# MrTornado24/IDE-3D

Hardware: NVIDIA H100
Metric: rendered frames/sec at 64^2 neural x 96 samples -> 512^2 (higher is better)
Workload: dtype f32

## Files before the change

ide-3d_b200/_lib.py:

```python

import ctypes as C
import os

import torch

_HERE = os.path.dirname(os.path.abspath(__file__))
LIB_PATH = os.environ.get('IDE3D_B200_LIB') or os.path.join(_HERE, 'lib', 'libide3d_b200.so')

OK, UNSUPPORTED, INVALID, CUDA_ERROR = 0, -1, -2, -3
F32, F16, F64 = 0, 1, 2
JITTER_NONE, JITTER_TENSOR, JITTER_HASH, JITTER_ZVALS = 0, 1, 2, 3
CLAMP_SOFTPLUS, CLAMP_RELU = 0, 1
PRECISION = {'auto': 0, 'fp32': 1, 'tc': 2}

_DTYPES = {torch.float32: F32, torch.float16: F16, torch.float64: F64}


class UpfirParams(C.Structure):
    _fields_ = [('x', C.c_void_p), ('f', C.c_void_p), ('y', C.c_void_p), ('dtype', C.c_int),
                ('up_x', C.c_int), ('up_y', C.c_int), ('down_x', C.c_int), ('down_y', C.c_int),
                ('pad_x0', C.c_int), ('pad_y0', C.c_int), ('flip', C.c_int), ('gain', C.c_float),
                ('in_w', C.c_int), ('in_h', C.c_int), ('in_c', C.c_int), ('in_n', C.c_int),
                ('in_stride_w', C.c_int64), ('in_stride_h', C.c_int64), ('in_stride_c', C.c_int64), ('in_stride_n', C.c_int64),
                ('f_w', C.c_int), ('f_h', C.c_int), ('f_stride_w', C.c_int64), ('f_stride_h', C.c_int64),
                ('out_w', C.c_int), ('out_h', C.c_int),
                ('out_stride_w', C.c_int64), ('out_stride_h', C.c_int64), ('out_stride_c', C.c_int64), ('out_stride_n', C.c_int64)]


class FirEpilogue(C.Structure):
    _fields_ = [('scale', C.c_void_p), ('noise', C.c_void_p), ('b', C.c_void_p), ('scale2', C.c_void_p), ('y2', C.c_void_p),
                ('act', C.c_int), ('alpha', C.c_float), ('gain', C.c_float), ('clamp', C.c_float), ('noise_batch', C.c_int64)]


class StyleLayer(C.Structure):
    _fields_ = [('affine_w', C.c_void_p), ('affine_b', C.c_void_p), ('wsq', C.c_void_p), ('w_gain', C.c_float), ('b_gain', C.c_float),
                ('out_scale', C.c_float), ('w_index', C.c_int), ('in_ch', C.c_int), ('out_ch', C.c_int),
                ('style_off', C.c_int64), ('dcoef_off', C.c_int64)]


class FlreluParams(C.Structure):
    _fields_ = [('x', C.c_void_p), ('b', C.c_void_p), ('fu', C.c_void_p), ('fd', C.c_void_p), ('y', C.c_void_p),
                ('s', C.c_void_p), ('dtype', C.c_int), ('up', C.c_int), ('down', C.c_int),
                ('fu_w', C.c_int), ('fu_h', C.c_int), ('fd_w', C.c_int), ('fd_h', C.c_int),
                ('pad_x0', C.c_int), ('pad_y0', C.c_int), ('flip', C.c_int),
                ('gain', C.c_float), ('slope', C.c_float), ('clamp', C.c_float),
                ('x_w', C.c_int), ('x_h', C.c_int), ('x_c', C.c_int), ('x_n', C.c_int),
                ('x_stride_w', C.c_int64), ('x_stride_h', C.c_int64), ('x_stride_c', C.c_int64), ('x_stride_n', C.c_int64),
                ('y_w', C.c_int), ('y_h', C.c_int),
                ('y_stride_w', C.c_int64), ('y_stride_h', C.c_int64), ('y_stride_c', C.c_int64), ('y_stride_n', C.c_int64),
                ('s_w', C.c_int), ('s_h', C.c_int), ('s_ofs_x', C.c_int), ('s_ofs_y', C.c_int),
                ('write_signs', C.c_int), ('read_signs', C.c_int)]


class FlreluActParams(C.Structure):
    _fields_ = [('x', C.c_void_p), ('s', C.c_void_p), ('dtype', C.c_int),
                ('x_w', C.c_int), ('x_h', C.c_int), ('x_c', C.c_int), ('x_n', C.c_int),
                ('x_stride_w', C.c_int64), ('x_stride_h', C.c_int64), ('x_stride_c', C.c_int64), ('x_stride_n', C.c_int64),
                ('s_w', C.c_int), ('s_h', C.c_int), ('s_ofs_x', C.c_int), ('s_ofs_y', C.c_int),
                ('gain', C.c_float), ('slope', C.c_float), ('clamp', C.c_float),
                ('write_signs', C.c_int), ('read_signs', C.c_int)]


class TriPlane(C.Structure):
    _fields_ = [('data', C.c_void_p), ('n', C.c_int), ('h', C.c_int), ('w', C.c_int),
                ('stride_n', C.c_int64), ('stride_c', C.c_int64), ('stride_h', C.c_int64), ('stride_w', C.c_int64)]


class MlpHead(C.Structure):
    _fields_ = [('in_sel', C.c_int), ('hidden', C.c_int), ('out_offset', C.c_int), ('out_count', C.c_int),
                ('w1', C.c_void_p), ('b1', C.c_void_p), ('w2', C.c_void_p), ('b2', C.c_void_p)]


class Decoder(C.Structure):
    _fields_ = [('num_heads', C.c_int), ('heads', MlpHead * 4)]


class RaymarchParams(C.Structure):
    _fields_ = [('tex', TriPlane), ('seg', TriPlane), ('dec', Decoder), ('cam2world', C.c_void_p),
                ('n', C.c_int), ('res_w', C.c_int), ('res_h', C.c_int), ('num_steps', C.c_int),
                ('fov_deg', C.c_float), ('ray_start', C.c_float), ('ray_end', C.c_float), ('box_scale', C.c_float),
                ('jitter_mode', C.c_int), ('jitter_u', C.c_void_p), ('jitter_seed', C.c_uint64),
                ('clamp_mode', C.c_int), ('last_back', C.c_int), ('white_back', C.c_int), ('max_depth', C.c_float),
                ('fill_weight', C.c_int), ('noise_std', C.c_float), ('noise', C.c_void_p),
                ('out_feat', C.c_void_p), ('out_depth', C.c_void_p), ('out_weights', C.c_void_p), ('precision', C.c_int),
                ('views', C.c_int), ('jitter_seeds', C.c_void_p)]


class RasterParams(C.Structure):
    _fields_ = [('vertices', C.c_void_p), ('triangles', C.c_void_p), ('normals', C.c_void_p), ('cam2world', C.c_void_p),
                ('num_vertices', C.c_int64), ('num_triangles', C.c_int64), ('num_frames', C.c_int), ('width', C.c_int), ('height', C.c_int),
                ('yfov_deg', C.c_float), ('znear', C.c_float), ('base', C.c_float), ('ambient', C.c_float), ('diffuse', C.c_float),
                ('background', C.c_int), ('rgb', C.c_void_p), ('ids', C.c_void_p), ('scratch', C.c_void_p), ('scratch_bytes', C.c_int64)]


FRAMES_IMAGE_SEG, FRAMES_IMAGE_DEPTH = 1, 2
FRAMES_PARTIALS = 64


class FramesParams(C.Structure):
    _fields_ = [('image', C.c_void_p), ('n', C.c_int), ('height', C.c_int), ('width', C.c_int),
                ('image_stride_n', C.c_int64), ('image_stride_c', C.c_int64), ('image_stride_h', C.c_int64), ('image_stride_w', C.c_int64),
                ('seg', C.c_void_p), ('seg_c', C.c_int), ('seg_h', C.c_int), ('seg_w', C.c_int),
                ('seg_stride_n', C.c_int64), ('seg_stride_c', C.c_int64), ('seg_stride_h', C.c_int64), ('seg_stride_w', C.c_int64),
                ('lut', C.c_void_p), ('mode', C.c_int), ('out', C.c_void_p), ('scratch', C.c_void_p)]


class StripsParams(C.Structure):
    _fields_ = [('image', C.c_void_p), ('seeds', C.c_int), ('views', C.c_int), ('height', C.c_int), ('width', C.c_int),
                ('image_stride_n', C.c_int64), ('image_stride_c', C.c_int64), ('image_stride_h', C.c_int64), ('image_stride_w', C.c_int64),
                ('seg', C.c_void_p), ('seg_c', C.c_int), ('seg_h', C.c_int), ('seg_w', C.c_int),
                ('seg_stride_n', C.c_int64), ('seg_stride_c', C.c_int64), ('seg_stride_h', C.c_int64), ('seg_stride_w', C.c_int64),
                ('lut', C.c_void_p), ('out_image', C.c_void_p), ('out_seg', C.c_void_p)]


NOISE_MAX_BUFFERS = 64


class NoiseTable(C.Structure):
    _fields_ = [('count', C.c_int), ('sides', C.c_int * NOISE_MAX_BUFFERS), ('bufs', C.c_void_p * NOISE_MAX_BUFFERS),
                ('grads', C.c_void_p * NOISE_MAX_BUFFERS), ('scratch', C.c_void_p), ('scratch_floats', C.c_int64)]


class SegXentParams(C.Structure):
    _fields_ = [('seg', C.c_void_p), ('n', C.c_int), ('classes', C.c_int), ('in_h', C.c_int), ('in_w', C.c_int),
                ('seg_stride_n', C.c_int64), ('seg_stride_c', C.c_int64), ('seg_stride_h', C.c_int64), ('seg_stride_w', C.c_int64),
                ('mask', C.c_void_p), ('out_h', C.c_int), ('out_w', C.c_int), ('lse', C.c_void_p), ('partials', C.c_void_p),
                ('loss', C.c_void_p), ('grad_loss', C.c_void_p), ('grad_seg', C.c_void_p)]


LPIPS_MAX_LAYERS = 8


class LpipsLayer(C.Structure):
    _fields_ = [('c', C.c_int), ('h', C.c_int), ('w', C.c_int), ('x', C.c_void_p), ('x_stride', C.c_int64 * 4),
                ('y', C.c_void_p), ('y_stride', C.c_int64 * 4), ('lin', C.c_void_p),
                ('grad_x', C.c_void_p), ('gx_stride', C.c_int64 * 4), ('grad_y', C.c_void_p), ('gy_stride', C.c_int64 * 4)]


class LpipsParams(C.Structure):
    _fields_ = [('n', C.c_int), ('num_layers', C.c_int), ('layers', LpipsLayer * LPIPS_MAX_LAYERS), ('value', C.c_void_p),
                ('scratch', C.c_void_p), ('scratch_bytes', C.c_int64), ('grad_value', C.c_void_p)]


_lib = None


class _StreamHandle(int):
    device = None


class _GuardedLib:

    def __init__(self, lib):
        self._lib = lib

    def __getattr__(self, name):
        fn = getattr(self._lib, name)
        if not name.startswith('ide3d_'):
            return fn

        def call(*args):
            dev = getattr(args[-1], 'device', None) if args else None
            if dev is None:
                return fn(*args)
            with torch.cuda.device(dev):
                return fn(*args)

        call.__name__ = name
        self.__dict__[name] = call
        return call


def get_lib():
    global _lib
    if _lib is not None:
        return _lib
    if not os.path.exists(LIB_PATH):
        raise RuntimeError(f'ide3d_b200: CUDA library not built ({LIB_PATH} missing); run '
                           f'`python {os.path.join(_HERE, "build.py")}` -- there is no CPU fallback')
    lib = C.CDLL(LIB_PATH, mode=os.RTLD_NOW)
    lib.ide3d_last_error.restype = C.c_char_p
    lib.ide3d_launch_count.restype = C.c_uint64
    vp, i32, i64, f32 = C.c_void_p, C.c_int, C.c_int64, C.c_float
    lib.ide3d_bias_act.argtypes = [vp, vp, vp, vp, vp, vp, i32, i32, i32, f32, f32, f32, i64, i64, i64, vp]
    lib.ide3d_modconv_epilogue.argtypes = [vp, vp, vp, vp, vp, vp, vp, i32, i32, f32, f32, f32, i64, i64, i64, i64, i32, vp]
    lib.ide3d_modconv_epilogue_rgb.argtypes = [vp, vp, vp, vp, vp, vp, vp, vp, vp, vp, vp, vp, i64, i32, i32, f32, f32, f32, i64, i64, i64,
                                               i64, vp]
    lib.ide3d_upfirdn2d.argtypes = [C.POINTER(UpfirParams), vp]
    lib.ide3d_upfirdn2d_add.argtypes = [C.POINTER(UpfirParams), vp, i64, i64, i64, vp, vp]
    lib.ide3d_upfirdn2d_epilogue.argtypes = [C.POINTER(UpfirParams), C.POINTER(FirEpilogue), vp]
    lib.ide3d_filtered_lrelu.argtypes = [C.POINTER(FlreluParams), vp]
    lib.ide3d_filtered_lrelu_act.argtypes = [C.POINTER(FlreluActParams), vp]
    lib.ide3d_raymarch_fwd.argtypes = [C.POINTER(RaymarchParams), vp]
    lib.ide3d_raymarch_bwd.argtypes = [C.POINTER(RaymarchParams), vp, vp, vp, vp, C.POINTER(C.c_void_p), vp]
    lib.ide3d_raymarch_bwd_cam.argtypes = [C.POINTER(RaymarchParams), vp, vp, vp, vp, C.POINTER(C.c_void_p), vp, vp]
    lib.ide3d_sample_voxel.argtypes = [C.POINTER(TriPlane), C.POINTER(TriPlane), C.POINTER(Decoder), vp, i64, f32, i32, vp, vp]
    lib.ide3d_sigma_grid.argtypes = [C.POINTER(TriPlane), C.POINTER(TriPlane), C.POINTER(Decoder), i32,
                                     C.POINTER(C.c_float * 3), f32, f32, f32, i64, i64, vp, vp]
    lib.ide3d_planes_to_nhwc.argtypes = [vp, i32, i32, i32, i32, i64, i64, i64, i64, vp, vp]
    lib.ide3d_initial_rays.argtypes = [i32, i32, f32, i32, i32, f32, f32, vp, vp, vp, vp]
    lib.ide3d_transform_points.argtypes = [vp, vp, vp, vp, vp, i32, i32, i32, vp, vp, vp, vp, vp]
    lib.ide3d_sample_triplane.argtypes = [C.POINTER(TriPlane), vp, i64, vp, vp]
    lib.ide3d_mask2color.argtypes = [vp, i32, i32, i32, i32, i64, i64, i64, i64, vp, vp, i32, vp]
    lib.ide3d_integrate.argtypes = [vp, vp, vp, vp, f32, i32, i32, i32, i32, i32, i32, i32, f32, i32, vp, vp, vp, vp]
    lib.ide3d_sample_pdf.argtypes = [vp, vp, vp, i32, i32, i32, f32, vp, vp]
    lib.ide3d_mc_classify.argtypes = [vp, i32, i32, i32, f32, vp, vp, vp]
    lib.ide3d_mc_emit.argtypes = [vp, i32, i32, i32, f32, vp, vp, vp, vp, vp, vp, vp]
    lib.ide3d_style_plan.argtypes = [vp, i32, i32, i32, C.POINTER(StyleLayer), i32, vp, vp, vp]
    lib.ide3d_mesh_normals.argtypes = [vp, vp, i64, vp, vp, vp, vp]
    lib.ide3d_raster_scratch_bytes.argtypes = [i32, i32, i32, i64, i64]
    lib.ide3d_raster_scratch_bytes.restype = C.c_int64
    lib.ide3d_raster.argtypes = [C.POINTER(RasterParams), vp]
    lib.ide3d_video_frames.argtypes = [C.POINTER(FramesParams), vp]
    lib.ide3d_image_strips.argtypes = [C.POINTER(StripsParams), vp]
    lib.ide3d_noise_reg.argtypes = [C.POINTER(NoiseTable), vp, vp, vp]
    lib.ide3d_noise_normalize.argtypes = [C.POINTER(NoiseTable), vp]
    lib.ide3d_seg_xent_fwd.argtypes = [C.POINTER(SegXentParams), vp]
    lib.ide3d_seg_xent_bwd.argtypes = [C.POINTER(SegXentParams), vp]
    lib.ide3d_lpips_scratch_bytes.argtypes = [C.POINTER(LpipsParams)]
    lib.ide3d_lpips_scratch_bytes.restype = C.c_int64
    lib.ide3d_lpips_fwd.argtypes = [C.POINTER(LpipsParams), vp]
    lib.ide3d_lpips_bwd.argtypes = [C.POINTER(LpipsParams), vp]
    for name in ('bias_act', 'upfirdn2d', 'filtered_lrelu', 'filtered_lrelu_act', 'raymarch_fwd', 'raymarch_bwd', 'raymarch_bwd_cam', 'sample_voxel',
                 'sigma_grid', 'planes_to_nhwc', 'initial_rays', 'transform_points', 'sample_triplane', 'integrate',
                 'sample_pdf', 'style_plan', 'mc_classify', 'mc_emit', 'mesh_normals', 'raster', 'video_frames', 'image_strips',
                 'noise_reg', 'noise_normalize', 'seg_xent_fwd', 'seg_xent_bwd', 'lpips_fwd', 'lpips_bwd', 'abi_version'):
        getattr(lib, 'ide3d_' + name).restype = C.c_int
    if lib.ide3d_abi_version() != 1:
        raise RuntimeError('ide3d_b200: ABI version mismatch between _lib.py and libide3d_b200.so')
    _lib = _GuardedLib(lib)
    return _lib


def exported_symbols():
    return ['ide3d_abi_version', 'ide3d_last_error', 'ide3d_launch_count', 'ide3d_bias_act', 'ide3d_modconv_epilogue', 'ide3d_modconv_epilogue_rgb',
            'ide3d_upfirdn2d', 'ide3d_upfirdn2d_add', 'ide3d_upfirdn2d_epilogue',
            'ide3d_filtered_lrelu', 'ide3d_filtered_lrelu_act', 'ide3d_raymarch_fwd', 'ide3d_raymarch_bwd', 'ide3d_raymarch_bwd_cam', 'ide3d_sample_voxel',
            'ide3d_sigma_grid', 'ide3d_planes_to_nhwc', 'ide3d_initial_rays', 'ide3d_transform_points',
            'ide3d_sample_triplane', 'ide3d_integrate', 'ide3d_sample_pdf', 'ide3d_mask2color', 'ide3d_style_plan', 'ide3d_mc_classify', 'ide3d_mc_emit',
            'ide3d_mesh_normals', 'ide3d_raster_scratch_bytes', 'ide3d_raster', 'ide3d_video_frames', 'ide3d_image_strips',
            'ide3d_noise_reg', 'ide3d_noise_normalize', 'ide3d_seg_xent_fwd', 'ide3d_seg_xent_bwd',
            'ide3d_lpips_scratch_bytes', 'ide3d_lpips_fwd', 'ide3d_lpips_bwd']


def check(rc, allow_unsupported=False):
    if rc == OK or (allow_unsupported and rc == UNSUPPORTED):
        return rc
    msg = get_lib().ide3d_last_error().decode(errors='replace')
    raise RuntimeError(f'ide3d_b200: {msg} (status {rc})')


def require_cuda(*tensors):
    for t in tensors:
        if t is not None and (not isinstance(t, torch.Tensor) or t.device.type != 'cuda'):
            raise RuntimeError('ide3d_b200: tensors must reside on a CUDA device -- this package has no CPU path '
                               '(the CPU restatement lives in oracle/ and is test infrastructure only)')


def forbid_grad(name, *tensors):
    if torch.is_grad_enabled() and any(isinstance(t, torch.Tensor) and t.requires_grad for t in tensors):
        raise RuntimeError(f'ide3d_b200.{name}: inputs require grad, but this stage kernel is forward-only -- use '
                           f'ide3d_b200.render.raymarch (fused forward, render_grad backward) or wrap the call in torch.no_grad()')


def dtype_code(t):
    try:
        return _DTYPES[t.dtype]
    except KeyError:
        raise RuntimeError(f'ide3d_b200: unsupported dtype {t.dtype}') from None


def ptr(t):
    return None if t is None else t.data_ptr()


def stream_ptr(device=None):
    h = _StreamHandle(torch.cuda.current_stream(device).cuda_stream)
    h.device = torch.device('cuda', torch.cuda.current_device()) if device is None else torch.device(device)
    return h


def launch_count():
    return int(get_lib().ide3d_launch_count())


def triplane_view(t):
    if t.ndim != 4 or t.shape[1] != 96 or t.dtype != torch.float32:
        raise RuntimeError(f'ide3d_b200: tri-plane tensor must be float32 [N, 96, H, W], got {tuple(t.shape)} {t.dtype}')
    s = t.stride()
    return TriPlane(t.data_ptr(), t.shape[0], t.shape[2], t.shape[3], s[0], s[1], s[2], s[3])
```

ide-3d_b200/_plugins.py:

```python

import ctypes as C

import torch

from . import _lib as L


def _req(cond, msg):
    if not cond:
        raise RuntimeError(msg)


def _has(t):
    return t is not None and t.numel() > 0


def _suggest_memory_format(x):
    if x.ndim == 4 and x.is_contiguous(memory_format=torch.channels_last) and not x.is_contiguous():
        return torch.channels_last
    return torch.contiguous_format


def bias_act(x, b, xref, yref, dy, grad, dim, act, alpha, gain, clamp):
    L.require_cuda(x)
    _req(not _has(b) or (b.dtype == x.dtype and b.device == x.device), 'b must have the same dtype and device as x')
    for name, t in (('xref', xref), ('yref', yref), ('dy', dy)):
        _req(not _has(t) or (t.shape == x.shape and t.dtype == x.dtype and t.device == x.device),
             f'{name} must have the same shape, dtype, and device as x')
    _req(not _has(b) or b.ndim == 1, 'b must have rank 1')
    _req(not _has(b) or (0 <= dim < x.ndim), 'dim is out of bounds')
    _req(not _has(b) or b.shape[0] == x.shape[dim], 'b has wrong number of elements')
    _req(grad >= 0, 'grad must be non-negative')
    dense = x.is_contiguous() or (x.ndim == 4 and x.is_contiguous(memory_format=torch.channels_last))
    _req(dense, 'x must be non-overlapping and dense')
    for t in (xref, yref, dy):
        _req(not _has(t) or t.stride() == x.stride(), 'xref, yref and dy must have the same layout as x')
    if _has(b):
        b = b.contiguous()
    y = torch.empty_like(x)
    if x.numel() == 0:
        return y
    step_b = x.stride(dim) if _has(b) else 1
    rc = L.get_lib().ide3d_bias_act(L.ptr(x), L.ptr(b) if _has(b) else None, L.ptr(xref) if _has(xref) else None,
                                    L.ptr(yref) if _has(yref) else None, L.ptr(dy) if _has(dy) else None, L.ptr(y),
                                    L.dtype_code(x), int(grad), int(act), float(alpha), float(gain), float(clamp),
                                    x.numel(), b.numel() if _has(b) else 0, step_b, L.stream_ptr(x.device))
    L.check(rc)
    return y


def modconv_epilogue(x, scale, noise, b, act, alpha, gain, clamp, next_scale=None, only_next=False):
    L.require_cuda(x)
    _req(x.ndim == 4, 'x must be rank 4')
    n, c, h, w = x.shape
    cl = (not x.is_contiguous()) and x.is_contiguous(memory_format=torch.channels_last)
    _req(x.is_contiguous() or cl, 'x must be non-overlapping and dense')
    vec = 16 // x.element_size()
    if x.numel() == 0 or (cl and c % vec != 0) or (not cl and (h * w) % vec != 0):
        return None
    if _has(scale):
        _req(scale.numel() == n * c, 'scale must have N*C elements')
        scale = scale.to(dtype=x.dtype).reshape(n, c).contiguous()
    noise_batch = 1
    if _has(noise):
        _req(noise.numel() in (h * w, n * h * w), 'noise must be [H,W] or [N,1,H,W]')
        noise_batch = noise.numel() // (h * w)
        noise = noise.to(dtype=x.dtype).contiguous()
    if _has(b):
        _req(b.ndim == 1 and b.shape[0] == c, 'b has wrong number of elements')
        b = b.to(dtype=x.dtype).contiguous()
    y = y2 = None
    if _has(next_scale):
        _req(next_scale.numel() == n * c, 'next_scale must have N*C elements')
        next_scale = next_scale.to(dtype=x.dtype).reshape(n, c).contiguous()
        y2 = torch.empty_like(x)
    if not (only_next and y2 is not None):
        y = torch.empty_like(x)
    rc = L.get_lib().ide3d_modconv_epilogue(L.ptr(x), L.ptr(scale) if _has(scale) else None, L.ptr(noise) if _has(noise) else None,
                                            L.ptr(b) if _has(b) else None, L.ptr(y) if y is not None else None,
                                            L.ptr(next_scale) if y2 is not None else None, L.ptr(y2) if y2 is not None else None,
                                            L.dtype_code(x), int(act), float(alpha), float(gain), float(clamp), n, c, h * w,
                                            noise_batch, int(cl), L.stream_ptr(x.device))
    if L.check(rc, allow_unsupported=True) == L.UNSUPPORTED:
        return None
    if y2 is None:
        return y
    return y2 if y is None else (y, y2)


def modconv_epilogue_rgb(x, scale, noise, b, act, alpha, gain, clamp, emit_y=True, y_scale=None, next_scale=None, rgb=None):
    L.require_cuda(x)
    _req(x.ndim == 4, 'x must be rank 4')
    n, c, h, w = x.shape
    cl = (not x.is_contiguous()) and x.is_contiguous(memory_format=torch.channels_last)
    if not cl or x.dtype != torch.float32 or c % 4 != 0 or c > 512 or x.numel() == 0:
        return None

    def per_sample(t, name):
        if not _has(t):
            return None
        _req(t.numel() == n * c, f'{name} must have N*C elements')
        return t.to(dtype=x.dtype).reshape(n, c).contiguous()

    scale, y_scale, next_scale = per_sample(scale, 'scale'), per_sample(y_scale, 'y_scale'), per_sample(next_scale, 'next_scale')
    noise_batch = 1
    if _has(noise):
        _req(noise.numel() in (h * w, n * h * w), 'noise must be [H,W] or [N,1,H,W]')
        noise_batch = noise.numel() // (h * w)
        noise = noise.to(dtype=x.dtype).contiguous()
    if _has(b):
        _req(b.ndim == 1 and b.shape[0] == c, 'b has wrong number of elements')
        b = b.to(dtype=x.dtype).contiguous()
    _req(y_scale is None or emit_y, 'y_scale needs emit_y')
    wrgb = srgb = brgb = out_rgb = None
    o = 0
    if rgb is not None:
        wrgb, srgb, brgb = rgb
        o = wrgb.shape[0]
        if o > 4:
            return None
        _req(wrgb.numel() == o * c, 'rgb weight must be [O, C, 1, 1]')
        wrgb = wrgb.to(dtype=x.dtype).reshape(o, c).contiguous()
        srgb = per_sample(srgb, 'rgb styles')
        if brgb is not None:
            _req(brgb.numel() == o, 'rgb bias must have O elements')
            brgb = brgb.to(dtype=x.dtype).contiguous()
        out_rgb = torch.empty([n, o, h, w], dtype=x.dtype, device=x.device)
    y = torch.empty_like(x) if emit_y else None
    y2 = torch.empty_like(x) if next_scale is not None else None
    _req(y is not None or y2 is not None or out_rgb is not None, 'no output requested')
    opt = lambda t: L.ptr(t) if t is not None else None
    rc = L.get_lib().ide3d_modconv_epilogue_rgb(L.ptr(x), opt(scale), opt(noise), opt(b), opt(y_scale), opt(y), opt(next_scale), opt(y2),
                                                opt(wrgb), opt(srgb), opt(brgb), opt(out_rgb), o, L.dtype_code(x), int(act), float(alpha),
                                                float(gain), float(clamp), n, c, h * w, noise_batch, L.stream_ptr(x.device))
    if L.check(rc, allow_unsupported=True) == L.UNSUPPORTED:
        return None
    return [t for t in (y, y2, out_rgb) if t is not None]


def upfirdn2d(x, f, upx, upy, downx, downy, padx0, padx1, pady0, pady1, flip, gain, add=None, bias=None, epilogue=None):
    L.require_cuda(x, f)
    _req(f.device == x.device, 'f must reside on the same device as x')
    _req(f.dtype == torch.float32, 'f must be float32')
    _req(x.numel() > 0, 'x has zero size')
    _req(f.numel() > 0, 'f has zero size')
    _req(x.ndim == 4, 'x must be rank 4')
    _req(f.ndim == 2, 'f must be rank 2')
    _req(f.shape[0] >= 1 and f.shape[1] >= 1, 'f must be at least 1x1')
    _req(upx >= 1 and upy >= 1, 'upsampling factor must be at least 1')
    _req(downx >= 1 and downy >= 1, 'downsampling factor must be at least 1')
    n, c, h, w = x.shape
    fh, fw = f.shape
    out_w = (w * upx + padx0 + padx1 - fw + downx) // downx
    out_h = (h * upy + pady0 + pady1 - fh + downy) // downy
    _req(out_w >= 1 and out_h >= 1, 'output must be at least 1x1')
    y = torch.empty([n, c, out_h, out_w], dtype=x.dtype, device=x.device, memory_format=_suggest_memory_format(x))
    xs, ys, fs = x.stride(), y.stride(), f.stride()
    p = L.UpfirParams(L.ptr(x), L.ptr(f), L.ptr(y), L.dtype_code(x), upx, upy, downx, downy, padx0, pady0,
                      1 if flip else 0, float(gain), w, h, c, n, xs[3], xs[2], xs[1], xs[0],
                      fw, fh, fs[1], fs[0], out_w, out_h, ys[3], ys[2], ys[1], ys[0])
    if epilogue is not None:
        e = epilogue
        if not (y.is_contiguous(memory_format=torch.channels_last) and not y.is_contiguous()) or e['act'] not in (1, 3) or x.dtype == torch.float64:
            return None
        def prep(t, numel):
            if t is None:
                return None
            _req(t.numel() == numel, 'epilogue operand has the wrong number of elements')
            return t.to(dtype=x.dtype).contiguous()
        scale, b, scale2 = prep(e.get('scale'), n * c), prep(e.get('b'), c), prep(e.get('next_scale'), n * c)
        noise = e.get('noise')
        noise_batch = 1
        if noise is not None:
            _req(noise.numel() in (out_h * out_w, n * out_h * out_w), 'noise must be [H,W] or [N,1,H,W]')
            noise_batch = noise.numel() // (out_h * out_w)
            noise = noise.to(dtype=x.dtype).contiguous()
        y2 = torch.empty_like(y) if scale2 is not None else None
        want_y = not (e.get('only_next') and y2 is not None)
        if not want_y:
            p.y = None
        ep = L.FirEpilogue(L.ptr(scale) if scale is not None else None, L.ptr(noise) if noise is not None else None,
                           L.ptr(b) if b is not None else None, L.ptr(scale2) if scale2 is not None else None,
                           L.ptr(y2) if y2 is not None else None, int(e['act']), float(e['alpha']), float(e['gain']),
                           float(e['clamp']), noise_batch)
        rc = L.get_lib().ide3d_upfirdn2d_epilogue(C.byref(p), C.byref(ep), L.stream_ptr(x.device))
        if L.check(rc, allow_unsupported=True) == L.UNSUPPORTED:
            return None
        if y2 is None:
            return y
        return (y, y2) if want_y else y2
    if add is not None:
        if tuple(add.shape) != (n, c, out_h, out_w) or add.dtype != x.dtype or add.stride(1) != 1 or not y.is_contiguous(memory_format=torch.channels_last) or y.is_contiguous():
            return None
        if bias is not None:
            bias = bias.to(dtype=x.dtype).contiguous()
        a = add.stride()
        rc = L.get_lib().ide3d_upfirdn2d_add(C.byref(p), L.ptr(add), a[0], a[2], a[3], L.ptr(bias) if bias is not None else None,
                                             L.stream_ptr(x.device))
        return None if L.check(rc, allow_unsupported=True) == L.UNSUPPORTED else y
    L.check(L.get_lib().ide3d_upfirdn2d(C.byref(p), L.stream_ptr(x.device)))
    return y


def filtered_lrelu(x, fu, fd, b, si, up, down, px0, px1, py0, py1, sx, sy, gain, slope, clamp, flip_filters, writeSigns):
    L.require_cuda(x, fu, fd, b)
    _req(fu.device == x.device and fd.device == x.device and b.device == x.device, 'all input tensors must reside on the same device')
    _req(fu.dtype == torch.float32 and fd.dtype == torch.float32, 'fu and fd must be float32')
    _req(b.dtype == x.dtype, 'x and b must have the same dtype')
    _req(x.dtype in (torch.float16, torch.float32), 'x and b must be float16 or float32')
    _req(x.ndim == 4, 'x must be rank 4')
    _req(x.numel() > 0, 'x is empty')
    _req(fu.ndim in (1, 2) and fd.ndim in (1, 2), 'fu and fd must be rank 1 or 2')
    _req(fu.numel() > 0, 'fu is empty')
    _req(fd.numel() > 0, 'fd is empty')
    _req(b.ndim == 1 and b.shape[0] == x.shape[1], 'b must be a vector with the same number of channels as x')
    _req(up >= 1 and down >= 1, 'up and down must be at least 1')
    n, c, xh, xw = x.shape
    fut_w, fut_h = fu.shape[-1] - 1, fu.shape[0] - 1
    fdt_w, fdt_h = fd.shape[-1] - 1, fd.shape[0] - 1
    cw = xw * up + (px0 + px1) - fut_w
    ch = xh * up + (py0 + py1) - fut_h
    _req(cw > fdt_w and ch > fdt_h, 'upsampled buffer must be at least the size of downsampling filter')
    yw = (cw - fdt_w + (down - 1)) // down
    yh = (ch - fdt_h + (down - 1)) // down
    _req(yw > 0 and yh > 0, 'output must be at least 1x1')
    read_signs = _has(si)
    s = si if read_signs else None
    so = None
    sw = sh = 0
    y = torch.empty([n, c, yh, yw], dtype=x.dtype, device=x.device, memory_format=_suggest_memory_format(x))
    if writeSigns:
        sw_active = yw * down - (down - 1) + fdt_w
        sh = yh * down - (down - 1) + fdt_h
        sw = (sw_active + 15) & ~15
        s = so = torch.empty([n, c, sh, sw >> 2], dtype=torch.uint8, device=x.device)
    elif read_signs:
        _req(s.is_contiguous(), 'signs must be contiguous')
        _req(s.dtype == torch.uint8, 'signs must be uint8')
        _req(s.ndim == 4 and s.shape[0] == n and s.shape[1] == c, 'signs must have same batch & channels as x')
        sw, sh = s.shape[3] << 2, s.shape[2]
    fu_c, fd_c = fu.contiguous(), fd.contiguous()
    xs, ys = x.stride(), y.stride()
    p = L.FlreluParams(L.ptr(x), L.ptr(b.contiguous()), L.ptr(fu_c), L.ptr(fd_c), L.ptr(y), L.ptr(s) if s is not None else None,
                       L.dtype_code(x), up, down, fu.shape[-1], fu.shape[0] if fu.ndim == 2 else 0,
                       fd.shape[-1], fd.shape[0] if fd.ndim == 2 else 0, px0, py0, 1 if flip_filters else 0,
                       float(gain), float(slope), float(min(clamp, 3.0e38)), xw, xh, c, n, xs[3], xs[2], xs[1], xs[0],
                       yw, yh, ys[3], ys[2], ys[1], ys[0], sw, sh, sx, sy, 1 if writeSigns else 0,
                       1 if (read_signs and not writeSigns) else 0)
    rc = L.check(L.get_lib().ide3d_filtered_lrelu(C.byref(p), L.stream_ptr(x.device)), allow_unsupported=True)
    if rc == L.UNSUPPORTED:
        return None, None, -1
    return y, so, 0


def filtered_lrelu_act_(x, si, sx, sy, gain, slope, clamp, writeSigns):
    L.require_cuda(x)
    _req(x.ndim == 4, 'x must be rank 4')
    _req(x.numel() > 0, 'x is empty')
    _req(x.dtype in (torch.float16, torch.float32, torch.float64), 'x must be float16, float32 or float64')
    read_signs = _has(si)
    s, so = (si if read_signs else None), None
    n, c, h, w = x.shape
    if writeSigns:
        sw = (w + 15) & ~15
        s = so = torch.empty([n, c, h, sw >> 2], dtype=torch.uint8, device=x.device)
    if s is not None:
        _req(s.is_contiguous(), 'signs must be contiguous')
        _req(s.dtype == torch.uint8, 'signs must be uint8')
        _req(s.device == x.device, 'signs must reside on the same device as x')
        _req(s.ndim == 4 and s.shape[0] == n and s.shape[1] == c, 'signs must have same batch & channels as x')
    xs = x.stride()
    p = L.FlreluActParams(L.ptr(x), L.ptr(s) if s is not None else None, L.dtype_code(x), w, h, c, n,
                          xs[3], xs[2], xs[1], xs[0], (s.shape[3] << 2) if s is not None else 0,
                          s.shape[2] if s is not None else 0, sx, sy, float(gain), float(slope),
                          float(min(clamp, 3.0e38)), 1 if writeSigns else 0, 1 if (read_signs and not writeSigns) else 0)
    L.check(L.get_lib().ide3d_filtered_lrelu_act(C.byref(p), L.stream_ptr(x.device)))
    return so


class _Plugin:

    def __init__(self, name, **funcs):
        self.__name__ = name
        self.__dict__.update(funcs)


PLUGINS = {
    'bias_act_plugin': _Plugin('bias_act_plugin', bias_act=bias_act, modconv_epilogue=modconv_epilogue,
                                 modconv_epilogue_rgb=modconv_epilogue_rgb),
    'upfirdn2d_plugin': _Plugin('upfirdn2d_plugin', upfirdn2d=upfirdn2d),
    'filtered_lrelu_plugin': _Plugin('filtered_lrelu_plugin', filtered_lrelu=filtered_lrelu,
                                     filtered_lrelu_act_=filtered_lrelu_act_),
}
```

ide-3d_b200/build.py:

```python

import hashlib
import os
import shutil
import subprocess
import sys
from concurrent.futures import ThreadPoolExecutor

HERE = os.path.dirname(os.path.abspath(__file__))
CSRC = os.path.join(HERE, 'csrc')
OBJ = os.path.join(HERE, '_build_tuning' if os.environ.get('IDE3D_BUILD_TUNING', '0') == '1' else '_build')
LIBDIR = os.path.join(HERE, 'lib')
LIB = os.path.join(LIBDIR, 'libide3d_b200_tuning.so' if os.environ.get('IDE3D_BUILD_TUNING', '0') == '1' else 'libide3d_b200.so')
TUNING = os.environ.get('IDE3D_BUILD_TUNING', '0') == '1'
UNITS = ['capi', 'raymarch', 'raymarch_bwd', 'raymarch_tc', 'voxel', 'voxel_tc', 'stages', 'style_plan', 'mcubes', 'raster', 'frames', 'strips', 'projector', 'lpips', 'bias_act', 'upfirdn2d', 'filtered_lrelu', 'filtered_lrelu_fused']
NVCC_FLAGS = ['-O3', '-std=c++17', '--expt-relaxed-constexpr', '-gencode', 'arch=compute_90a,code=sm_90a',
              '-lineinfo', '-Xcompiler', '-fPIC', '-Xptxas', '-v'] + (['-DIDE3D_TUNING'] if TUNING else [])


def _nvcc():
    for cand in (os.environ.get('NVCC'), shutil.which('nvcc'), '/usr/local/cuda/bin/nvcc'):
        if cand and os.path.exists(cand):
            return cand
    raise RuntimeError('nvcc not found (set NVCC=/path/to/nvcc)')


def _sources():
    return [u for u in UNITS if os.path.exists(os.path.join(CSRC, u + '.cu'))]


def _digest():
    h = hashlib.sha256(' '.join(NVCC_FLAGS).encode())
    names = sorted(os.listdir(CSRC)) + ['../../include/ide3d_b200.h']
    for n in names:
        p = os.path.join(CSRC, n)
        if os.path.isfile(p):
            h.update(n.encode())
            h.update(open(p, 'rb').read())
    return h.hexdigest()


def _compile(nvcc, unit, verbose):
    src = os.path.join(CSRC, unit + '.cu')
    obj = os.path.join(OBJ, unit + '.o')
    cmd = [nvcc, '-c'] + NVCC_FLAGS + [src, '-o', obj]
    r = subprocess.run(cmd, stdout=subprocess.PIPE, stderr=subprocess.STDOUT, text=True)
    with open(os.path.join(OBJ, unit + '.log'), 'w') as f:
        f.write(' '.join(cmd) + '\n' + r.stdout)
    if r.returncode != 0:
        raise RuntimeError(f'nvcc failed on {unit}.cu:\n{r.stdout[-6000:]}')
    if verbose:
        print(r.stdout)
    return obj


def build(force=False, verbose=False):
    os.makedirs(OBJ, exist_ok=True)
    os.makedirs(LIBDIR, exist_ok=True)
    stamp = os.path.join(LIBDIR, 'build_tuning.sha256' if TUNING else 'build.sha256')
    digest = _digest()
    if not force and os.path.exists(LIB) and os.path.exists(stamp) and open(stamp).read().strip() == digest:
        return LIB
    nvcc = _nvcc()
    units = _sources()
    with ThreadPoolExecutor(max_workers=min(8, len(units))) as ex:
        objs = list(ex.map(lambda u: _compile(nvcc, u, verbose), units))
    cmd = [nvcc, '-shared', '-gencode', 'arch=compute_90a,code=sm_90a', '-o', LIB] + objs + ['-lcudart']
    r = subprocess.run(cmd, stdout=subprocess.PIPE, stderr=subprocess.STDOUT, text=True)
    if r.returncode != 0:
        raise RuntimeError('link failed:\n' + r.stdout)
    with open(stamp, 'w') as f:
        f.write(digest)
    return LIB


if __name__ == '__main__':
    path = build(force='--force' in sys.argv, verbose='--verbose' in sys.argv)
    print(path)
```

ide-3d_b200/csrc/bias_act.cu:

```cuda
#include "common.cuh"

namespace ide3d {

struct BiasActArgs {
    const void *x, *b, *xref, *yref, *dy;
    void* y;
    int grad;
    float alpha, gain, clamp;
    long long size_x, size_b, step_b;
};

template <typename T> struct Acc { using type = float; };
template <> struct Acc<double> { using type = double; };

template <typename S> __device__ __forceinline__ S exp_(S v);
template <> __device__ __forceinline__ float exp_<float>(float v) { return __expf(v); }
template <> __device__ __forceinline__ double exp_<double>(double v) { return exp(v); }
template <typename S> __device__ __forceinline__ S log_(S v);
template <> __device__ __forceinline__ float log_<float>(float v) { return __logf(v); }
template <> __device__ __forceinline__ double log_<double>(double v) { return log(v); }

template <typename S, int A>
__device__ __forceinline__ S eval(S x, S b, S xref, S yref, S dy, int G, S alpha, S gain, S clamp) {
    const S one = (S)1, two = (S)2, expRange = (S)80, halfExpRange = (S)40;
    const S seluScale = (S)1.0507009873554804934193349852946, seluAlpha = (S)1.6732632423543772848170429916717;
    const S yy = (gain != (S)0) ? yref / gain : (S)0;
    S y = 0;
    if (G == 0) x += b; else xref += b;
    if (A == 1) { y = x; if (G == 2) y = 0; }
    if (A == 2) { if (G == 0) y = (x > 0) ? x : 0; if (G == 1) y = (yy > 0) ? x : 0; }
    if (A == 3) { if (G == 0) y = (x > 0) ? x : x * alpha; if (G == 1) y = (yy > 0) ? x : x * alpha; }
    if (A == 4) {
        if (G == 0) { const S c = exp_(x), d = one / c; y = (x < -expRange) ? -one : (x > expRange) ? one : (c - d) / (c + d); }
        if (G == 1) y = x * (one - yy * yy);
        if (G == 2) y = x * (one - yy * yy) * (-two * yy);
    }
    if (A == 5) {
        if (G == 0) y = (x < -expRange) ? 0 : one / (exp_(-x) + one);
        if (G == 1) y = x * yy * (one - yy);
        if (G == 2) y = x * yy * (one - yy) * (one - two * yy);
    }
    if (A == 6) {
        if (G == 0) y = (x >= 0) ? x : exp_(x) - one;
        if (G == 1) y = (yy >= 0) ? x : x * (yy + one);
        if (G == 2) y = (yy >= 0) ? 0 : x * (yy + one);
    }
    if (A == 7) {
        if (G == 0) y = (x >= 0) ? seluScale * x : (seluScale * seluAlpha) * (exp_(x) - one);
        if (G == 1) y = (yy >= 0) ? x * seluScale : x * (yy + seluScale * seluAlpha);
        if (G == 2) y = (yy >= 0) ? 0 : x * (yy + seluScale * seluAlpha);
    }
    if (A == 8) {
        if (G == 0) y = (x > expRange) ? x : log_(exp_(x) + one);
        if (G == 1) y = x * (one - exp_(-yy));
        if (G == 2) { const S c = exp_(-yy); y = x * c * (one - c); }
    }
    if (A == 9) {
        if (G == 0) {
            y = (x < -expRange) ? 0 : x / (exp_(-x) + one);
        } else {
            const S c = exp_(xref), d = c + one;
            if (G == 1) y = (xref > halfExpRange) ? x : x * c * (xref + d) / (d * d);
            else y = (xref > halfExpRange) ? 0 : x * c * (xref * (two - d) + two * d) / (d * d * d);
            yref = (xref < -expRange) ? 0 : xref / (exp_(-xref) + one) * gain;
        }
    }
    y *= gain * dy;
    if (clamp >= 0) {
        if (G == 0) y = (y > -clamp & y < clamp) ? y : (y >= 0) ? clamp : -clamp;
        else y = (yref > -clamp & yref < clamp) ? y : 0;
    }
    return y;
}

__device__ __forceinline__ long long bias_index(long long e, const BiasActArgs& p, bool small) {
    if (small) return (long long)(((unsigned)e / (unsigned)p.step_b) % (unsigned)p.size_b);
    return (e / p.step_b) % p.size_b;
}

template <typename T> struct Vec;
template <> struct Vec<float> { static constexpr int N = 4; using type = float4; };
template <> struct Vec<__half> { static constexpr int N = 8; using type = uint4; };
template <> struct Vec<double> { static constexpr int N = 2; using type = double2; };

template <typename T> __device__ __forceinline__ typename Acc<T>::type to_acc(T v) { return (typename Acc<T>::type)v; }
template <> __device__ __forceinline__ float to_acc<__half>(__half v) { return __half2float(v); }
template <typename T> __device__ __forceinline__ T from_acc(typename Acc<T>::type v) { return (T)v; }
template <> __device__ __forceinline__ __half from_acc<__half>(float v) { return __float2half(v); }

__device__ __forceinline__ void load_vec(const float* p, long long v, float (&o)[4]) {
    const float4 t = __ldcs(reinterpret_cast<const float4*>(p) + v);
    o[0] = t.x; o[1] = t.y; o[2] = t.z; o[3] = t.w;
}
__device__ __forceinline__ void load_vec(const double* p, long long v, double (&o)[2]) {
    const double2 t = __ldcs(reinterpret_cast<const double2*>(p) + v);
    o[0] = t.x; o[1] = t.y;
}
__device__ __forceinline__ void load_vec(const __half* p, long long v, float (&o)[8]) {
    const uint4 t = __ldcs(reinterpret_cast<const uint4*>(p) + v);
    const unsigned w[4] = {t.x, t.y, t.z, t.w};
#pragma unroll
    for (int i = 0; i < 4; ++i) {
        const float2 f = __half22float2(*reinterpret_cast<const __half2*>(&w[i]));
        o[2 * i] = f.x; o[2 * i + 1] = f.y;
    }
}
__device__ __forceinline__ void store_vec(float* p, long long v, const float (&o)[4]) {
    __stcs(reinterpret_cast<float4*>(p) + v, make_float4(o[0], o[1], o[2], o[3]));
}
__device__ __forceinline__ void store_vec(double* p, long long v, const double (&o)[2]) {
    __stcs(reinterpret_cast<double2*>(p) + v, make_double2(o[0], o[1]));
}
__device__ __forceinline__ void store_vec(__half* p, long long v, const float (&o)[8]) {
    unsigned w[4];
#pragma unroll
    for (int i = 0; i < 4; ++i) {
        const __half2 h = __floats2half2_rn(o[2 * i], o[2 * i + 1]);
        w[i] = *reinterpret_cast<const unsigned*>(&h);
    }
    __stcs(reinterpret_cast<uint4*>(p) + v, make_uint4(w[0], w[1], w[2], w[3]));
}

template <typename T, int A, int UNROLL, bool kFwd>
__global__ void __launch_bounds__(256) bias_act_kernel(const BiasActArgs p, const int bmode) {
    using S = typename Acc<T>::type;
    constexpr int N = Vec<T>::N;
    const S alpha = (S)p.alpha, gain = (S)p.gain, clamp = (S)p.clamp;
    const int G = kFwd ? 0 : p.grad;
    const T* x = (const T*)p.x;
    const T* b = (const T*)p.b;
    const T* xref = (const T*)p.xref;
    const T* yref = (const T*)p.yref;
    const T* dy = (const T*)p.dy;
    T* y = (T*)p.y;
    const long long nvec = p.size_x / N;
    const long long stride = (long long)gridDim.x * blockDim.x;
    const bool small = p.size_x <= 0x7fffffffll;

    for (long long v0 = (long long)blockIdx.x * blockDim.x + threadIdx.x; v0 < nvec; v0 += stride * UNROLL) {
        S vx[UNROLL][N];
#pragma unroll
        for (int u = 0; u < UNROLL; ++u) {
            const long long v = v0 + u * stride;
            if (v < nvec) load_vec(x, v, vx[u]);
        }
#pragma unroll
        for (int u = 0; u < UNROLL; ++u) {
            const long long v = v0 + u * stride;
            if (v >= nvec) continue;
            const long long e0 = v * N;
            S exr[N], eyr[N], edy[N], out[N], bb[N];
            if (xref) load_vec(xref, v, exr);
            if (yref) load_vec(yref, v, eyr);
            if (dy) load_vec(dy, v, edy);
            if (bmode == 1) {
                const S t = to_acc<T>(b[bias_index(e0, p, small)]);
#pragma unroll
                for (int j = 0; j < N; ++j) bb[j] = t;
            } else if (bmode == 2) {
                const long long i0 = small ? (long long)((unsigned)e0 % (unsigned)p.size_b) : e0 % p.size_b;
#pragma unroll
                for (int j = 0; j < N; ++j) bb[j] = to_acc<T>(b[i0 + j]);
            } else {
#pragma unroll
                for (int j = 0; j < N; ++j) bb[j] = (bmode == 3) ? to_acc<T>(b[bias_index(e0 + j, p, small)]) : (S)0;
            }
#pragma unroll
            for (int j = 0; j < N; ++j)
                out[j] = eval<S, A>(vx[u][j], bb[j], xref ? exr[j] : (S)0, yref ? eyr[j] : (S)0, dy ? edy[j] : (S)1, G, alpha, gain, clamp);
            store_vec(y, v, out);
        }
    }
    const long long tail0 = nvec * N;
    for (long long e = tail0 + (long long)blockIdx.x * blockDim.x + threadIdx.x; e < p.size_x; e += stride) {
        const S bb = b ? to_acc<T>(b[bias_index(e, p, small)]) : (S)0;
        y[e] = from_acc<T>(eval<S, A>(to_acc<T>(x[e]), bb, xref ? to_acc<T>(xref[e]) : (S)0,
                                      yref ? to_acc<T>(yref[e]) : (S)0, dy ? to_acc<T>(dy[e]) : (S)1, G, alpha,
                                      gain, clamp));
    }
}

template <typename T, int A, int UNROLL, bool kFwd>
__global__ void __launch_bounds__(256) bias_act_planar_kernel(const BiasActArgs p, long long plane_elems, long long chunks_per_plane,
                                                             long long items) {
    using S = typename Acc<T>::type;
    constexpr int N = Vec<T>::N;
    const S alpha = (S)p.alpha, gain = (S)p.gain, clamp = (S)p.clamp;
    const int G = kFwd ? 0 : p.grad;
    const T* b = (const T*)p.b;
    const long long plane_vecs = plane_elems / N;
    for (long long item = blockIdx.x; item < items; item += gridDim.x) {
        const long long plane = item / chunks_per_plane;
        const long long chunk = item - plane * chunks_per_plane;
        const S bias = b ? to_acc<T>(b[plane % p.size_b]) : (S)0;
        const long long vbase = plane * plane_vecs;
        const long long v0 = chunk * (256 * UNROLL) + threadIdx.x;
        S vx[UNROLL][N];
#pragma unroll
        for (int u = 0; u < UNROLL; ++u)
            if (v0 + u * 256 < plane_vecs) load_vec((const T*)p.x, vbase + v0 + u * 256, vx[u]);
#pragma unroll
        for (int u = 0; u < UNROLL; ++u) {
            const long long vi = v0 + u * 256;
            if (vi >= plane_vecs) continue;
            const long long v = vbase + vi;
            S exr[N], eyr[N], edy[N], out[N];
            if (p.xref) load_vec((const T*)p.xref, v, exr);
            if (p.yref) load_vec((const T*)p.yref, v, eyr);
            if (p.dy) load_vec((const T*)p.dy, v, edy);
#pragma unroll
            for (int j = 0; j < N; ++j)
                out[j] = eval<S, A>(vx[u][j], bias, p.xref ? exr[j] : (S)0, p.yref ? eyr[j] : (S)0, p.dy ? edy[j] : (S)1, G, alpha, gain, clamp);
            store_vec((T*)p.y, v, out);
        }
    }
}

template <typename T, int A>
static int launch_bias_act(const BiasActArgs& p, cudaStream_t st) {
    constexpr int UNROLL = 4;
    constexpr int N = Vec<T>::N;
    const long long nvec = p.size_x / N;
    long long blocks = ceil_div<long long>(nvec > 0 ? nvec : 1, 256ll * UNROLL);
    const long long cap = (long long)sm_count() * 8;
    if (blocks > cap) blocks = cap;
    if (blocks < 1) blocks = 1;
    int bmode = 0;
    if (p.b != nullptr) bmode = (p.step_b % N == 0) ? 1 : ((p.step_b == 1 && p.size_b % N == 0) ? 2 : 3);
    const long long plane_elems = (p.b == nullptr) ? p.size_x : p.step_b;
    if ((p.b == nullptr || bmode == 1) && plane_elems >= 1024 && plane_elems % N == 0 && p.size_x % plane_elems == 0) {
        const long long cpp = ceil_div<long long>(plane_elems / N, 256ll * UNROLL);
        const long long items = (p.size_x / plane_elems) * cpp;
        long long g = items < cap ? items : cap;
        if (p.grad == 0) bias_act_planar_kernel<T, A, UNROLL, true><<<(unsigned)g, 256, 0, st>>>(p, plane_elems, cpp, items);
        else bias_act_planar_kernel<T, A, UNROLL, false><<<(unsigned)g, 256, 0, st>>>(p, plane_elems, cpp, items);
        IDE3D_CHECK_LAUNCH("bias_act_planar_kernel");
        return IDE3D_OK;
    }
    if (p.grad == 0) bias_act_kernel<T, A, UNROLL, true><<<(unsigned)blocks, 256, 0, st>>>(p, bmode);
    else bias_act_kernel<T, A, UNROLL, false><<<(unsigned)blocks, 256, 0, st>>>(p, bmode);
    IDE3D_CHECK_LAUNCH("bias_act_kernel");
    return IDE3D_OK;
}

template <typename T>
static int dispatch_act(const BiasActArgs& p, int act, cudaStream_t st) {
    switch (act) {
        case 1: return launch_bias_act<T, 1>(p, st);
        case 2: return launch_bias_act<T, 2>(p, st);
        case 3: return launch_bias_act<T, 3>(p, st);
        case 4: return launch_bias_act<T, 4>(p, st);
        case 5: return launch_bias_act<T, 5>(p, st);
        case 6: return launch_bias_act<T, 6>(p, st);
        case 7: return launch_bias_act<T, 7>(p, st);
        case 8: return launch_bias_act<T, 8>(p, st);
        case 9: return launch_bias_act<T, 9>(p, st);
    }
    IDE3D_FAIL(IDE3D_INVALID, "bias_act: unknown activation index %d", act);
}

}

using namespace ide3d;

extern "C" int ide3d_bias_act(const void* x, const void* b, const void* xref, const void* yref, const void* dy,
                              void* y, int dtype, int grad, int act, float alpha, float gain, float clamp,
                              int64_t size_x, int64_t size_b, int64_t step_b, ide3d_stream_t stream) {
    IDE3D_REQUIRE(size_x >= 0, "bias_act: negative size");
    if (size_x == 0) return IDE3D_OK;
    IDE3D_REQUIRE(x && y, "bias_act: null x/y");
    IDE3D_REQUIRE(grad >= 0 && grad <= 2, "bias_act: grad must be 0, 1 or 2");
    IDE3D_REQUIRE(b == nullptr || (size_b > 0 && step_b > 0), "bias_act: bad bias geometry");
    const uintptr_t all = (uintptr_t)x | (uintptr_t)y | (uintptr_t)xref | (uintptr_t)yref | (uintptr_t)dy;
    IDE3D_REQUIRE((all & 15) == 0, "bias_act: tensors must be 16-byte aligned");
    BiasActArgs p{x, b, xref, yref, dy, y, grad, alpha, gain, clamp, size_x, size_b > 0 ? size_b : 1,
                  step_b > 0 ? step_b : 1};
    cudaStream_t st = (cudaStream_t)stream;
    switch (dtype) {
        case IDE3D_F32: return dispatch_act<float>(p, act, st);
        case IDE3D_F16: return dispatch_act<__half>(p, act, st);
        case IDE3D_F64: return dispatch_act<double>(p, act, st);
    }
    IDE3D_FAIL(IDE3D_INVALID, "bias_act: unsupported dtype %d", dtype);
}

namespace ide3d {

struct EpiArgs {
    const void *x, *scale, *noise, *b;
    void* y;
    const void* scale2;
    void* y2;
    float alpha, gain, clamp;
    long long n, c, hw;
    int noise_batch;
};

template <typename T> __device__ __forceinline__ void load_vec_keep(const T* p, long long v, typename Acc<T>::type (&o)[Vec<T>::N]);
template <> __device__ __forceinline__ void load_vec_keep<float>(const float* p, long long v, float (&o)[4]) {
    const float4 t = __ldg(reinterpret_cast<const float4*>(p) + v);
    o[0] = t.x; o[1] = t.y; o[2] = t.z; o[3] = t.w;
}
template <> __device__ __forceinline__ void load_vec_keep<double>(const double* p, long long v, double (&o)[2]) {
    const double2 t = __ldg(reinterpret_cast<const double2*>(p) + v);
    o[0] = t.x; o[1] = t.y;
}
template <> __device__ __forceinline__ void load_vec_keep<__half>(const __half* p, long long v, float (&o)[8]) {
    const uint4 t = __ldg(reinterpret_cast<const uint4*>(p) + v);
    const unsigned w[4] = {t.x, t.y, t.z, t.w};
#pragma unroll
    for (int i = 0; i < 4; ++i) {
        const float2 f = __half22float2(*reinterpret_cast<const __half2*>(&w[i]));
        o[2 * i] = f.x; o[2 * i + 1] = f.y;
    }
}

template <typename T, int A, int UNROLL>
__global__ void __launch_bounds__(256) modconv_epilogue_planar_kernel(const EpiArgs p, long long chunks_per_plane, long long items) {
    using S = typename Acc<T>::type;
    constexpr int N = Vec<T>::N;
    const S alpha = (S)p.alpha, gain = (S)p.gain, clamp = (S)p.clamp;
    const long long plane_vecs = p.hw / N;
    for (long long item = blockIdx.x; item < items; item += gridDim.x) {
        const long long plane = item / chunks_per_plane;
        const long long chunk = item - plane * chunks_per_plane;
        const long long smp = plane / p.c;
        const S d = p.scale ? to_acc<T>(((const T*)p.scale)[plane]) : (S)1;
        const S bias = p.b ? to_acc<T>(((const T*)p.b)[plane - smp * p.c]) : (S)0;
        const S d2 = p.y2 ? to_acc<T>(((const T*)p.scale2)[plane]) : (S)1;
        const long long vbase = plane * plane_vecs;
        const long long nbase = (p.noise_batch == 1 ? 0 : smp) * plane_vecs;
        const long long v0 = chunk * (256 * UNROLL) + threadIdx.x;
        S vx[UNROLL][N], vn[UNROLL][N];
#pragma unroll
        for (int u = 0; u < UNROLL; ++u)
            if (v0 + u * 256 < plane_vecs) {
                load_vec((const T*)p.x, vbase + v0 + u * 256, vx[u]);
                if (p.noise) load_vec_keep<T>((const T*)p.noise, nbase + v0 + u * 256, vn[u]);
            }
#pragma unroll
        for (int u = 0; u < UNROLL; ++u) {
            const long long vi = v0 + u * 256;
            if (vi >= plane_vecs) continue;
            S out[N];
#pragma unroll
            for (int j = 0; j < N; ++j) {
                const S t = p.noise ? vx[u][j] * d + vn[u][j] : vx[u][j] * d;
                out[j] = eval<S, A>(t, bias, (S)0, (S)0, (S)1, 0, alpha, gain, clamp);
            }
            if (p.y) store_vec((T*)p.y, vbase + vi, out);
            if (p.y2) {
#pragma unroll
                for (int j = 0; j < N; ++j) out[j] *= d2;
                store_vec((T*)p.y2, vbase + vi, out);
            }
        }
    }
}

template <typename T, int A, int UNROLL>
__global__ void __launch_bounds__(256) modconv_epilogue_cl_kernel(const EpiArgs p, unsigned chunks_per_sample, long long items, int cv_shift) {
    using S = typename Acc<T>::type;
    constexpr int N = Vec<T>::N;
    const S alpha = (S)p.alpha, gain = (S)p.gain, clamp = (S)p.clamp;
    const unsigned cv = (unsigned)(p.c / N);
    const unsigned svec = (unsigned)p.hw * cv;
    for (long long item = blockIdx.x; item < items; item += gridDim.x) {
        const unsigned smp = (unsigned)(item / chunks_per_sample);
        const unsigned chunk = (unsigned)(item - (long long)smp * chunks_per_sample);
        const long long vbase = (long long)smp * svec;
        const unsigned v0 = chunk * (256u * UNROLL) + threadIdx.x;
        S vx[UNROLL][N];
#pragma unroll
        for (int u = 0; u < UNROLL; ++u)
            if (v0 + u * 256u < svec) load_vec((const T*)p.x, vbase + v0 + u * 256u, vx[u]);
#pragma unroll
// ... 272 lines not shown
```

ide-3d_b200/csrc/tc_ptx.cuh:

```cuda
#pragma once

#include <cuda_bf16.h>
#include <stdint.h>

namespace ide3d {
namespace tc {

__device__ __forceinline__ uint32_t smem_u32(const void* p) { return (uint32_t)__cvta_generic_to_shared(p); }

__device__ __forceinline__ void fence_async_smem() { asm volatile("fence.proxy.async.shared::cta;" ::: "memory"); }

__device__ __forceinline__ void bar_sync(int id, int threads) { asm volatile("bar.sync %0, %1;" ::"r"(id), "r"(threads) : "memory"); }

__device__ __forceinline__ void wgmma_fence() { asm volatile("wgmma.fence.sync.aligned;" ::: "memory"); }
__device__ __forceinline__ void wgmma_commit() { asm volatile("wgmma.commit_group.sync.aligned;" ::: "memory"); }
template <int N> __device__ __forceinline__ void wgmma_wait() { asm volatile("wgmma.wait_group.sync.aligned %0;" ::"n"(N) : "memory"); }
template <int R> __device__ __forceinline__ void fence_regs(float (&d)[R]) {
#pragma unroll
    for (int i = 0; i < R; ++i) asm volatile("" : "+f"(d[i])::"memory");
}

__device__ __forceinline__ uint64_t make_sdesc_sw128(uint32_t smem_addr) {
    return (uint64_t)((smem_addr & 0x3FFFFu) >> 4) | (1ull << 16) | ((uint64_t)(1024u >> 4) << 32) | (1ull << 62);
}

__device__ __forceinline__ uint32_t sw128_offset(int r, int c) {
    return (uint32_t)((r >> 3) * 1024 + (r & 7) * 128 + (((c ^ r) & 7) << 4));
}

template <int N> struct Wgmma;

template <> struct Wgmma<16> {
    __device__ __forceinline__ static void ss(float* d, uint64_t a_desc, uint64_t b_desc, int scale_d) {
        asm volatile(
            "{\n\t.reg .pred p;\n\tsetp.ne.b32 p, %10, 0;\n\t"
            "wgmma.mma_async.sync.aligned.m64n16k16.f32.bf16.bf16 {%0, %1, %2, %3, %4, %5, %6, %7}, %8, %9, p, 1, 1, 0, 0;\n\t}\n"
            : "+f"(d[0]), "+f"(d[1]), "+f"(d[2]), "+f"(d[3]), "+f"(d[4]), "+f"(d[5]), "+f"(d[6]), "+f"(d[7])
            : "l"(a_desc), "l"(b_desc), "r"(scale_d));
    }
    __device__ __forceinline__ static void rs(float* d, const uint32_t (&a)[4], uint64_t b_desc) {
        asm volatile(
            "{\n\t.reg .pred p;\n\tsetp.ne.b32 p, %13, 0;\n\t"
            "wgmma.mma_async.sync.aligned.m64n16k16.f32.bf16.bf16 {%0, %1, %2, %3, %4, %5, %6, %7}, {%8, %9, %10, %11}, %12, p, 1, 1, 0;\n\t}\n"
            : "+f"(d[0]), "+f"(d[1]), "+f"(d[2]), "+f"(d[3]), "+f"(d[4]), "+f"(d[5]), "+f"(d[6]), "+f"(d[7])
            : "r"(a[0]), "r"(a[1]), "r"(a[2]), "r"(a[3]), "l"(b_desc), "r"(1));
    }
};

template <> struct Wgmma<32> {
    __device__ __forceinline__ static void ss(float* d, uint64_t a_desc, uint64_t b_desc, int scale_d) {
        asm volatile(
            "{\n\t.reg .pred p;\n\tsetp.ne.b32 p, %18, 0;\n\t"
            "wgmma.mma_async.sync.aligned.m64n32k16.f32.bf16.bf16 {%0, %1, %2, %3, %4, %5, %6, %7, %8, %9, %10, %11, %12, %13, %14, %15}, %16, %17, p, 1, 1, 0, 0;\n\t}\n"
            : "+f"(d[0]), "+f"(d[1]), "+f"(d[2]), "+f"(d[3]), "+f"(d[4]), "+f"(d[5]), "+f"(d[6]), "+f"(d[7]), "+f"(d[8]), "+f"(d[9]), "+f"(d[10]), "+f"(d[11]), "+f"(d[12]), "+f"(d[13]), "+f"(d[14]), "+f"(d[15])
            : "l"(a_desc), "l"(b_desc), "r"(scale_d));
    }
    __device__ __forceinline__ static void rs(float* d, const uint32_t (&a)[4], uint64_t b_desc) {
        asm volatile(
            "{\n\t.reg .pred p;\n\tsetp.ne.b32 p, %21, 0;\n\t"
            "wgmma.mma_async.sync.aligned.m64n32k16.f32.bf16.bf16 {%0, %1, %2, %3, %4, %5, %6, %7, %8, %9, %10, %11, %12, %13, %14, %15}, {%16, %17, %18, %19}, %20, p, 1, 1, 0;\n\t}\n"
            : "+f"(d[0]), "+f"(d[1]), "+f"(d[2]), "+f"(d[3]), "+f"(d[4]), "+f"(d[5]), "+f"(d[6]), "+f"(d[7]), "+f"(d[8]), "+f"(d[9]), "+f"(d[10]), "+f"(d[11]), "+f"(d[12]), "+f"(d[13]), "+f"(d[14]), "+f"(d[15])
            : "r"(a[0]), "r"(a[1]), "r"(a[2]), "r"(a[3]), "l"(b_desc), "r"(1));
    }
};

template <> struct Wgmma<48> {
    __device__ __forceinline__ static void ss(float* d, uint64_t a_desc, uint64_t b_desc, int scale_d) {
        asm volatile(
            "{\n\t.reg .pred p;\n\tsetp.ne.b32 p, %26, 0;\n\t"
            "wgmma.mma_async.sync.aligned.m64n48k16.f32.bf16.bf16 {%0, %1, %2, %3, %4, %5, %6, %7, %8, %9, %10, %11, %12, %13, %14, %15, %16, %17, %18, %19, %20, %21, %22, %23}, %24, %25, p, 1, 1, 0, 0;\n\t}\n"
            : "+f"(d[0]), "+f"(d[1]), "+f"(d[2]), "+f"(d[3]), "+f"(d[4]), "+f"(d[5]), "+f"(d[6]), "+f"(d[7]), "+f"(d[8]), "+f"(d[9]), "+f"(d[10]), "+f"(d[11]), "+f"(d[12]), "+f"(d[13]), "+f"(d[14]), "+f"(d[15]), "+f"(d[16]), "+f"(d[17]), "+f"(d[18]), "+f"(d[19]), "+f"(d[20]), "+f"(d[21]), "+f"(d[22]), "+f"(d[23])
            : "l"(a_desc), "l"(b_desc), "r"(scale_d));
    }
    __device__ __forceinline__ static void rs(float* d, const uint32_t (&a)[4], uint64_t b_desc) {
        asm volatile(
            "{\n\t.reg .pred p;\n\tsetp.ne.b32 p, %29, 0;\n\t"
            "wgmma.mma_async.sync.aligned.m64n48k16.f32.bf16.bf16 {%0, %1, %2, %3, %4, %5, %6, %7, %8, %9, %10, %11, %12, %13, %14, %15, %16, %17, %18, %19, %20, %21, %22, %23}, {%24, %25, %26, %27}, %28, p, 1, 1, 0;\n\t}\n"
            : "+f"(d[0]), "+f"(d[1]), "+f"(d[2]), "+f"(d[3]), "+f"(d[4]), "+f"(d[5]), "+f"(d[6]), "+f"(d[7]), "+f"(d[8]), "+f"(d[9]), "+f"(d[10]), "+f"(d[11]), "+f"(d[12]), "+f"(d[13]), "+f"(d[14]), "+f"(d[15]), "+f"(d[16]), "+f"(d[17]), "+f"(d[18]), "+f"(d[19]), "+f"(d[20]), "+f"(d[21]), "+f"(d[22]), "+f"(d[23])
            : "r"(a[0]), "r"(a[1]), "r"(a[2]), "r"(a[3]), "l"(b_desc), "r"(1));
    }
};

template <> struct Wgmma<64> {
    __device__ __forceinline__ static void ss(float* d, uint64_t a_desc, uint64_t b_desc, int scale_d) {
        asm volatile(
            "{\n\t.reg .pred p;\n\tsetp.ne.b32 p, %34, 0;\n\t"
            "wgmma.mma_async.sync.aligned.m64n64k16.f32.bf16.bf16 {%0, %1, %2, %3, %4, %5, %6, %7, %8, %9, %10, %11, %12, %13, %14, %15, %16, %17, %18, %19, %20, %21, %22, %23, %24, %25, %26, %27, %28, %29, %30, %31}, %32, %33, p, 1, 1, 0, 0;\n\t}\n"
            : "+f"(d[0]), "+f"(d[1]), "+f"(d[2]), "+f"(d[3]), "+f"(d[4]), "+f"(d[5]), "+f"(d[6]), "+f"(d[7]), "+f"(d[8]), "+f"(d[9]), "+f"(d[10]), "+f"(d[11]), "+f"(d[12]), "+f"(d[13]), "+f"(d[14]), "+f"(d[15]), "+f"(d[16]), "+f"(d[17]), "+f"(d[18]), "+f"(d[19]), "+f"(d[20]), "+f"(d[21]), "+f"(d[22]), "+f"(d[23]), "+f"(d[24]), "+f"(d[25]), "+f"(d[26]), "+f"(d[27]), "+f"(d[28]), "+f"(d[29]), "+f"(d[30]), "+f"(d[31])
            : "l"(a_desc), "l"(b_desc), "r"(scale_d));
    }
    __device__ __forceinline__ static void rs(float* d, const uint32_t (&a)[4], uint64_t b_desc) {
        asm volatile(
            "{\n\t.reg .pred p;\n\tsetp.ne.b32 p, %37, 0;\n\t"
            "wgmma.mma_async.sync.aligned.m64n64k16.f32.bf16.bf16 {%0, %1, %2, %3, %4, %5, %6, %7, %8, %9, %10, %11, %12, %13, %14, %15, %16, %17, %18, %19, %20, %21, %22, %23, %24, %25, %26, %27, %28, %29, %30, %31}, {%32, %33, %34, %35}, %36, p, 1, 1, 0;\n\t}\n"
            : "+f"(d[0]), "+f"(d[1]), "+f"(d[2]), "+f"(d[3]), "+f"(d[4]), "+f"(d[5]), "+f"(d[6]), "+f"(d[7]), "+f"(d[8]), "+f"(d[9]), "+f"(d[10]), "+f"(d[11]), "+f"(d[12]), "+f"(d[13]), "+f"(d[14]), "+f"(d[15]), "+f"(d[16]), "+f"(d[17]), "+f"(d[18]), "+f"(d[19]), "+f"(d[20]), "+f"(d[21]), "+f"(d[22]), "+f"(d[23]), "+f"(d[24]), "+f"(d[25]), "+f"(d[26]), "+f"(d[27]), "+f"(d[28]), "+f"(d[29]), "+f"(d[30]), "+f"(d[31])
            : "r"(a[0]), "r"(a[1]), "r"(a[2]), "r"(a[3]), "l"(b_desc), "r"(1));
    }
};

__device__ __forceinline__ void split_bf16(float x, __nv_bfloat16& hi, __nv_bfloat16& lo) {
    hi = __float2bfloat16_rn(x);
    lo = __float2bfloat16_rn(x - __bfloat162float(hi));
}
__device__ __forceinline__ void split4_bf16(const float (&f)[4], uint2& hi, uint2& lo) {
    const __nv_bfloat162 h01 = __floats2bfloat162_rn(f[0], f[1]), h23 = __floats2bfloat162_rn(f[2], f[3]);
    const float2 b01 = __bfloat1622float2(h01), b23 = __bfloat1622float2(h23);
    const __nv_bfloat162 l01 = __floats2bfloat162_rn(f[0] - b01.x, f[1] - b01.y), l23 = __floats2bfloat162_rn(f[2] - b23.x, f[3] - b23.y);
    hi = make_uint2(*reinterpret_cast<const uint32_t*>(&h01), *reinterpret_cast<const uint32_t*>(&h23));
    lo = make_uint2(*reinterpret_cast<const uint32_t*>(&l01), *reinterpret_cast<const uint32_t*>(&l23));
}
__device__ __forceinline__ void split2_bf16(float x0, float x1, uint32_t& hi, uint32_t& lo) {
    const __nv_bfloat162 h = __floats2bfloat162_rn(x0, x1);
    const float2 b = __bfloat1622float2(h);
    const __nv_bfloat162 l = __floats2bfloat162_rn(x0 - b.x, x1 - b.y);
    hi = *reinterpret_cast<const uint32_t*>(&h);
    lo = *reinterpret_cast<const uint32_t*>(&l);
}

}
}
```

ide-3d_b200/csrc/upfirdn2d.cu:

```cuda
#include <cuda.h>
#include <stdlib.h>

#include "common.cuh"

namespace ide3d {

struct UpfirArgs {
    const void* x;
    const float* f;
    void* y;
    int ux, uy, dx, dy, px0, py0, flip;
    float gain;
    int in_w, in_h, in_c, in_n;
    long long isw, ish, isc, isn;
    int fw, fh;
    long long fsw, fsh;
    int out_w, out_h;
    long long osw, osh, osc, osn;
    const void* add = nullptr;
    long long asw = 0, ash = 0, asn = 0;
    const void* bias = nullptr;
    int epi = 0, act = 1, noise_batch = 1;
    float alpha = 0.f, act_gain = 1.f, clamp = -1.f;
    const void *scale = nullptr, *noise = nullptr, *scale2 = nullptr;
    void* y2 = nullptr;
};

template <typename T> struct AccT { using type = float; };
template <> struct AccT<double> { using type = double; };
template <typename T> __device__ __forceinline__ typename AccT<T>::type ld(const T* p) { return (typename AccT<T>::type)(*p); }
template <> __device__ __forceinline__ float ld<__half>(const __half* p) { return __half2float(*p); }
template <typename T> __device__ __forceinline__ void st(T* p, typename AccT<T>::type v) { *p = (T)v; }
template <> __device__ __forceinline__ void st<__half>(__half* p, float v) { *p = __float2half(v); }

constexpr int cmod(int a, int m) { return ((a % m) + m) % m; }
constexpr int cfloor(int a, int m) { return (a - cmod(a, m)) / m; }
constexpr int kPatch = 4;
constexpr int kTile = 64;

template <int U, int D, int F, int PH>
struct Axis {
    static constexpr int k0(int j) { return cmod(PH - j * D, U); }
    static constexpr int taps(int j) { return k0(j) < F ? (F - k0(j) + U - 1) / U : 0; }
    static constexpr int off(int j) { return cfloor(j * D - PH + k0(j), U); }
    static constexpr int lo() {
        int m = 1 << 20;
        for (int j = 0; j < kPatch; ++j) if (taps(j) > 0 && off(j) < m) m = off(j);
        return m == (1 << 20) ? 0 : m;
    }
    static constexpr int hi() {
        int m = -(1 << 20);
        for (int j = 0; j < kPatch; ++j) if (taps(j) > 0 && off(j) + taps(j) - 1 > m) m = off(j) + taps(j) - 1;
        return m == -(1 << 20) ? 0 : m;
    }
    static constexpr int kWin = hi() - lo() + 1;
    static constexpr int kStep = kPatch * D / U;
    static constexpr int kTileIn = (kTile / kPatch - 1) * kStep + kWin;
    static_assert((kPatch * D) % U == 0, "patch origin must stay phase aligned");
};

template <typename T, typename TT, int UX, int UY, int DX, int DY, int FW, int FH, int PHX, int PHY, int PITCH>
__device__ __forceinline__ void patch_compute_store_impl(const UpfirArgs& p, const TT* __restrict__ tile,
                                                         const typename AccT<T>::type (&fk)[FH][FW], int n, int c, int ox_t, int oy_t) {
    using S = typename AccT<T>::type;
    using AX = Axis<UX, DX, FW, PHX>;
    using AY = Axis<UY, DY, FH, PHY>;
    constexpr int TIWP = PITCH;
    const int tx = threadIdx.x & 15, ty = threadIdx.x >> 4;
    const TT* wbase = tile + (ty * AY::kStep) * TIWP + tx * AX::kStep;
    S acc[kPatch][kPatch];
#pragma unroll
    for (int i = 0; i < kPatch; ++i)
#pragma unroll
        for (int j = 0; j < kPatch; ++j) acc[i][j] = 0;

#pragma unroll
    for (int r = 0; r < AY::kWin; ++r) {
        S win[AX::kWin];
#pragma unroll
        for (int q = 0; q < AX::kWin; ++q) win[q] = ld<TT>(wbase + r * TIWP + q);
#pragma unroll
        for (int i = 0; i < kPatch; ++i) {
#pragma unroll
            for (int ty_ = 0; ty_ < AY::taps(i); ++ty_) {
                if (AY::off(i) - AY::lo() + ty_ != r) continue;
                const int ky = AY::k0(i) + ty_ * UY;
#pragma unroll
                for (int j = 0; j < kPatch; ++j)
#pragma unroll
                    for (int tx_ = 0; tx_ < AX::taps(j); ++tx_)
                        acc[i][j] += fk[ky][AX::k0(j) + tx_ * UX] * win[AX::off(j) - AX::lo() + tx_];
            }
        }
    }

    const int ox0 = ox_t + tx * kPatch, oy0 = oy_t + ty * kPatch;
    T* yout = (T*)p.y + n * p.osn + c * p.osc;
#pragma unroll
    for (int i = 0; i < kPatch; ++i) {
        const int oy = oy0 + i;
        if (oy >= p.out_h) break;
        T* rowp = yout + oy * p.osh + ox0;
        if (sizeof(T) == 4 && ox0 + kPatch <= p.out_w && ((reinterpret_cast<uintptr_t>(rowp) & 15) == 0)) {
            __stcs(reinterpret_cast<float4*>(rowp), make_float4((float)acc[i][0], (float)acc[i][1], (float)acc[i][2], (float)acc[i][3]));
        } else {
#pragma unroll
            for (int j = 0; j < kPatch; ++j)
                if (ox0 + j < p.out_w) st<T>(rowp + j, acc[i][j]);
        }
    }
}

template <typename T, int UX, int UY, int DX, int DY, int FW, int FH, int PHX, int PHY, int PITCH>
__device__ __forceinline__ void patch_compute_store(const UpfirArgs& p, const typename AccT<T>::type* __restrict__ tile,
                                                    const typename AccT<T>::type (&fk)[FH][FW], int n, int c, int ox_t, int oy_t) {
    patch_compute_store_impl<T, typename AccT<T>::type, UX, UY, DX, DY, FW, FH, PHX, PHY, PITCH>(p, tile, fk, n, c, ox_t, oy_t);
}
template <int UX, int UY, int DX, int DY, int FW, int FH, int PHX, int PHY, int PITCH>
__device__ __forceinline__ void patch_compute_store_h(const UpfirArgs& p, const __half* __restrict__ tile, const float (&fk)[FH][FW],
                                                      int n, int c, int ox_t, int oy_t) {
    patch_compute_store_impl<__half, __half, UX, UY, DX, DY, FW, FH, PHX, PHY, PITCH>(p, tile, fk, n, c, ox_t, oy_t);
}

template <typename T, int UX, int UY, int DX, int DY, int FW, int FH, int PHX, int PHY, bool kVec>
__global__ void __launch_bounds__(256) upfirdn2d_patch_kernel(const UpfirArgs p, int tiles_x, int tiles_y) {
    using S = typename AccT<T>::type;
    using AX = Axis<UX, DX, FW, PHX>;
    using AY = Axis<UY, DY, FH, PHY>;
    constexpr int TIW = AX::kTileIn, TIH = AY::kTileIn;
    constexpr int TIWP = (kVec ? ((TIW + 3 + 3) / 4 * 4) : TIW) | 1;
    constexpr int TIV = (TIW + 3 + 3) / 4;
    extern __shared__ __align__(16) unsigned char smem_raw[];
    S* tile = reinterpret_cast<S*>(smem_raw);

    S fk[FH][FW];
#pragma unroll
    for (int ky = 0; ky < FH; ++ky)
#pragma unroll
        for (int kx = 0; kx < FW; ++kx) {
            const int sy = p.flip ? ky : FH - 1 - ky, sx = p.flip ? kx : FW - 1 - kx;
            fk[ky][kx] = (S)p.f[sy * p.fsh + sx * p.fsw] * (S)p.gain;
        }

    const int ax = floor_div(p.px0, UX), ay = floor_div(p.py0, UY);
    const long long tiles_plane = (long long)tiles_x * tiles_y;
    const long long total = tiles_plane * p.in_c * p.in_n;

    for (long long blk = blockIdx.x; blk < total; blk += gridDim.x) {
        const long long plane = blk / tiles_plane;
        const int t = (int)(blk - plane * tiles_plane);
        const int n = (int)(plane / p.in_c), c = (int)(plane - (long long)n * p.in_c);
        const int ox_t = (t % tiles_x) * kTile, oy_t = (t / tiles_x) * kTile;
        const int ix_t = ox_t * DX / UX - ax + AX::lo();
        const int iy_t = oy_t * DY / UY - ay + AY::lo();
        const T* xin = (const T*)p.x + n * p.isn + c * p.isc;

        __syncthreads();
        int shift = 0;
        if constexpr (kVec) {
            const int ixa = ix_t & ~3;
            shift = ix_t - ixa;
            for (int i = threadIdx.x; i < TIV * TIH; i += 256) {
                const int ty = i / TIV, tv = i - ty * TIV;
                const int gx = ixa + tv * 4, gy = iy_t + ty;
                float4 v = make_float4(0.f, 0.f, 0.f, 0.f);
                if ((unsigned)gx < (unsigned)p.in_w && (unsigned)gy < (unsigned)p.in_h)
                    v = __ldg(reinterpret_cast<const float4*>(reinterpret_cast<const float*>(xin) + gy * p.ish + gx));
                S* d = tile + ty * TIWP + tv * 4;
                d[0] = v.x; d[1] = v.y; d[2] = v.z; d[3] = v.w;
            }
        } else {
            for (int i = threadIdx.x; i < TIW * TIH; i += 256) {
                const int ty = i / TIW, tx = i - ty * TIW;
                const int gx = ix_t + tx, gy = iy_t + ty;
                S v = 0;
                if ((unsigned)gx < (unsigned)p.in_w && (unsigned)gy < (unsigned)p.in_h) v = ld<T>(xin + gy * p.ish + gx);
                tile[ty * TIWP + tx] = v;
            }
        }
        __syncthreads();

        patch_compute_store<T, UX, UY, DX, DY, FW, FH, PHX, PHY, TIWP>(p, tile + shift, fk, n, c, ox_t, oy_t);
    }
}

__device__ __forceinline__ unsigned smem_addr(const void* p) { return (unsigned)__cvta_generic_to_shared(p); }
__device__ __forceinline__ void tma_bar_init(unsigned long long* bar) {
    asm volatile("mbarrier.init.shared::cta.b64 [%0], 1;" ::"r"(smem_addr(bar)) : "memory");
}
__device__ __forceinline__ void tma_load_tile(void* dst, const CUtensorMap* map, unsigned long long* bar, int x, int y, int z, unsigned bytes) {
    asm volatile("mbarrier.arrive.expect_tx.shared::cta.b64 _, [%0], %1;" ::"r"(smem_addr(bar)), "r"(bytes) : "memory");
    asm volatile("cp.async.bulk.tensor.3d.shared::cluster.global.tile.mbarrier::complete_tx::bytes [%0], [%1, {%3, %4, %5}], [%2];"
                 ::"r"(smem_addr(dst)), "l"(map), "r"(smem_addr(bar)), "r"(x), "r"(y), "r"(z) : "memory");
}
__device__ __forceinline__ void tma_bar_wait(unsigned long long* bar, unsigned parity) {
    unsigned ok = 0;
    while (!ok) {
        asm volatile("{\n\t.reg .pred p;\n\tmbarrier.try_wait.parity.shared::cta.b64 p, [%1], %2;\n\tselp.u32 %0, 1, 0, p;\n\t}\n"
                     : "=r"(ok) : "r"(smem_addr(bar)), "r"(parity) : "memory");
    }
}

template <typename T, int UX, int UY, int DX, int DY, int FW, int FH, int PHX, int PHY>
struct TmaGeom {
    using AX = Axis<UX, DX, FW, PHX>;
    using AY = Axis<UY, DY, FH, PHY>;
    static constexpr int kVec = 16 / (int)sizeof(T);
    static constexpr int BW = (AX::kTileIn + kVec - 1 + kVec - 1) / kVec * kVec, BH = AY::kTileIn;
    static constexpr int kTileBytes = ((BW * BH * (int)sizeof(T) + 127) / 128) * 128;
    static constexpr int kSmem = 2 * kTileBytes + 128 + 128;
};

template <typename T, int UX, int UY, int DX, int DY, int FW, int FH, int PHX, int PHY>
__global__ void __launch_bounds__(256) upfirdn2d_patch_tma_kernel(const UpfirArgs p, int tiles_x, int tiles_y,
                                                                  const __grid_constant__ CUtensorMap tmap) {
    using GM = TmaGeom<T, UX, UY, DX, DY, FW, FH, PHX, PHY>;
    using AX = typename GM::AX;
    using AY = typename GM::AY;
    static_assert(sizeof(T) == sizeof(typename AccT<T>::type) || sizeof(T) == 2, "fp32 / fp16 only");
    static_assert((kTile * DX / UX) % GM::kVec == 0, "tile origins must keep the 16-byte phase of the box origin");
    extern __shared__ unsigned char tma_raw[];
    unsigned char* base = reinterpret_cast<unsigned char*>((reinterpret_cast<uintptr_t>(tma_raw) + 127) & ~(uintptr_t)127);
    T* tiles[2] = {reinterpret_cast<T*>(base), reinterpret_cast<T*>(base + GM::kTileBytes)};
    unsigned long long* bars = reinterpret_cast<unsigned long long*>(base + 2 * GM::kTileBytes);

    float fk[FH][FW];
#pragma unroll
    for (int ky = 0; ky < FH; ++ky)
#pragma unroll
        for (int kx = 0; kx < FW; ++kx) {
            const int sy = p.flip ? ky : FH - 1 - ky, sx = p.flip ? kx : FW - 1 - kx;
            fk[ky][kx] = p.f[sy * p.fsh + sx * p.fsw] * p.gain;
        }
    const int ax = floor_div(p.px0, UX), ay = floor_div(p.py0, UY);
    const long long tiles_plane = (long long)tiles_x * tiles_y;
    const long long total = tiles_plane * p.in_c * p.in_n;
    constexpr unsigned kBytes = GM::BW * GM::BH * sizeof(T);

    auto coords = [&](long long blk, int& plane, int& ox_t, int& oy_t) {
        const long long pl = blk / tiles_plane;
        const int t = (int)(blk - pl * tiles_plane);
        plane = (int)pl;
        ox_t = (t % tiles_x) * kTile; oy_t = (t / tiles_x) * kTile;
    };
    const int shift = (-ax + AX::lo()) & (GM::kVec - 1);
    auto issue = [&](long long blk, int buf) {
        int pl, ox_t, oy_t;
        coords(blk, pl, ox_t, oy_t);
        tma_load_tile(tiles[buf], &tmap, &bars[buf], ox_t * DX / UX - ax + AX::lo() - shift, oy_t * DY / UY - ay + AY::lo(), pl, kBytes);
    };
    if (threadIdx.x == 0) {
        tma_bar_init(&bars[0]); tma_bar_init(&bars[1]);
        asm volatile("fence.mbarrier_init.release.cluster;" ::: "memory");
        if ((long long)blockIdx.x < total) issue(blockIdx.x, 0);
    }
    __syncthreads();

    int it = 0;
    for (long long blk = blockIdx.x; blk < total; blk += gridDim.x, ++it) {
        const int cur = it & 1;
        const long long nxt = blk + gridDim.x;
        if (threadIdx.x == 0 && nxt < total) issue(nxt, cur ^ 1);
        int plane, ox_t, oy_t;
        coords(blk, plane, ox_t, oy_t);
        const int n = plane / p.in_c, c = plane - n * p.in_c;
        tma_bar_wait(&bars[cur], (it >> 1) & 1);
        if constexpr (sizeof(T) == 4) {
            patch_compute_store<T, UX, UY, DX, DY, FW, FH, PHX, PHY, GM::BW>(p, reinterpret_cast<const float*>(tiles[cur]) + shift, fk, n, c, ox_t, oy_t);
        } else {
            patch_compute_store_h<UX, UY, DX, DY, FW, FH, PHX, PHY, GM::BW>(p, reinterpret_cast<const __half*>(tiles[cur]) + shift, fk, n, c, ox_t, oy_t);
        }
        __syncthreads();
    }
}

template <typename T>
__global__ void __launch_bounds__(256) upfirdn2d_generic_kernel(const UpfirArgs p, int c_fastest) {
    using S = typename AccT<T>::type;
    const long long total = (long long)p.out_w * p.out_h * p.in_c * p.in_n;
    for (long long i = (long long)blockIdx.x * blockDim.x + threadIdx.x; i < total; i += (long long)gridDim.x * blockDim.x) {
        int ox, oy, c, n;
        long long r = i;
        if (c_fastest) { c = (int)(r % p.in_c); r /= p.in_c; ox = (int)(r % p.out_w); r /= p.out_w; oy = (int)(r % p.out_h); n = (int)(r / p.out_h); }
        else { ox = (int)(r % p.out_w); r /= p.out_w; oy = (int)(r % p.out_h); r /= p.out_h; c = (int)(r % p.in_c); n = (int)(r / p.in_c); }
        const int bx = ox * p.dx - p.px0, by = oy * p.dy - p.py0;
        const int kx0 = ((-bx) % p.ux + p.ux) % p.ux, ky0 = ((-by) % p.uy + p.uy) % p.uy;
        const T* xin = (const T*)p.x + n * p.isn + c * p.isc;
        S acc = 0;
        for (int ky = ky0; ky < p.fh; ky += p.uy) {
            const int iy = (by + ky) / p.uy;
            if (iy < 0 || by + ky < 0) continue;
            if (iy >= p.in_h) break;
            const int sy = p.flip ? ky : p.fh - 1 - ky;
            for (int kx = kx0; kx < p.fw; kx += p.ux) {
                const int ix = (bx + kx) / p.ux;
                if (ix < 0 || bx + kx < 0) continue;
                if (ix >= p.in_w) break;
                const int sx = p.flip ? kx : p.fw - 1 - kx;
                acc += (S)p.f[sy * p.fsh + sx * p.fsw] * ld<T>(xin + iy * p.ish + ix * p.isw);
            }
        }
        st<T>((T*)p.y + n * p.osn + c * p.osc + oy * p.osh + ox * p.osw, acc * (S)p.gain);
    }
}

typedef CUresult (*EncodeTiledFn)(CUtensorMap*, CUtensorMapDataType, cuuint32_t, void*, const cuuint64_t*, const cuuint64_t*,
                                  const cuuint32_t*, const cuuint32_t*, CUtensorMapInterleave, CUtensorMapSwizzle,
                                  CUtensorMapL2promotion, CUtensorMapFloatOOBfill);
static EncodeTiledFn encode_tiled() {
    static EncodeTiledFn fn = []() -> EncodeTiledFn {
        void* ptr = nullptr;
        cudaDriverEntryPointQueryResult qr;
        if (cudaGetDriverEntryPoint("cuTensorMapEncodeTiled", &ptr, cudaEnableDefault, &qr) != cudaSuccess || qr != cudaDriverEntryPointSuccess) return nullptr;
        return (EncodeTiledFn)ptr;
    }();
    return fn;
}

template <typename T>
static bool tma_eligible(const UpfirArgs& p) {
    if (sizeof(T) > 4 || encode_tiled() == nullptr) return false;
    if (p.isw != 1 || p.osw != 1) return false;
    if (p.isn != p.isc * p.in_c) return false;
    if ((reinterpret_cast<uintptr_t>(p.x) & 15) || (p.ish * sizeof(T)) % 16 || (p.isc * sizeof(T)) % 16) return false;
    if ((long long)p.in_c * p.in_n > 0x7fffffffll) return false;
    return true;
}

template <typename T, int UX, int UY, int DX, int DY, int FW, int FH, int PHX, int PHY>
static int launch_patch_tma(const UpfirArgs& p, cudaStream_t st_) {
    using GM = TmaGeom<T, UX, UY, DX, DY, FW, FH, PHX, PHY>;
    CUtensorMap map;
    const cuuint64_t dims[3] = {(cuuint64_t)p.in_w, (cuuint64_t)p.in_h, (cuuint64_t)p.in_c * p.in_n};
    const cuuint64_t strides[2] = {(cuuint64_t)p.ish * sizeof(T), (cuuint64_t)p.isc * sizeof(T)};
    const cuuint32_t box[3] = {(cuuint32_t)GM::BW, (cuuint32_t)GM::BH, 1};
    const cuuint32_t estr[3] = {1, 1, 1};
    const CUresult r = encode_tiled()(&map, sizeof(T) == 4 ? CU_TENSOR_MAP_DATA_TYPE_FLOAT32 : CU_TENSOR_MAP_DATA_TYPE_FLOAT16, 3,
                                      const_cast<void*>(p.x), dims, strides, box, estr, CU_TENSOR_MAP_INTERLEAVE_NONE,
                                      CU_TENSOR_MAP_SWIZZLE_NONE, CU_TENSOR_MAP_L2_PROMOTION_L2_128B, CU_TENSOR_MAP_FLOAT_OOB_FILL_NONE);
    if (r != CUDA_SUCCESS) IDE3D_FAIL(IDE3D_UNSUPPORTED, "upfirdn2d: cuTensorMapEncodeTiled failed (%d)", (int)r);
    auto kern = upfirdn2d_patch_tma_kernel<T, UX, UY, DX, DY, FW, FH, PHX, PHY>;
    const size_t smem = GM::kSmem;
    if (smem > 48 * 1024) IDE3D_CUDA(cudaFuncSetAttribute(kern, cudaFuncAttributeMaxDynamicSharedMemorySize, (int)smem));
    const int tiles_x = ceil_div(p.out_w, kTile), tiles_y = ceil_div(p.out_h, kTile);
    const long long total = (long long)tiles_x * tiles_y * p.in_c * p.in_n;
    int per_sm = 1;
    IDE3D_CUDA(cudaOccupancyMaxActiveBlocksPerMultiprocessor(&per_sm, kern, 256, smem));
    if (per_sm < 1) per_sm = 1;
    long long grid = (long long)sm_count() * per_sm;
    if (grid > total) grid = total;
    kern<<<(unsigned)grid, 256, smem, st_>>>(p, tiles_x, tiles_y, map);
    IDE3D_CHECK_LAUNCH("upfirdn2d_patch_tma_kernel");
    return IDE3D_OK;
}

template <typename T, int UX, int UY, int DX, int DY, int FW, int FH, int PHX, int PHY>
static int launch_patch(const UpfirArgs& p, cudaStream_t st_) {
    if constexpr (sizeof(T) <= 4) {
        constexpr bool fits = TmaGeom<T, UX, UY, DX, DY, FW, FH, PHX, PHY>::kSmem <= 200 * 1024;
        const char* tma_env = tuning_env("IDE3D_TMA");
        if (fits && !(tma_env != nullptr && tma_env[0] == '0') && tma_eligible<T>(p)) {
            const int rc = launch_patch_tma<T, UX, UY, DX, DY, FW, FH, PHX, PHY>(p, st_);
// ... 512 lines not shown
```

ide-3d_b200/torch_utils/ops/bias_act.py:

```python

import math

import torch

from .. import custom_ops


class _Spec(dict):
    __getattr__ = dict.__getitem__


def _spec(def_alpha, def_gain, cuda_idx, ref, has_2nd_grad):
    return _Spec(def_alpha=def_alpha, def_gain=def_gain, cuda_idx=cuda_idx, ref=ref, has_2nd_grad=has_2nd_grad)


_SQRT2 = math.sqrt(2)
activation_funcs = {
    'linear':   _spec(0,   1,      1, '',  False),
    'relu':     _spec(0,   _SQRT2, 2, 'y', False),
    'lrelu':    _spec(0.2, _SQRT2, 3, 'y', False),
    'tanh':     _spec(0,   1,      4, 'y', True),
    'sigmoid':  _spec(0,   1,      5, 'y', True),
    'elu':      _spec(0,   1,      6, 'y', True),
    'selu':     _spec(0,   1,      7, 'y', True),
    'softplus': _spec(0,   1,      8, 'y', True),
    'swish':    _spec(0,   _SQRT2, 9, 'x', True),
}

_plugin = None


def _init():
    global _plugin
    if _plugin is None:
        _plugin = custom_ops.get_plugin(module_name='bias_act_plugin', sources=['bias_act.cu'])
    return True


def _layout(x):
    if x.ndim == 4 and x.is_contiguous(memory_format=torch.channels_last):
        return x
    return x.contiguous()


class _BiasAct(torch.autograd.Function):
    @staticmethod
    def forward(ctx, x, b, dim, spec, alpha, gain, clamp):
        x = _layout(x)
        y = _plugin.bias_act(x, b, None, None, None, 0, dim, spec.cuda_idx, alpha, gain, clamp)
        ctx.cfg = (dim, spec, alpha, gain, clamp)
        ctx.has_bias = b is not None
        ctx.cl = (x.ndim == 4 and not x.is_contiguous())
        ctx.save_for_backward(x if 'x' in spec.ref or spec.has_2nd_grad else None, b if b is not None else None,
                              y if 'y' in spec.ref else None)
        return y

    @staticmethod
    def backward(ctx, dy):
        dim, spec, alpha, gain, clamp = ctx.cfg
        x, b, y = ctx.saved_tensors
        dx = db = None
        if ctx.needs_input_grad[0] or ctx.needs_input_grad[1]:
            dy = dy.contiguous(memory_format=torch.channels_last) if ctx.cl else dy.contiguous()
            dx = dy
            if spec.cuda_idx != 1 or gain != 1 or clamp >= 0:
                dx = _BiasActGrad.apply(dy, x, b, y, dim, spec, alpha, gain, clamp)
        if ctx.needs_input_grad[1] and ctx.has_bias:
            db = dx.sum([i for i in range(dx.ndim) if i != dim])
        return dx, db, None, None, None, None, None


class _BiasActGrad(torch.autograd.Function):

    @staticmethod
    def forward(ctx, dy, x, b, y, dim, spec, alpha, gain, clamp):
        ctx.cfg = (dim, spec, alpha, gain, clamp)
        ctx.cl = (dy.ndim == 4 and not dy.is_contiguous())
        dx = _plugin.bias_act(dy, b, x, y, None, 1, dim, spec.cuda_idx, alpha, gain, clamp)
        ctx.save_for_backward(dy if spec.has_2nd_grad else None, x, b, y)
        return dx

    @staticmethod
    def backward(ctx, d_dx):
        dim, spec, alpha, gain, clamp = ctx.cfg
        d_dx = d_dx.contiguous(memory_format=torch.channels_last) if ctx.cl else d_dx.contiguous()
        dy, x, b, y = ctx.saved_tensors
        d_dy = d_x = d_b = None
        if ctx.needs_input_grad[0]:
            d_dy = _BiasActGrad.apply(d_dx, x, b, y, dim, spec, alpha, gain, clamp)
        if spec.has_2nd_grad and (ctx.needs_input_grad[1] or ctx.needs_input_grad[2]):
            d_x = _plugin.bias_act(d_dx, b, x, y, dy, 2, dim, spec.cuda_idx, alpha, gain, clamp)
        if spec.has_2nd_grad and ctx.needs_input_grad[2]:
            d_b = d_x.sum([i for i in range(d_x.ndim) if i != dim])
        return d_dy, d_x, d_b, None, None, None, None, None, None


def bias_act(x, b=None, dim=1, act='linear', alpha=None, gain=None, clamp=None, impl='cuda'):
    assert isinstance(x, torch.Tensor)
    assert impl in ['ref', 'cuda']
    if impl == 'ref':
        raise NotImplementedError("ide3d_b200 has no PyTorch reference path; impl='ref' lives in oracle/ops.py (tests only)")
    if x.device.type != 'cuda':
        raise RuntimeError('ide3d_b200.bias_act: x must be a CUDA tensor (no CPU path in this package)')
    _init()
    assert clamp is None or clamp >= 0
    spec = activation_funcs[act]
    alpha = float(alpha if alpha is not None else spec.def_alpha)
    gain = float(gain if gain is not None else spec.def_gain)
    clamp = float(clamp if clamp is not None else -1)
    if b is not None:
        assert isinstance(b, torch.Tensor) and b.ndim == 1
        assert 0 <= dim < x.ndim
        assert b.shape[0] == x.shape[dim]
    if act == 'linear' and gain == 1 and clamp < 0 and b is None:
        return x
    if torch.is_grad_enabled() and (x.requires_grad or (b is not None and b.requires_grad)):
        return _BiasAct.apply(x, b, dim, spec, alpha, gain, clamp)
    return _plugin.bias_act(_layout(x), b, None, None, None, 0, dim, spec.cuda_idx, alpha, gain, clamp)


def scaled_bias_act(x, scale=None, noise=None, b=None, act='linear', alpha=None, gain=None, clamp=None, next_scale=None,
                    only_next=False, emit_y=True, y_scale=None, rgb=None):
    from . import fma
    if x.device.type != 'cuda':
        raise RuntimeError('ide3d_b200.scaled_bias_act: x must be a CUDA tensor (no CPU path in this package)')
    _init()
    if rgb is not None or y_scale is not None or not emit_y:
        return _scaled_bias_act_fold(x, scale, noise, b, act, alpha, gain, clamp, next_scale, emit_y and not only_next, y_scale, rgb)
    spec = activation_funcs[act]
    needs_grad = torch.is_grad_enabled() and any(t is not None and t.requires_grad for t in (x, scale, noise, b, next_scale))
    if not needs_grad and x.ndim == 4:
        out = _plugin.modconv_epilogue(_layout(x), scale, noise, b, spec.cuda_idx, float(alpha if alpha is not None else spec.def_alpha),
                                       float(gain if gain is not None else spec.def_gain), float(clamp if clamp is not None else -1),
                                       next_scale=next_scale, only_next=only_next)
        if out is not None:
            return out
    if scale is not None and noise is not None:
        x = fma.fma(x, scale.to(x.dtype).reshape(x.shape[0], -1, 1, 1), noise.to(x.dtype))
    elif scale is not None:
        x = x * scale.to(x.dtype).reshape(x.shape[0], -1, 1, 1)
    elif noise is not None:
        x = x + noise.to(x.dtype)
    y = bias_act(x, None if b is None else b.to(x.dtype), act=act, alpha=alpha, gain=gain, clamp=clamp)
    if next_scale is None:
        return y
    y2 = y * next_scale.to(y.dtype).reshape(y.shape[0], -1, 1, 1)
    return y2 if only_next else (y, y2)


def _scaled_bias_act_fold(x, scale, noise, b, act, alpha, gain, clamp, next_scale, emit_y, y_scale, rgb):
    from . import conv2d_resample
    spec = activation_funcs[act]
    alpha = float(alpha if alpha is not None else spec.def_alpha)
    gain = float(gain if gain is not None else spec.def_gain)
    clamp_f = float(clamp if clamp is not None else -1)
    needs_grad = torch.is_grad_enabled() and any(t is not None and t.requires_grad for t in (x, scale, noise, b, next_scale, y_scale, *(rgb or ())))
    if not needs_grad and x.ndim == 4:
        out = _plugin.modconv_epilogue_rgb(x, scale, noise, b, spec.cuda_idx, alpha, gain, clamp_f, emit_y=emit_y, y_scale=y_scale,
                                           next_scale=next_scale, rgb=rgb)
        if out is not None:
            return out
    y = scaled_bias_act(x, scale, noise, b, act=act, alpha=alpha, gain=gain, clamp=clamp)
    mod = lambda s: y * s.to(y.dtype).reshape(y.shape[0], -1, 1, 1)
    out = []
    if emit_y:
        out.append(y if y_scale is None else mod(y_scale))
    if next_scale is not None:
        out.append(mod(next_scale))
    if rgb is not None:
        weight, styles, bias = rgb
        r = conv2d_resample.conv2d_resample(x=mod(styles), w=weight.to(y.dtype))
        r = bias_act(r, None if bias is None else bias.to(r.dtype))
        out.append(r.contiguous())
    return out
```

ide-3d_b200/training/networks.py:

```python

import os

import numpy as np
import torch

from ..torch_utils import misc, persistence
from ..torch_utils.ops import bias_act, conv2d_resample, fma, upfirdn2d


FUSED_MODCONV_MIN_RES = 1 << 30

CHANNELS_LAST = os.environ.get('IDE3D_CHANNELS_LAST', '1') != '0'
STYLE_PLAN = os.environ.get('IDE3D_STYLE_PLAN', '1') != '0'
CHAIN_MODULATION = True
FUSED_TORGB = os.environ.get('IDE3D_FUSED_TORGB', '1') != '0'
CONV1X1_AS_MATMUL = os.environ.get('IDE3D_CONV1X1_MM', '0') != '0'


def _conv1x1_nhwc(x, weight):
    n, c, h, w = x.shape
    o = weight.shape[0]
    prev = torch.backends.cuda.matmul.allow_tf32
    torch.backends.cuda.matmul.allow_tf32 = bool(torch.backends.cudnn.allow_tf32)
    try:
        y = x.permute(0, 2, 3, 1).reshape(n * h * w, c) @ weight.reshape(o, c).t()
    finally:
        torch.backends.cuda.matmul.allow_tf32 = prev
    return y.reshape(n, h, w, o).permute(0, 3, 1, 2)


def normalize_2nd_moment(x, dim=1, eps=1e-8):
    return x * (x.square().mean(dim=dim, keepdim=True) + eps).rsqrt()


def modulated_conv2d(x, weight, styles, noise=None, up=1, down=1, padding=0, resample_filter=None, demodulate=True,
                     flip_weight=True, fused_modconv=True, epilogue=None, premodulated=False, dcoefs=None, w_transposed=None):
    batch_size = x.shape[0]
    out_channels, in_channels, kh, kw = weight.shape
    if x.dtype == torch.float16 and demodulate:
        weight = weight * (1 / np.sqrt(in_channels * kh * kw) / weight.norm(float('inf'), dim=[1, 2, 3], keepdim=True))
        styles = styles / styles.norm(float('inf'), dim=1, keepdim=True)
    w = None
    if fused_modconv:
        dcoefs = None
        w = weight.unsqueeze(0) * styles.reshape(batch_size, 1, -1, 1, 1)
    if demodulate and fused_modconv:
        dcoefs = (w.square().sum(dim=[2, 3, 4]) + 1e-8).rsqrt()
        w = w * dcoefs.reshape(batch_size, -1, 1, 1, 1)
    elif demodulate and dcoefs is not None:
        pass
    elif demodulate:
        dcoefs = (styles.square() @ weight.square().sum(dim=[2, 3]).t() + 1e-8).rsqrt()

    assert not (premodulated and (fused_modconv or (x.dtype == torch.float16 and demodulate)))
    if not fused_modconv:
        if not premodulated:
            x = bias_act.scaled_bias_act(x, scale=styles)
        if epilogue is not None and up > 1 and down == 1 and kh > 1:
            e = dict(epilogue)
            e['act_gain'] = e.pop('gain', None)
            e.update(scale=dcoefs if demodulate else None, noise=noise)
            return conv2d_resample.conv2d_resample(x=x, w=weight.to(x.dtype), f=resample_filter, up=up, down=down,
                                                   padding=padding, flip_weight=flip_weight, fir_epilogue=e, w_transposed=w_transposed)
        if (CONV1X1_AS_MATMUL and kh == 1 and kw == 1 and up == 1 and down == 1 and padding == 0 and x.dtype == torch.float32 and x.is_cuda
                and x.is_contiguous(memory_format=torch.channels_last) and not x.is_contiguous()
                and not (torch.is_grad_enabled() and (x.requires_grad or weight.requires_grad))):
            x = _conv1x1_nhwc(x, weight)
        else:
            x = conv2d_resample.conv2d_resample(x=x, w=weight.to(x.dtype), f=resample_filter, up=up, down=down,
                                                padding=padding, flip_weight=flip_weight)
        if epilogue is not None:
            return bias_act.scaled_bias_act(x, scale=dcoefs if demodulate else None, noise=noise, **epilogue)
        if demodulate and noise is not None:
            x = fma.fma(x, dcoefs.to(x.dtype).reshape(batch_size, -1, 1, 1), noise.to(x.dtype))
        elif demodulate:
            x = x * dcoefs.to(x.dtype).reshape(batch_size, -1, 1, 1)
        elif noise is not None:
            x = x.add_(noise.to(x.dtype))
        return x

    x = x.reshape(1, -1, *x.shape[2:])
    w = w.reshape(-1, in_channels, kh, kw)
    x = conv2d_resample.conv2d_resample(x=x, w=w.to(x.dtype), f=resample_filter, up=up, down=down, padding=padding,
                                        groups=batch_size, flip_weight=flip_weight)
    x = x.reshape(batch_size, -1, *x.shape[2:])
    if noise is not None:
        x = x.add_(noise)
    if epilogue is not None:
        b = epilogue['b']
        return bias_act.bias_act(x, None if b is None else b.to(x.dtype), act=epilogue.get('act', 'linear'), gain=epilogue.get('gain'),
                                 clamp=epilogue.get('clamp'))
    return x


@persistence.persistent_class
class FullyConnectedLayer(torch.nn.Module):

    def __init__(self, in_features, out_features, bias=True, activation='linear', lr_multiplier=1, bias_init=0):
        super().__init__()
        self.in_features, self.out_features, self.activation = in_features, out_features, activation
        self.weight = torch.nn.Parameter(torch.randn([out_features, in_features]) / lr_multiplier)
        self.bias = torch.nn.Parameter(torch.full([out_features], np.float32(bias_init))) if bias else None
        self.weight_gain = lr_multiplier / np.sqrt(in_features)
        self.bias_gain = lr_multiplier

    def effective(self):
        w = self.weight.to(torch.float32) * self.weight_gain
        b = None if self.bias is None else self.bias.to(torch.float32) * self.bias_gain
        return w, b

    def forward(self, x):
        w = self.weight.to(x.dtype) * self.weight_gain
        b = self.bias
        if b is not None:
            b = b.to(x.dtype)
            if self.bias_gain != 1:
                b = b * self.bias_gain
        if self.activation == 'linear' and b is not None:
            return torch.addmm(b.unsqueeze(0), x, w.t())
        x = x.matmul(w.t())
        return bias_act.bias_act(x, b, act=self.activation)


@persistence.persistent_class
class MappingNetwork(torch.nn.Module):

    def __init__(self, z_dim, c_dim, w_dim, num_ws, num_layers=8, embed_features=None, layer_features=None,
                 activation='lrelu', lr_multiplier=0.01, w_avg_beta=0.995):
        super().__init__()
        self.z_dim, self.c_dim, self.w_dim, self.num_ws = z_dim, c_dim, w_dim, num_ws
        self.num_layers, self.w_avg_beta = num_layers, w_avg_beta
        if embed_features is None:
            embed_features = w_dim
        if c_dim == 0:
            embed_features = 0
        if layer_features is None:
            layer_features = w_dim
        feats = [z_dim + embed_features] + [layer_features] * (num_layers - 1) + [w_dim]
        if c_dim > 0:
            self.embed = FullyConnectedLayer(c_dim, embed_features)
        for idx in range(num_layers):
            setattr(self, f'fc{idx}', FullyConnectedLayer(feats[idx], feats[idx + 1], activation=activation,
                                                          lr_multiplier=lr_multiplier))
        if num_ws is not None and w_avg_beta is not None:
            self.register_buffer('w_avg', torch.zeros([w_dim]))

    def forward(self, z=None, c=None, truncation_psi=1, truncation_cutoff=None, skip_w_avg_update=False, **_unused):
        x = None
        if self.z_dim > 0:
            misc.assert_shape(z, [None, self.z_dim])
            x = normalize_2nd_moment(z.to(torch.float32))
        if self.c_dim > 0:
            misc.assert_shape(c, [None, self.c_dim])
            y = normalize_2nd_moment(self.embed(c.to(torch.float32)))
            x = torch.cat([x, y], dim=1) if x is not None else y
        for idx in range(self.num_layers):
            x = getattr(self, f'fc{idx}')(x)
        if self.w_avg_beta is not None and self.training and not skip_w_avg_update:
            self.w_avg.copy_(x.detach().mean(dim=0).lerp(self.w_avg, self.w_avg_beta))
        if self.num_ws is not None:
            x = x.unsqueeze(1).repeat([1, self.num_ws, 1])
        if truncation_psi != 1:
            if self.num_ws is None or truncation_cutoff is None:
                x = self.w_avg.lerp(x, truncation_psi)
            else:
                x[:, :truncation_cutoff] = self.w_avg.lerp(x[:, :truncation_cutoff], truncation_psi)
        return x


@persistence.persistent_class
class SynthesisLayer(torch.nn.Module):

    def __init__(self, in_channels, out_channels, w_dim, resolution, kernel_size=3, up=1, use_noise=True,
                 activation='lrelu', resample_filter=[1, 3, 3, 1], conv_clamp=None, channels_last=False):
        super().__init__()
        self.resolution, self.up, self.use_noise = resolution, up, use_noise
        self.activation, self.conv_clamp = activation, conv_clamp
        self.register_buffer('resample_filter', upfirdn2d.setup_filter(resample_filter))
        self.padding = kernel_size // 2
        self.act_gain = bias_act.activation_funcs[activation].def_gain
        self.affine = FullyConnectedLayer(w_dim, in_channels, bias_init=1)
        memory_format = torch.channels_last if channels_last else torch.contiguous_format
        self.weight = torch.nn.Parameter(torch.randn([out_channels, in_channels, kernel_size, kernel_size]).to(memory_format=memory_format))
        if use_noise:
            self.register_buffer('noise_const', torch.randn([resolution, resolution]))
            self.noise_strength = torch.nn.Parameter(torch.zeros([]))
        self.bias = torch.nn.Parameter(torch.zeros([out_channels]))

    def forward(self, x, w, noise_mode='random', fused_modconv=True, gain=1, styles=None, premodulated=False, next_styles=None,
                only_next=False, dcoefs=None, y_styles=None, emit_y=True, rgb=None):
        assert noise_mode in ['random', 'const', 'none']
        if styles is None:
            styles = self.affine(w)
        noise = None
        if self.use_noise and noise_mode == 'random':
            noise = torch.randn([x.shape[0], 1, self.up * x.shape[2], self.up * x.shape[3]], device=x.device) * self.noise_strength
        inference = not (torch.is_grad_enabled() and (self.weight.requires_grad or (self.use_noise and (
            self.noise_strength.requires_grad or self.noise_const.requires_grad))))
        if self.use_noise and noise_mode == 'const':
            noise = self._cached('noise', (self.noise_const, self.noise_strength), lambda: self.noise_const * self.noise_strength) if inference \
                else self.noise_const * self.noise_strength
        act_gain = self.act_gain * gain
        act_clamp = self.conv_clamp * gain if self.conv_clamp is not None else None
        epilogue = dict(b=self.bias, act=self.activation, gain=act_gain, clamp=act_clamp)
        if next_styles is not None:
            epilogue.update(next_scale=next_styles, only_next=only_next)
        if y_styles is not None:
            epilogue['y_scale'] = y_styles
        if not emit_y:
            epilogue['emit_y'] = False
        if rgb is not None:
            epilogue['rgb'] = rgb
        w_t = None
        if inference and self.up > 1 and not fused_modconv and x.dtype == self.weight.dtype:
            fmt = torch.channels_last if CHANNELS_LAST else torch.contiguous_format
            w_t = self._cached('w_t', (self.weight,), lambda: self.weight.detach().transpose(0, 1).contiguous(memory_format=fmt))
        return modulated_conv2d(x=x, weight=self.weight, styles=styles, noise=noise, up=self.up, padding=self.padding,
                                resample_filter=self.resample_filter, flip_weight=(self.up == 1), fused_modconv=fused_modconv,
                                epilogue=epilogue, premodulated=premodulated, dcoefs=None if fused_modconv else dcoefs, w_transposed=w_t)

    def _cached(self, name, tensors, make):
        key = tuple((t.data_ptr(), t._version, str(t.device)) for t in tensors)
        store = self.__dict__.setdefault('_const_cache', {})
        hit = store.get(name)
        if hit is None or hit[0] != key:
            with torch.no_grad():
                hit = store[name] = (key, make())
        return hit[1]


@persistence.persistent_class
class ToRGBLayer(torch.nn.Module):

    def __init__(self, in_channels, out_channels, w_dim, kernel_size=1, conv_clamp=None, channels_last=False):
        super().__init__()
        self.conv_clamp = conv_clamp
        self.affine = FullyConnectedLayer(w_dim, in_channels, bias_init=1)
        memory_format = torch.channels_last if channels_last else torch.contiguous_format
        self.weight = torch.nn.Parameter(torch.randn([out_channels, in_channels, kernel_size, kernel_size]).to(memory_format=memory_format))
        self.bias = torch.nn.Parameter(torch.zeros([out_channels]))
        self.weight_gain = 1 / np.sqrt(in_channels * (kernel_size ** 2))

    def styles(self, w):
        return self.affine(w) * self.weight_gain

    def forward(self, x, w, fused_modconv=True, styles=None, premodulated=False, raw=False):
        if styles is None:
            styles = self.styles(w)
        return modulated_conv2d(x=x, weight=self.weight, styles=styles, demodulate=False, fused_modconv=fused_modconv,
                                epilogue=None if raw else dict(b=self.bias, clamp=self.conv_clamp), premodulated=premodulated)


@persistence.persistent_class
class SynthesisBlock(torch.nn.Module):

    def __init__(self, in_channels, out_channels, w_dim, resolution, img_channels, is_last, resample_filter=[1, 3, 3, 1],
                 conv_clamp=None, use_fp16=False, fp16_channels_last=False, **layer_kwargs):
        super().__init__()
        self.in_channels, self.out_channels, self.w_dim = in_channels, out_channels, w_dim
        self.resolution, self.img_channels, self.is_last = resolution, img_channels, is_last
        self.architecture = 'skip'
        self.use_fp16 = use_fp16
        self.channels_last = use_fp16 and fp16_channels_last
        self.register_buffer('resample_filter', upfirdn2d.setup_filter(resample_filter))
        self.num_conv = 0
        self.num_torgb = 0
        if in_channels == 0:
            self.const = torch.nn.Parameter(torch.randn([out_channels, resolution, resolution]))
        if in_channels != 0:
            self.conv0 = SynthesisLayer(in_channels, out_channels, w_dim=w_dim, resolution=resolution, up=2,
                                        resample_filter=resample_filter, conv_clamp=conv_clamp,
                                        channels_last=self.channels_last or CHANNELS_LAST, **layer_kwargs)
            self.num_conv += 1
        self.conv1 = SynthesisLayer(out_channels, out_channels, w_dim=w_dim, resolution=resolution, conv_clamp=conv_clamp,
                                    channels_last=self.channels_last or CHANNELS_LAST, **layer_kwargs)
        self.num_conv += 1
        self.torgb = ToRGBLayer(out_channels, img_channels, w_dim=w_dim, conv_clamp=conv_clamp,
                                channels_last=self.channels_last or CHANNELS_LAST)
        self.num_torgb += 1

    def can_fold(self):
        return FUSED_TORGB and CHAIN_MODULATION and CHANNELS_LAST and self.conv1.conv_clamp is None and self.torgb.conv_clamp is None

    def _features(self, x, ws, force_fp32, fused_modconv, layer_kwargs):
        layer_kwargs = dict(layer_kwargs)
        premod_in = layer_kwargs.pop('premodulated_x', False)
        x_next_styles = layer_kwargs.pop('x_next_styles', None)
        drop_x = layer_kwargs.pop('drop_x', False)
        misc.assert_shape(ws, [None, self.num_conv + self.num_torgb, self.w_dim])
        w_iter = iter(ws.unbind(dim=1))
        dtype = torch.float16 if self.use_fp16 and not force_fp32 else torch.float32
        memory_format = torch.channels_last if CHANNELS_LAST or (self.channels_last and not force_fp32) else torch.contiguous_format
        if fused_modconv is None:
            fused_modconv = (not self.training) and (dtype == torch.float32 or int(ws.shape[0]) == 1)
            thr = int(os.environ.get('IDE3D_FUSED_MODCONV_MIN_RES', FUSED_MODCONV_MIN_RES))
            fused_modconv = fused_modconv and self.resolution >= thr
        chain = CHAIN_MODULATION and (not fused_modconv) and dtype == torch.float32 and not (torch.is_grad_enabled() and (
            ws.requires_grad or any(p.requires_grad for p in self.parameters())))
        if not chain and (premod_in or x_next_styles is not None or drop_x):
            raise RuntimeError('SynthesisBlock: cross-block chaining needs the chained fp32 inference path')
        rgb_in = y_rgb = None
        if self.in_channels == 0:
            x = self.const.to(dtype=dtype).unsqueeze(0).repeat([ws.shape[0], 1, 1, 1]).contiguous(memory_format=memory_format)
            w1 = next(w_iter)
        else:
            misc.assert_shape(x, [None, self.in_channels, self.resolution // 2, self.resolution // 2])
            x = x.to(dtype=dtype, memory_format=memory_format)
            w0, w1 = next(w_iter), next(w_iter)
        w_rgb = next(w_iter)
        plan = layer_kwargs.pop('style_plan', None) if chain else None
        layer_kwargs.pop('style_plan', None)
        if chain:
            if plan is not None:
                (s1, d1), (s_rgb, _) = plan[self.conv1], plan[self.torgb]
                s0, d0 = plan[self.conv0] if self.in_channels != 0 else (None, None)
            else:
                s1, s_rgb, s0, d0, d1 = self.conv1.affine(w1), self.torgb.styles(w_rgb), None, None, None
            pre = False
            if self.in_channels != 0:
                x = self.conv0(x, w0, fused_modconv=False, styles=s0, dcoefs=d0, premodulated=premod_in, next_styles=s1, only_next=True,
                               **layer_kwargs)
                pre = True
            fold_rgb = x.is_cuda and self.torgb.weight.shape[0] <= 4 and self.can_fold()
            fold = {}
            if x_next_styles is not None:
                fold['y_styles'] = x_next_styles
            if drop_x:
                fold['emit_y'] = False
            if fold_rgb:
                fold['rgb'] = (self.torgb.weight, s_rgb, self.torgb.bias)
            outs = self.conv1(x, w1, fused_modconv=False, styles=s1, dcoefs=d1, premodulated=pre, next_styles=None if fold_rgb else s_rgb,
                              **fold, **layer_kwargs)
            x = None if drop_x else outs[0]
            if fold_rgb:
                y_rgb = outs[-1]
            else:
                rgb_in = (outs[-1], s_rgb)
        else:
            if self.in_channels != 0:
                x = self.conv0(x, w0, fused_modconv=fused_modconv, **layer_kwargs)
            x = self.conv1(x, w1, fused_modconv=fused_modconv, **layer_kwargs)
        return x, w_rgb, fused_modconv, rgb_in, y_rgb

    def _torgb(self, x, w_rgb, fused_modconv, rgb_in, raw=False):
        if rgb_in is not None:
            return self.torgb(rgb_in[0], w_rgb, fused_modconv=False, styles=rgb_in[1], premodulated=True, raw=raw)
        return self.torgb(x, w_rgb, fused_modconv=fused_modconv, raw=raw)

    def _fuse_skip(self, rgb_in, *imgs):
        return (rgb_in is not None and CHANNELS_LAST and self.torgb.conv_clamp is None and all(
            i is not None and i.dtype == torch.float32 and i.shape[-1] * 2 == self.resolution and i.shape[1] % 4 == 0 and
            i.stride(1) == 1 for i in imgs))

    def _accumulate(self, img, y):
        if img is not None and img.shape[-1] * 2 == y.shape[-1]:
            img = upfirdn2d.upsample2d(img, self.resample_filter)
        if CHANNELS_LAST and y.stride(1) == 1 and y.shape[1] % 4 == 0:
            y = y.to(dtype=torch.float32)
            return img.add_(y) if img is not None else y.contiguous(memory_format=torch.channels_last)
        y = y.to(dtype=torch.float32, memory_format=torch.contiguous_format)
        return img.add_(y) if img is not None else y

    def forward(self, x, img, ws, force_fp32=False, fused_modconv=None, **layer_kwargs):
        x, w_rgb, fused_modconv, rgb_in, y_rgb = self._features(x, ws, force_fp32, fused_modconv, layer_kwargs)
        if y_rgb is not None:
            return x, self._accumulate(img, y_rgb)
        if self._fuse_skip(rgb_in, img):
            y = self._torgb(x, w_rgb, fused_modconv, rgb_in, raw=True)
            return x, upfirdn2d.upsample2d_add(img, self.resample_filter, y, self.torgb.bias)
        img = self._accumulate(img, self._torgb(x, w_rgb, fused_modconv, rgb_in))
        return x, img


@persistence.persistent_class
class SegSynthesisBlock(SynthesisBlock):

    def __init__(self, in_channels, out_channels, w_dim, resolution, img_channels, seg_channels, is_last, **kwargs):
        super().__init__(in_channels, out_channels, w_dim, resolution, img_channels + seg_channels, is_last, **kwargs)
        self.img_channels, self.seg_channels = img_channels, seg_channels

    def _load_from_state_dict(self, state_dict, prefix, *args, **kwargs):
        ts = prefix + 'toseg.'
        if any(k.startswith(ts) for k in state_dict):
            for name in ('affine.weight', 'affine.bias'):
                a, b = state_dict.get(prefix + 'torgb.' + name), state_dict.get(ts + name)
                if a is None or b is None or a.shape != b.shape or not torch.equal(a, b):
                    raise RuntimeError(f'SegSynthesisBlock: {ts}{name} differs from torgb.{name}; a block with independent torgb / toseg '
                                       'affines has no equivalent in this single-ToRGB structure')
            for name in ('weight', 'bias'):
                state_dict[prefix + 'torgb.' + name] = torch.cat([state_dict[prefix + 'torgb.' + name], state_dict[ts + name]], 0)
            for k in [k for k in state_dict if k.startswith(ts)]:
                del state_dict[k]
        return super()._load_from_state_dict(state_dict, prefix, *args, **kwargs)

    def forward(self, x, img, ws, condition_img=None, force_fp32=False, fused_modconv=None, **layer_kwargs):
        x, w_shared, fused_modconv, rgb_in, y = self._features(x, ws, force_fp32, fused_modconv, layer_kwargs)
        if y is not None:
            return x, self._accumulate(img, y[:, :self.img_channels]), self._accumulate(condition_img, y[:, self.img_channels:])
        if self._fuse_skip(rgb_in, img, condition_img):
            y, b, ci = self._torgb(x, w_shared, fused_modconv, rgb_in, raw=True), self.torgb.bias, self.img_channels
            img = upfirdn2d.upsample2d_add(img, self.resample_filter, y[:, :ci], b[:ci])
            seg = upfirdn2d.upsample2d_add(condition_img, self.resample_filter, y[:, ci:], b[ci:])
            return x, img, seg
        y = self._torgb(x, w_shared, fused_modconv, rgb_in)
        img = self._accumulate(img, y[:, :self.img_channels])
        seg = self._accumulate(condition_img, y[:, self.img_channels:])
        return x, img, seg


class StylePlan:

    def __init__(self, blocks_with_base):
        self.entries = []
        for block, base in blocks_with_base:
            j = base
            if block.in_channels != 0:
                self.entries.append((block.conv0, j, True, 1.0)); j += 1
            self.entries.append((block.conv1, j, True, 1.0)); j += 1
            self.entries.append((block.torgb, j, False, float(block.torgb.weight_gain)))
        assert len(self.entries) <= 32
        self._key = None
        self._consts = None

    def _constants(self, device):
        params = [p for layer, *_ in self.entries for p in (layer.affine.weight, layer.affine.bias, layer.weight)]
        key = (str(device),) + tuple((p.data_ptr(), p._version) for p in params)
        if key == self._key:
            return self._consts
        from .. import _lib as L
        keep, structs = [], (L.StyleLayer * len(self.entries))()
        s_off = d_off = 0
        for k, (layer, w_index, demod, out_scale) in enumerate(self.entries):
            aw = layer.affine.weight.detach().to(device=device, dtype=torch.float32).contiguous()
            ab = layer.affine.bias.detach().to(device=device, dtype=torch.float32).contiguous()
            o, i = layer.weight.shape[0], layer.weight.shape[1]
            wsq = layer.weight.detach().to(device=device, dtype=torch.float32).square().sum(dim=[2, 3]).contiguous() if demod else None
            keep += [aw, ab, wsq]
            structs[k] = L.StyleLayer(aw.data_ptr(), ab.data_ptr(), wsq.data_ptr() if demod else None, float(layer.affine.weight_gain),
                                      float(layer.affine.bias_gain), float(out_scale), int(w_index), int(i), int(o), 0, 0)
            structs[k].style_off, structs[k].dcoef_off = s_off, d_off
            s_off += i
            d_off += o if demod else 0
        self._key, self._consts = key, (keep, structs, s_off, d_off)
        return self._consts

    @torch.no_grad()
    def run(self, ws):
        import ctypes as C
        from .. import _lib as L
        ws = ws.detach().to(torch.float32).contiguous()
        n, num_ws, w_dim = ws.shape
        _, base, s_tot, d_tot = self._constants(ws.device)
        structs = (L.StyleLayer * len(self.entries))()
        for k in range(len(self.entries)):
            C.memmove(C.byref(structs[k]), C.byref(base[k]), C.sizeof(L.StyleLayer))
            structs[k].style_off, structs[k].dcoef_off = base[k].style_off * n, base[k].dcoef_off * n
        styles = torch.empty(n * s_tot, dtype=torch.float32, device=ws.device)
        dcoefs = torch.empty(max(1, n * d_tot), dtype=torch.float32, device=ws.device)
        with torch.cuda.device(ws.device):
            L.check(L.get_lib().ide3d_style_plan(L.ptr(ws), n, num_ws, w_dim, structs, len(self.entries), L.ptr(styles), L.ptr(dcoefs),
                                                 L.stream_ptr(ws.device)))
        out = {}
        for k, (layer, _, demod, _) in enumerate(self.entries):
            i, o = structs[k].in_ch, structs[k].out_ch
            s = styles[structs[k].style_off:structs[k].style_off + n * i].view(n, i)
            d = dcoefs[structs[k].dcoef_off:structs[k].dcoef_off + n * o].view(n, o) if demod else None
            out[layer] = (s, d)
        return out
```

include/ide3d_b200.h:

```cpp
#ifndef IDE3D_B200_H_
#define IDE3D_B200_H_

#include <stdint.h>

#ifdef __cplusplus
extern "C" {
#endif

#define IDE3D_ABI_VERSION 1

enum ide3d_status {
    IDE3D_OK = 0,
    IDE3D_UNSUPPORTED = -1,
    IDE3D_INVALID = -2,
    IDE3D_CUDA_ERROR = -3
};

enum ide3d_dtype { IDE3D_F32 = 0, IDE3D_F16 = 1, IDE3D_F64 = 2 };

typedef void* ide3d_stream_t;

int ide3d_abi_version(void);
const char* ide3d_last_error(void);
uint64_t ide3d_launch_count(void);

int ide3d_bias_act(const void* x, const void* b, const void* xref, const void* yref, const void* dy,
                   void* y, int dtype, int grad, int act, float alpha, float gain, float clamp,
                   int64_t size_x, int64_t size_b, int64_t step_b, ide3d_stream_t stream);

int ide3d_modconv_epilogue(const void* x, const void* scale, const void* noise, const void* b, void* y,
                           const void* scale2, void* y2, int dtype, int act, float alpha, float gain, float clamp,
                           int64_t n, int64_t c, int64_t hw, int64_t noise_batch, int channels_last,
                           ide3d_stream_t stream);

int ide3d_modconv_epilogue_rgb(const void* x, const void* scale, const void* noise, const void* b, const void* yscale,
                               void* y, const void* scale2, void* y2, const void* wrgb, const void* srgb, const void* brgb,
                               void* rgb, int64_t rgb_channels, int dtype, int act, float alpha, float gain, float clamp,
                               int64_t n, int64_t c, int64_t hw, int64_t noise_batch, ide3d_stream_t stream);

typedef struct ide3d_upfirdn2d_params {
    const void* x;
    const float* f;
    void* y;
    int dtype;
    int up_x, up_y, down_x, down_y, pad_x0, pad_y0;
    int flip;
    float gain;
    int in_w, in_h, in_c, in_n;
    int64_t in_stride_w, in_stride_h, in_stride_c, in_stride_n;
    int f_w, f_h;
    int64_t f_stride_w, f_stride_h;
    int out_w, out_h;
    int64_t out_stride_w, out_stride_h, out_stride_c, out_stride_n;
} ide3d_upfirdn2d_params;
int ide3d_upfirdn2d(const ide3d_upfirdn2d_params* p, ide3d_stream_t stream);

int ide3d_upfirdn2d_add(const ide3d_upfirdn2d_params* p, const void* add, int64_t add_stride_n, int64_t add_stride_h,
                        int64_t add_stride_w, const void* bias, ide3d_stream_t stream);

typedef struct ide3d_fir_epilogue {
    const void *scale, *noise, *b, *scale2;
    void* y2;
    int act;
    float alpha, gain, clamp;
    int64_t noise_batch;
} ide3d_fir_epilogue;
int ide3d_upfirdn2d_epilogue(const ide3d_upfirdn2d_params* p, const ide3d_fir_epilogue* e, ide3d_stream_t stream);

typedef struct ide3d_filtered_lrelu_params {
    const void* x;
    const void* b;
    const float* fu;
    const float* fd;
    void* y;
    unsigned char* s;
    int dtype;
    int up, down;
    int fu_w, fu_h;
    int fd_w, fd_h;
    int pad_x0, pad_y0;
    int flip;
    float gain, slope, clamp;
    int x_w, x_h, x_c, x_n;
    int64_t x_stride_w, x_stride_h, x_stride_c, x_stride_n;
    int y_w, y_h;
    int64_t y_stride_w, y_stride_h, y_stride_c, y_stride_n;
    int s_w, s_h;
    int s_ofs_x, s_ofs_y;
    int write_signs, read_signs;
} ide3d_filtered_lrelu_params;
int ide3d_filtered_lrelu(const ide3d_filtered_lrelu_params* p, ide3d_stream_t stream);

typedef struct ide3d_filtered_lrelu_act_params {
    void* x;
    unsigned char* s;
    int dtype;
    int x_w, x_h, x_c, x_n;
    int64_t x_stride_w, x_stride_h, x_stride_c, x_stride_n;
    int s_w, s_h;
    int s_ofs_x, s_ofs_y;
    float gain, slope, clamp;
    int write_signs, read_signs;
} ide3d_filtered_lrelu_act_params;
int ide3d_filtered_lrelu_act(const ide3d_filtered_lrelu_act_params* p, ide3d_stream_t stream);

typedef struct ide3d_triplane {
    const float* data;
    int n, h, w;
    int64_t stride_n, stride_c, stride_h, stride_w;
} ide3d_triplane;

typedef struct ide3d_mlp_head {
    int in_sel, hidden, out_offset, out_count;
    const float *w1, *b1, *w2, *b2;
} ide3d_mlp_head;
typedef struct ide3d_decoder {
    int num_heads;
    ide3d_mlp_head heads[4];
} ide3d_decoder;

enum ide3d_jitter { IDE3D_JITTER_NONE = 0, IDE3D_JITTER_TENSOR = 1, IDE3D_JITTER_HASH = 2, IDE3D_JITTER_ZVALS = 3 };
enum ide3d_clamp { IDE3D_CLAMP_SOFTPLUS = 0, IDE3D_CLAMP_RELU = 1 };
enum ide3d_precision { IDE3D_PRECISION_AUTO = 0, IDE3D_PRECISION_FP32 = 1, IDE3D_PRECISION_TC = 2 };

typedef struct ide3d_raymarch_params {
    ide3d_triplane tex, seg;
    ide3d_decoder dec;
    const float* cam2world;
    int n;
    int res_w, res_h;
    int num_steps;
    float fov_deg, ray_start, ray_end;
    float box_scale;
    int jitter_mode;
    const float* jitter_u;
    uint64_t jitter_seed;
    int clamp_mode;
    int last_back, white_back;
    float max_depth;
    int fill_weight;
    float noise_std;
    const float* noise;
    float* out_feat;
    float* out_depth;
    float* out_weights;
    int precision;
    int views;
    const uint64_t* jitter_seeds;
} ide3d_raymarch_params;
int ide3d_raymarch_fwd(const ide3d_raymarch_params* p, ide3d_stream_t stream);

int ide3d_raymarch_bwd(const ide3d_raymarch_params* p, const float* grad_feat, const float* grad_depth, float* grad_tex,
                       float* grad_seg, float* const* grad_params, ide3d_stream_t stream);

int ide3d_raymarch_bwd_cam(const ide3d_raymarch_params* p, const float* grad_feat, const float* grad_depth, float* grad_tex,
                           float* grad_seg, float* const* grad_params, float* grad_cam2world, ide3d_stream_t stream);

int ide3d_sample_voxel(const ide3d_triplane* tex, const ide3d_triplane* seg, const ide3d_decoder* dec,
                       const float* points, int64_t num_points, float box_scale, int sigma_only,
                       float* out, ide3d_stream_t stream);

int ide3d_sigma_grid(const ide3d_triplane* tex, const ide3d_triplane* seg, const ide3d_decoder* dec,
                     int grid_n, const float voxel_origin[3], float cube_length, float pre_scale,
                     float box_scale, int64_t first, int64_t count, float* out, ide3d_stream_t stream);

int ide3d_planes_to_nhwc(const float* src, int n, int c, int h, int w, int64_t stride_n, int64_t stride_c,
                         int64_t stride_h, int64_t stride_w, float* dst, ide3d_stream_t stream);


int ide3d_initial_rays(int n, int num_steps, float fov_deg, int res_w, int res_h, float ray_start,
                       float ray_end, float* points, float* z_vals, float* rays_d_cam,
                       ide3d_stream_t stream);

int ide3d_transform_points(const float* points, const float* z_vals, const float* dirs, const float* u,
                           const float* cam2world, int n, int num_rays, int num_steps, float* points_world,
                           float* z_out, float* dirs_world, float* origins, ide3d_stream_t stream);

int ide3d_sample_triplane(const ide3d_triplane* planes, const float* coords, int64_t num_points,
                          float* out, ide3d_stream_t stream);

int ide3d_integrate(const float* rgb_sigma, const float* rays_d_cam, const float* z_vals, const float* noise,
                    float noise_std, int n, int num_rays, int num_steps, int channels, int clamp_mode,
                    int last_back, int white_back, float max_depth, int fill_weight, float* rgb,
                    float* depth, float* weights, ide3d_stream_t stream);

int ide3d_sample_pdf(const float* bins, const float* weights, const float* u, int num_rays, int num_bins,
                     int n_importance, float eps, float* samples, ide3d_stream_t stream);

int ide3d_mask2color(const float* masks, int n, int c, int h, int w, int64_t stride_n, int64_t stride_c, int64_t stride_h,
                     int64_t stride_w, const float* lut, void* out, int out_u8, ide3d_stream_t stream);

#define IDE3D_FRAMES_PARTIALS 64
enum ide3d_frames_mode { IDE3D_FRAMES_IMAGE_SEG = 1, IDE3D_FRAMES_IMAGE_DEPTH = 2 };
typedef struct ide3d_frames_params {
    const float* image;
    int n, height, width;
    int64_t image_stride_n, image_stride_c, image_stride_h, image_stride_w;
    const float* seg;
    int seg_c, seg_h, seg_w;
    int64_t seg_stride_n, seg_stride_c, seg_stride_h, seg_stride_w;
    const float* lut;
    int mode;
    uint8_t* out;
    float* scratch;
} ide3d_frames_params;
int ide3d_video_frames(const ide3d_frames_params* p, ide3d_stream_t stream);

typedef struct ide3d_strips_params {
    const float* image;
    int seeds, views, height, width;
    int64_t image_stride_n, image_stride_c, image_stride_h, image_stride_w;
    const float* seg;
    int seg_c, seg_h, seg_w;
    int64_t seg_stride_n, seg_stride_c, seg_stride_h, seg_stride_w;
    const float* lut;
    uint8_t* out_image;
    uint8_t* out_seg;
} ide3d_strips_params;
int ide3d_image_strips(const ide3d_strips_params* p, ide3d_stream_t stream);

int ide3d_mc_classify(const float* volume, int nx, int ny, int nz, float threshold, const int* ntri_table, unsigned char* counts,
                      ide3d_stream_t stream);
int ide3d_mc_emit(const float* volume, int nx, int ny, int nz, float threshold, const signed char* tri_table, const int* edge_corner,
                  const unsigned char* counts, const int64_t* offsets, int64_t* edge_ids, float* verts, ide3d_stream_t stream);

typedef struct ide3d_raster_params {
    const float* vertices;
    const int32_t* triangles;
    const float* normals;
    const float* cam2world;
    int64_t num_vertices, num_triangles;
    int num_frames, width, height;
    float yfov_deg, znear;
    float base, ambient, diffuse;
    int background;
    uint8_t* rgb;
    int32_t* ids;
    void* scratch;
    int64_t scratch_bytes;
} ide3d_raster_params;
int ide3d_mesh_normals(const float* vertices, const int32_t* triangles, int64_t num_vertices, const int32_t* adj_offsets,
                       const int32_t* adj_faces, float* normals, ide3d_stream_t stream);
int64_t ide3d_raster_scratch_bytes(int num_frames, int width, int height, int64_t num_vertices, int64_t num_triangles);
int ide3d_raster(const ide3d_raster_params* p, ide3d_stream_t stream);

typedef struct ide3d_style_layer {
    const float* affine_w;
    const float* affine_b;
    const float* wsq;
    float w_gain, b_gain;
    float out_scale;
    int w_index;
    int in_ch, out_ch;
    int64_t style_off, dcoef_off;
} ide3d_style_layer;
int ide3d_style_plan(const float* ws, int n, int num_ws, int w_dim, const ide3d_style_layer* layers, int num_layers,
                     float* styles, float* dcoefs, ide3d_stream_t stream);

#define IDE3D_NOISE_MAX_BUFFERS 64
typedef struct ide3d_noise_table {
    int count;
    int sides[IDE3D_NOISE_MAX_BUFFERS];
    float* bufs[IDE3D_NOISE_MAX_BUFFERS];
    float* grads[IDE3D_NOISE_MAX_BUFFERS];
    float* scratch;
    int64_t scratch_floats;
} ide3d_noise_table;
int ide3d_noise_reg(const ide3d_noise_table* t, float* loss, const float* grad_scale, ide3d_stream_t stream);
int ide3d_noise_normalize(const ide3d_noise_table* t, ide3d_stream_t stream);

typedef struct ide3d_seg_xent_params {
    const float* seg;
    int n, classes, in_h, in_w;
    int64_t seg_stride_n, seg_stride_c, seg_stride_h, seg_stride_w;
    const uint8_t* mask;
    int out_h, out_w;
    float* lse;
    double* partials;
    float* loss;
    const float* grad_loss;
    float* grad_seg;
} ide3d_seg_xent_params;
int ide3d_seg_xent_fwd(const ide3d_seg_xent_params* p, ide3d_stream_t stream);
int ide3d_seg_xent_bwd(const ide3d_seg_xent_params* p, ide3d_stream_t stream);

#define IDE3D_LPIPS_MAX_LAYERS 8
typedef struct ide3d_lpips_layer {
    int c, h, w;
    const float* x;
    int64_t x_stride[4];
    const float* y;
    int64_t y_stride[4];
    const float* lin;
    float* grad_x;
    int64_t gx_stride[4];
    float* grad_y;
    int64_t gy_stride[4];
} ide3d_lpips_layer;
typedef struct ide3d_lpips_params {
    int n, num_layers;
    ide3d_lpips_layer layers[IDE3D_LPIPS_MAX_LAYERS];
    float* value;
    void* scratch;
    int64_t scratch_bytes;
    const float* grad_value;
} ide3d_lpips_params;
int64_t ide3d_lpips_scratch_bytes(const ide3d_lpips_params* p);
int ide3d_lpips_fwd(const ide3d_lpips_params* p, ide3d_stream_t stream);
int ide3d_lpips_bwd(const ide3d_lpips_params* p, ide3d_stream_t stream);

#ifdef __cplusplus
}
#endif
#endif
```

Measured before the change: 777.1.

## Fuse conv1 epilogue with TF32 wgmma ToRGB and skip upsample-add for planes

```diff
diff --git a/ide-3d_b200/_lib.py b/ide-3d_b200/_lib.py
--- a/ide-3d_b200/_lib.py
+++ b/ide-3d_b200/_lib.py
@@ -186,6 +186,8 @@
     lib.ide3d_modconv_epilogue.argtypes = [vp, vp, vp, vp, vp, vp, vp, i32, i32, f32, f32, f32, i64, i64, i64, i64, i32, vp]
     lib.ide3d_modconv_epilogue_rgb.argtypes = [vp, vp, vp, vp, vp, vp, vp, vp, vp, vp, vp, vp, i64, i32, i32, f32, f32, f32, i64, i64, i64,
                                                i64, vp]
+    lib.ide3d_modconv_epilogue_planes.argtypes = [vp, vp, vp, vp, vp, vp, vp, vp, vp, i64, i64, C.POINTER(C.c_int64), C.POINTER(C.c_int64),
+                                                  C.POINTER(vp), C.POINTER(vp), vp, i32, i32, f32, f32, f32, i64, i64, i64, i64, i64, vp]
     lib.ide3d_upfirdn2d.argtypes = [C.POINTER(UpfirParams), vp]
     lib.ide3d_upfirdn2d_add.argtypes = [C.POINTER(UpfirParams), vp, i64, i64, i64, vp, vp]
     lib.ide3d_upfirdn2d_epilogue.argtypes = [C.POINTER(UpfirParams), C.POINTER(FirEpilogue), vp]
@@ -234,6 +236,7 @@
 
 def exported_symbols():
     return ['ide3d_abi_version', 'ide3d_last_error', 'ide3d_launch_count', 'ide3d_bias_act', 'ide3d_modconv_epilogue', 'ide3d_modconv_epilogue_rgb',
+            'ide3d_modconv_epilogue_planes',
             'ide3d_upfirdn2d', 'ide3d_upfirdn2d_add', 'ide3d_upfirdn2d_epilogue',
             'ide3d_filtered_lrelu', 'ide3d_filtered_lrelu_act', 'ide3d_raymarch_fwd', 'ide3d_raymarch_bwd', 'ide3d_raymarch_bwd_cam', 'ide3d_sample_voxel',
             'ide3d_sigma_grid', 'ide3d_planes_to_nhwc', 'ide3d_initial_rays', 'ide3d_transform_points',
diff --git a/ide-3d_b200/_plugins.py b/ide-3d_b200/_plugins.py
--- a/ide-3d_b200/_plugins.py
+++ b/ide-3d_b200/_plugins.py
@@ -136,6 +136,66 @@
     if L.check(rc, allow_unsupported=True) == L.UNSUPPORTED:
         return None
     return [t for t in (y, y2, out_rgb) if t is not None]
+
+
+def modconv_epilogue_planes(x, scale, noise, b, act, alpha, gain, clamp, emit_y, y_scale, planes):
+    L.require_cuda(x)
+    _req(x.ndim == 4, 'x must be rank 4')
+    n, c, h, w = x.shape
+    cl = (not x.is_contiguous()) and x.is_contiguous(memory_format=torch.channels_last)
+    weight, styles, bias, f, groups = planes
+    o = weight.shape[0]
+    if not cl or x.dtype != torch.float32 or c % 32 != 0 or c > 512 or o % 8 != 0 or o > 192 or len(groups) > 2 or (h * w) % 16 != 0:
+        return None
+    _req(sum(ch for ch, _ in groups) == o, 'the output groups must cover the ToRGB channels')
+    skips = []
+    for ch, skip in groups:
+        if skip is not None and (tuple(skip.shape) != (n, ch, h // 2, w // 2) or skip.dtype != x.dtype or
+                                 not skip.is_contiguous(memory_format=torch.channels_last)):
+            return None
+        skips.append(skip)
+
+    def per_sample(t, name):
+        if not _has(t):
+            return None
+        _req(t.numel() == n * c, f'{name} must have N*C elements')
+        return t.to(dtype=x.dtype).reshape(n, c).contiguous()
+
+    scale, y_scale, styles = per_sample(scale, 'scale'), per_sample(y_scale, 'y_scale'), per_sample(styles, 'rgb styles')
+    _req(styles is not None, 'rgb styles are required')
+    noise_batch = 1
+    if _has(noise):
+        _req(noise.numel() in (h * w, n * h * w), 'noise must be [H,W] or [N,1,H,W]')
+        noise_batch = noise.numel() // (h * w)
+        noise = noise.to(dtype=x.dtype).contiguous()
+    if _has(b):
+        _req(b.ndim == 1 and b.shape[0] == c, 'b has wrong number of elements')
+        b = b.to(dtype=x.dtype).contiguous()
+    _req(y_scale is None or emit_y, 'y_scale needs emit_y')
+    _req(weight.numel() == o * c, 'rgb weight must be [O, C, 1, 1]')
+    weight = weight.to(dtype=x.dtype).reshape(o, c).contiguous()
+    if bias is not None:
+        _req(bias.numel() == o, 'rgb bias must have O elements')
+        bias = bias.to(dtype=x.dtype).contiguous()
+    if any(s is not None for s in skips):
+        _req(f is not None and f.shape == (4, 4), 'the skip upsampling needs the 4x4 filter')
+        f = f.to(device=x.device, dtype=torch.float32).contiguous()
+    y = torch.empty_like(x) if emit_y else None
+    outs = [torch.empty([n, ch, h, w], dtype=x.dtype, device=x.device, memory_format=torch.channels_last) for ch, _ in groups]
+    begins, o0 = [], 0
+    for ch, _ in groups:
+        begins.append(o0)
+        o0 += ch
+    k = len(groups)
+    opt = lambda t: L.ptr(t) if t is not None else None
+    rc = L.get_lib().ide3d_modconv_epilogue_planes(
+        L.ptr(x), opt(scale), opt(noise), opt(b), opt(y_scale), opt(y), L.ptr(weight), L.ptr(styles), opt(bias), o, k,
+        (C.c_int64 * k)(*begins), (C.c_int64 * k)(*[ch for ch, _ in groups]), (C.c_void_p * k)(*[L.ptr(t) for t in outs]),
+        (C.c_void_p * k)(*[opt(s) for s in skips]), opt(f) if any(s is not None for s in skips) else None, L.dtype_code(x), int(act),
+        float(alpha), float(gain), float(clamp), n, c, h, w, noise_batch, L.stream_ptr(x.device))
+    if L.check(rc, allow_unsupported=True) == L.UNSUPPORTED:
+        return None
+    return ([y] if emit_y else []) + outs
 
 
 def upfirdn2d(x, f, upx, upy, downx, downy, padx0, padx1, pady0, pady1, flip, gain, add=None, bias=None, epilogue=None):
@@ -287,7 +347,7 @@
 
 PLUGINS = {
     'bias_act_plugin': _Plugin('bias_act_plugin', bias_act=bias_act, modconv_epilogue=modconv_epilogue,
-                                 modconv_epilogue_rgb=modconv_epilogue_rgb),
+                                 modconv_epilogue_rgb=modconv_epilogue_rgb, modconv_epilogue_planes=modconv_epilogue_planes),
     'upfirdn2d_plugin': _Plugin('upfirdn2d_plugin', upfirdn2d=upfirdn2d),
     'filtered_lrelu_plugin': _Plugin('filtered_lrelu_plugin', filtered_lrelu=filtered_lrelu,
                                      filtered_lrelu_act_=filtered_lrelu_act_),
diff --git a/ide-3d_b200/build.py b/ide-3d_b200/build.py
--- a/ide-3d_b200/build.py
+++ b/ide-3d_b200/build.py
@@ -12,7 +12,7 @@
 LIBDIR = os.path.join(HERE, 'lib')
 LIB = os.path.join(LIBDIR, 'libide3d_b200_tuning.so' if os.environ.get('IDE3D_BUILD_TUNING', '0') == '1' else 'libide3d_b200.so')
 TUNING = os.environ.get('IDE3D_BUILD_TUNING', '0') == '1'
-UNITS = ['capi', 'raymarch', 'raymarch_bwd', 'raymarch_tc', 'voxel', 'voxel_tc', 'stages', 'style_plan', 'mcubes', 'raster', 'frames', 'strips', 'projector', 'lpips', 'bias_act', 'upfirdn2d', 'filtered_lrelu', 'filtered_lrelu_fused']
+UNITS = ['capi', 'raymarch', 'raymarch_bwd', 'raymarch_tc', 'voxel', 'voxel_tc', 'stages', 'style_plan', 'mcubes', 'raster', 'frames', 'strips', 'projector', 'lpips', 'bias_act', 'torgb_tc', 'upfirdn2d', 'filtered_lrelu', 'filtered_lrelu_fused']
 NVCC_FLAGS = ['-O3', '-std=c++17', '--expt-relaxed-constexpr', '-gencode', 'arch=compute_90a,code=sm_90a',
               '-lineinfo', '-Xcompiler', '-fPIC', '-Xptxas', '-v'] + (['-DIDE3D_TUNING'] if TUNING else [])
 
diff --git a/ide-3d_b200/csrc/bias_act.cu b/ide-3d_b200/csrc/bias_act.cu
--- a/ide-3d_b200/csrc/bias_act.cu
+++ b/ide-3d_b200/csrc/bias_act.cu
@@ -1,4 +1,4 @@
-#include "common.cuh"
+#include "bias_act_common.cuh"
 
 namespace ide3d {
 
@@ -9,69 +9,6 @@
     float alpha, gain, clamp;
     long long size_x, size_b, step_b;
 };
-
-template <typename T> struct Acc { using type = float; };
-template <> struct Acc<double> { using type = double; };
-
-template <typename S> __device__ __forceinline__ S exp_(S v);
-template <> __device__ __forceinline__ float exp_<float>(float v) { return __expf(v); }
-template <> __device__ __forceinline__ double exp_<double>(double v) { return exp(v); }
-template <typename S> __device__ __forceinline__ S log_(S v);
-template <> __device__ __forceinline__ float log_<float>(float v) { return __logf(v); }
-template <> __device__ __forceinline__ double log_<double>(double v) { return log(v); }
-
-template <typename S, int A>
-__device__ __forceinline__ S eval(S x, S b, S xref, S yref, S dy, int G, S alpha, S gain, S clamp) {
-    const S one = (S)1, two = (S)2, expRange = (S)80, halfExpRange = (S)40;
-    const S seluScale = (S)1.0507009873554804934193349852946, seluAlpha = (S)1.6732632423543772848170429916717;
-    const S yy = (gain != (S)0) ? yref / gain : (S)0;
-    S y = 0;
-    if (G == 0) x += b; else xref += b;
-    if (A == 1) { y = x; if (G == 2) y = 0; }
-    if (A == 2) { if (G == 0) y = (x > 0) ? x : 0; if (G == 1) y = (yy > 0) ? x : 0; }
-    if (A == 3) { if (G == 0) y = (x > 0) ? x : x * alpha; if (G == 1) y = (yy > 0) ? x : x * alpha; }
-    if (A == 4) {
-        if (G == 0) { const S c = exp_(x), d = one / c; y = (x < -expRange) ? -one : (x > expRange) ? one : (c - d) / (c + d); }
-        if (G == 1) y = x * (one - yy * yy);
-        if (G == 2) y = x * (one - yy * yy) * (-two * yy);
-    }
-    if (A == 5) {
-        if (G == 0) y = (x < -expRange) ? 0 : one / (exp_(-x) + one);
-        if (G == 1) y = x * yy * (one - yy);
-        if (G == 2) y = x * yy * (one - yy) * (one - two * yy);
-    }
-    if (A == 6) {
-        if (G == 0) y = (x >= 0) ? x : exp_(x) - one;
-        if (G == 1) y = (yy >= 0) ? x : x * (yy + one);
-        if (G == 2) y = (yy >= 0) ? 0 : x * (yy + one);
-    }
-    if (A == 7) {
-        if (G == 0) y = (x >= 0) ? seluScale * x : (seluScale * seluAlpha) * (exp_(x) - one);
-        if (G == 1) y = (yy >= 0) ? x * seluScale : x * (yy + seluScale * seluAlpha);
-        if (G == 2) y = (yy >= 0) ? 0 : x * (yy + seluScale * seluAlpha);
-    }
-    if (A == 8) {
-        if (G == 0) y = (x > expRange) ? x : log_(exp_(x) + one);
-        if (G == 1) y = x * (one - exp_(-yy));
-        if (G == 2) { const S c = exp_(-yy); y = x * c * (one - c); }
-    }
-    if (A == 9) {
-        if (G == 0) {
-            y = (x < -expRange) ? 0 : x / (exp_(-x) + one);
-        } else {
-            const S c = exp_(xref), d = c + one;
-            if (G == 1) y = (xref > halfExpRange) ? x : x * c * (xref + d) / (d * d);
-            else y = (xref > halfExpRange) ? 0 : x * c * (xref * (two - d) + two * d) / (d * d * d);
-            yref = (xref < -expRange) ? 0 : xref / (exp_(-xref) + one) * gain;
-        }
-    }
-    y *= gain * dy;
-    if (clamp >= 0) {
-        if (G == 0) y = (y > -clamp & y < clamp) ? y : (y >= 0) ? clamp : -clamp;
-        else y = (yref > -clamp & yref < clamp) ? y : 0;
-    }
-    return y;
-}
 
 __device__ __forceinline__ long long bias_index(long long e, const BiasActArgs& p, bool small) {
     if (small) return (long long)(((unsigned)e / (unsigned)p.step_b) % (unsigned)p.size_b);
diff --git a/ide-3d_b200/csrc/bias_act_common.cuh b/ide-3d_b200/csrc/bias_act_common.cuh
--- /dev/null
+++ b/ide-3d_b200/csrc/bias_act_common.cuh
@@ -0,0 +1,70 @@
+#pragma once
+
+#include "common.cuh"
+
+namespace ide3d {
+
+template <typename T> struct Acc { using type = float; };
+template <> struct Acc<double> { using type = double; };
+
+template <typename S> __device__ __forceinline__ S exp_(S v);
+template <> __device__ __forceinline__ float exp_<float>(float v) { return __expf(v); }
+template <> __device__ __forceinline__ double exp_<double>(double v) { return exp(v); }
+template <typename S> __device__ __forceinline__ S log_(S v);
+template <> __device__ __forceinline__ float log_<float>(float v) { return __logf(v); }
+template <> __device__ __forceinline__ double log_<double>(double v) { return log(v); }
+
+template <typename S, int A>
+__device__ __forceinline__ S eval(S x, S b, S xref, S yref, S dy, int G, S alpha, S gain, S clamp) {
+    const S one = (S)1, two = (S)2, expRange = (S)80, halfExpRange = (S)40;
+    const S seluScale = (S)1.0507009873554804934193349852946, seluAlpha = (S)1.6732632423543772848170429916717;
+    const S yy = (gain != (S)0) ? yref / gain : (S)0;
+    S y = 0;
+    if (G == 0) x += b; else xref += b;
+    if (A == 1) { y = x; if (G == 2) y = 0; }
+    if (A == 2) { if (G == 0) y = (x > 0) ? x : 0; if (G == 1) y = (yy > 0) ? x : 0; }
+    if (A == 3) { if (G == 0) y = (x > 0) ? x : x * alpha; if (G == 1) y = (yy > 0) ? x : x * alpha; }
+    if (A == 4) {
+        if (G == 0) { const S c = exp_(x), d = one / c; y = (x < -expRange) ? -one : (x > expRange) ? one : (c - d) / (c + d); }
+        if (G == 1) y = x * (one - yy * yy);
+        if (G == 2) y = x * (one - yy * yy) * (-two * yy);
+    }
+    if (A == 5) {
+        if (G == 0) y = (x < -expRange) ? 0 : one / (exp_(-x) + one);
+        if (G == 1) y = x * yy * (one - yy);
+        if (G == 2) y = x * yy * (one - yy) * (one - two * yy);
+    }
+    if (A == 6) {
+        if (G == 0) y = (x >= 0) ? x : exp_(x) - one;
+        if (G == 1) y = (yy >= 0) ? x : x * (yy + one);
+        if (G == 2) y = (yy >= 0) ? 0 : x * (yy + one);
+    }
+    if (A == 7) {
+        if (G == 0) y = (x >= 0) ? seluScale * x : (seluScale * seluAlpha) * (exp_(x) - one);
+        if (G == 1) y = (yy >= 0) ? x * seluScale : x * (yy + seluScale * seluAlpha);
+        if (G == 2) y = (yy >= 0) ? 0 : x * (yy + seluScale * seluAlpha);
+    }
+    if (A == 8) {
+        if (G == 0) y = (x > expRange) ? x : log_(exp_(x) + one);
+        if (G == 1) y = x * (one - exp_(-yy));
+        if (G == 2) { const S c = exp_(-yy); y = x * c * (one - c); }
+    }
+    if (A == 9) {
+        if (G == 0) {
+            y = (x < -expRange) ? 0 : x / (exp_(-x) + one);
+        } else {
+            const S c = exp_(xref), d = c + one;
+            if (G == 1) y = (xref > halfExpRange) ? x : x * c * (xref + d) / (d * d);
+            else y = (xref > halfExpRange) ? 0 : x * c * (xref * (two - d) + two * d) / (d * d * d);
+            yref = (xref < -expRange) ? 0 : xref / (exp_(-xref) + one) * gain;
+        }
+    }
+    y *= gain * dy;
+    if (clamp >= 0) {
+        if (G == 0) y = (y > -clamp & y < clamp) ? y : (y >= 0) ? clamp : -clamp;
+        else y = (yref > -clamp & yref < clamp) ? y : 0;
+    }
+    return y;
+}
+
+}
diff --git a/ide-3d_b200/csrc/tc_ptx.cuh b/ide-3d_b200/csrc/tc_ptx.cuh
--- a/ide-3d_b200/csrc/tc_ptx.cuh
+++ b/ide-3d_b200/csrc/tc_ptx.cuh
@@ -98,6 +98,24 @@
     }
 };
 
+template <int N> struct WgmmaTf32;
+
+template <> struct WgmmaTf32<192> {
+    __device__ __forceinline__ static void rs(float* d, const uint32_t (&a)[4], uint64_t b_desc) {
+        asm volatile(
+            "{\n\t.reg .pred p;\n\tsetp.ne.b32 p, %101, 0;\n\t"
+            "wgmma.mma_async.sync.aligned.m64n192k8.f32.tf32.tf32 {%0, %1, %2, %3, %4, %5, %6, %7, %8, %9, %10, %11, %12, %13, %14, %15, %16, %17, %18, %19, %20, %21, %22, %23, %24, %25, %26, %27, %28, %29, %30, %31, %32, %33, %34, %35, %36, %37, %38, %39, %40, %41, %42, %43, %44, %45, %46, %47, %48, %49, %50, %51, %52, %53, %54, %55, %56, %57, %58, %59, %60, %61, %62, %63, %64, %65, %66, %67, %68, %69, %70, %71, %72, %73, %74, %75, %76, %77, %78, %79, %80, %81, %82, %83, %84, %85, %86, %87, %88, %89, %90, %91, %92, %93, %94, %95}, {%96, %97, %98, %99}, %100, p, 1, 1;\n\t}\n"
+            : "+f"(d[0]), "+f"(d[1]), "+f"(d[2]), "+f"(d[3]), "+f"(d[4]), "+f"(d[5]), "+f"(d[6]), "+f"(d[7]), "+f"(d[8]), "+f"(d[9]), "+f"(d[10]), "+f"(d[11]), "+f"(d[12]), "+f"(d[13]), "+f"(d[14]), "+f"(d[15]), "+f"(d[16]), "+f"(d[17]), "+f"(d[18]), "+f"(d[19]), "+f"(d[20]), "+f"(d[21]), "+f"(d[22]), "+f"(d[23]), "+f"(d[24]), "+f"(d[25]), "+f"(d[26]), "+f"(d[27]), "+f"(d[28]), "+f"(d[29]), "+f"(d[30]), "+f"(d[31]), "+f"(d[32]), "+f"(d[33]), "+f"(d[34]), "+f"(d[35]), "+f"(d[36]), "+f"(d[37]), "+f"(d[38]), "+f"(d[39]), "+f"(d[40]), "+f"(d[41]), "+f"(d[42]), "+f"(d[43]), "+f"(d[44]), "+f"(d[45]), "+f"(d[46]), "+f"(d[47]), "+f"(d[48]), "+f"(d[49]), "+f"(d[50]), "+f"(d[51]), "+f"(d[52]), "+f"(d[53]), "+f"(d[54]), "+f"(d[55]), "+f"(d[56]), "+f"(d[57]), "+f"(d[58]), "+f"(d[59]), "+f"(d[60]), "+f"(d[61]), "+f"(d[62]), "+f"(d[63]), "+f"(d[64]), "+f"(d[65]), "+f"(d[66]), "+f"(d[67]), "+f"(d[68]), "+f"(d[69]), "+f"(d[70]), "+f"(d[71]), "+f"(d[72]), "+f"(d[73]), "+f"(d[74]), "+f"(d[75]), "+f"(d[76]), "+f"(d[77]), "+f"(d[78]), "+f"(d[79]), "+f"(d[80]), "+f"(d[81]), "+f"(d[82]), "+f"(d[83]), "+f"(d[84]), "+f"(d[85]), "+f"(d[86]), "+f"(d[87]), "+f"(d[88]), "+f"(d[89]), "+f"(d[90]), "+f"(d[91]), "+f"(d[92]), "+f"(d[93]), "+f"(d[94]), "+f"(d[95])
+            : "r"(a[0]), "r"(a[1]), "r"(a[2]), "r"(a[3]), "l"(b_desc), "r"(1));
+    }
+};
+
+__device__ __forceinline__ uint32_t to_tf32(float x) {
+    uint32_t r;
+    asm("cvt.rna.tf32.f32 %0, %1;" : "=r"(r) : "f"(x));
+    return r;
+}
+
 __device__ __forceinline__ void split_bf16(float x, __nv_bfloat16& hi, __nv_bfloat16& lo) {
     hi = __float2bfloat16_rn(x);
     lo = __float2bfloat16_rn(x - __bfloat162float(hi));
diff --git a/ide-3d_b200/csrc/torgb_tc.cu b/ide-3d_b200/csrc/torgb_tc.cu
--- /dev/null
+++ b/ide-3d_b200/csrc/torgb_tc.cu
@@ -0,0 +1,279 @@
+#include "bias_act_common.cuh"
+#include "tc_ptx.cuh"
+#include "upfirdn2d_common.cuh"
+
+namespace ide3d {
+namespace {
+
+constexpr int kNT = 192;
+constexpr int kKC = 32;
+constexpr int kChunkBytes = kNT * kKC * 4;
+constexpr int kResidentChunks = 8;
+constexpr int kThreads = 256;
+constexpr int kTileM = 128;
+constexpr int kMaxGroups = 2;
+
+struct PlanesArgs {
+    const float *x, *scale, *noise, *b, *yscale;
+    float* y;
+    const float *wrgb, *srgb, *brgb, *filter;
+    float* out[kMaxGroups];
+    const float* skip[kMaxGroups];
+    int gbeg[kMaxGroups], gch[kMaxGroups];
+    int groups;
+    float alpha, gain, clamp;
+    int n, c, h, w, hw, o, noise_batch;
+    long long m;
+};
+
+__device__ __forceinline__ void stage_w(const PlanesArgs& p, unsigned char* dst, int kc) {
+    for (int f = threadIdx.x; f < kNT * 8; f += kThreads) {
+        const int row = f >> 3, m = f & 7;
+        float4 v = make_float4(0.f, 0.f, 0.f, 0.f);
+        if (row < p.o) v = __ldg(reinterpret_cast<const float4*>(p.wrgb + (long long)row * p.c + kc * kKC + 4 * m));
+        const float e[4] = {v.x, v.y, v.z, v.w};
+        const int kk = (m >> 1) + 4 * (m & 1);
+#pragma unroll
+        for (int s = 0; s < 4; ++s)
+            *reinterpret_cast<uint32_t*>(dst + tc::sw128_offset(row, 2 * s + (kk >> 2)) + (kk & 3) * 4) = tc::to_tf32(e[s]);
+    }
+}
+
+__device__ __forceinline__ void ld8(const float* p, float (&o)[8]) {
+    const float4 a = __ldg(reinterpret_cast<const float4*>(p)), b = __ldg(reinterpret_cast<const float4*>(p) + 1);
+    o[0] = a.x; o[1] = a.y; o[2] = a.z; o[3] = a.w; o[4] = b.x; o[5] = b.y; o[6] = b.z; o[7] = b.w;
+}
+
+constexpr int kStageBytes = kThreads * 64;
+
+__device__ __forceinline__ void cp_async16(void* dst, const void* src) {
+    asm volatile("cp.async.cg.shared.global [%0], [%1], 16;" ::"r"(tc::smem_u32(dst)), "l"(src) : "memory");
+}
+__device__ __forceinline__ void cp_async_commit() { asm volatile("cp.async.commit_group;" ::: "memory"); }
+template <int N> __device__ __forceinline__ void cp_async_wait() { asm volatile("cp.async.wait_group %0;" ::"n"(N) : "memory"); }
+
+}
+
+template <int A, int S>
+__global__ void __launch_bounds__(kThreads, 1) modconv_epilogue_planes_tc_kernel(const PlanesArgs p, int resident) {
+    extern __shared__ unsigned char smem_raw[];
+    unsigned char* wsm = reinterpret_cast<unsigned char*>((reinterpret_cast<uintptr_t>(smem_raw) + 1023) & ~(uintptr_t)1023);
+    const int nk = p.c / kKC;
+    unsigned char* ring = wsm + (resident ? nk : 1) * kChunkBytes + threadIdx.x * 16;
+    if (resident) {
+        for (int kc = 0; kc < nk; ++kc) stage_w(p, wsm + kc * kChunkBytes, kc);
+        tc::fence_async_smem();
+        __syncthreads();
+    }
+    const int wg = threadIdx.x >> 7, wi = (threadIdx.x >> 5) & 3, lane = threadIdx.x & 31, g = lane >> 2, t = lane & 3;
+    float fk[4][4];
+#pragma unroll
+    for (int ky = 0; ky < 4; ++ky)
+#pragma unroll
+        for (int kx = 0; kx < 4; ++kx) fk[ky][kx] = p.filter ? __ldg(p.filter + (3 - ky) * 4 + (3 - kx)) * 4.f : 0.f;
+
+    const long long tiles = (p.m + kTileM - 1) / kTileM;
+    const long long steps = blockIdx.x < tiles ? ((tiles - 1 - blockIdx.x) / gridDim.x + 1) * nk : 0;
+    auto issue = [&](long long it) {
+        if (it < steps) {
+            const long long tl = it / nk;
+            const int kc = (int)(it - tl * nk);
+            const long long r0 = (blockIdx.x + tl * gridDim.x) * kTileM + wg * 64 + wi * 16;
+            if (r0 < p.m) {
+                const float* src = p.x + (r0 + g) * p.c + kc * kKC + 8 * t;
+                unsigned char* dst = ring + (int)(it % S) * kStageBytes;
+                cp_async16(dst, src);
+                cp_async16(dst + kThreads * 16, src + 4);
+                cp_async16(dst + 2 * kThreads * 16, src + 8ll * p.c);
+                cp_async16(dst + 3 * kThreads * 16, src + 8ll * p.c + 4);
+            }
+        }
+        cp_async_commit();
+    };
+    for (int s = 0; s < S - 1; ++s) issue(s);
+    long long it = 0;
+    for (long long tile = blockIdx.x; tile < tiles; tile += gridDim.x) {
+        const long long row0 = tile * kTileM + wg * 64 + wi * 16;
+        const bool live = row0 < p.m;
+        const int smp = live ? (int)(row0 / p.hw) : 0;
+        const int pa = live ? (int)(row0 - (long long)smp * p.hw) + g : 0, pb = pa + 8;
+        float acc[kNT / 2];
+#pragma unroll
+        for (int i = 0; i < kNT / 2; ++i) acc[i] = 0.f;
+        float nza = 0.f, nzb = 0.f;
+        if (p.noise && live) {
+            const long long nb = p.noise_batch == 1 ? 0ll : (long long)smp * p.hw;
+            nza = __ldg(p.noise + nb + pa);
+            nzb = __ldg(p.noise + nb + pb);
+        }
+        for (int kc = 0; kc < nk; ++kc, ++it) {
+            if (!resident) {
+                __syncthreads();
+                stage_w(p, wsm, kc);
+                tc::fence_async_smem();
+                __syncthreads();
+            }
+            cp_async_wait<S - 2>();
+            float4 nx[4] = {make_float4(0.f, 0.f, 0.f, 0.f), make_float4(0.f, 0.f, 0.f, 0.f), make_float4(0.f, 0.f, 0.f, 0.f),
+                            make_float4(0.f, 0.f, 0.f, 0.f)};
+            if (live) {
+                const unsigned char* src = ring + (int)(it % S) * kStageBytes;
+#pragma unroll
+                for (int i = 0; i < 4; ++i) nx[i] = *reinterpret_cast<const float4*>(src + i * kThreads * 16);
+            }
+            issue(it + S - 1);
+            float xr[2][8] = {{nx[0].x, nx[0].y, nx[0].z, nx[0].w, nx[1].x, nx[1].y, nx[1].z, nx[1].w},
+                              {nx[2].x, nx[2].y, nx[2].z, nx[2].w, nx[3].x, nx[3].y, nx[3].z, nx[3].w}};
+            const int ch = kc * kKC + 8 * t;
+            const long long sv = (long long)smp * p.c + ch;
+            float d[8], bb[8], sr[8];
+            if (p.scale) ld8(p.scale + sv, d);
+            if (p.b) ld8(p.b + ch, bb);
+            ld8(p.srgb + sv, sr);
+            float tv[2][8];
+#pragma unroll
+            for (int r = 0; r < 2; ++r) {
+                const float nz = r ? nzb : nza;
+#pragma unroll
+                for (int j = 0; j < 8; ++j) {
+                    float v = p.scale ? xr[r][j] * d[j] : xr[r][j];
+                    if (p.noise) v = p.scale ? xr[r][j] * d[j] + nz : xr[r][j] + nz;
+                    tv[r][j] = eval<float, A>(v, p.b ? bb[j] : 0.f, 0.f, 0.f, 1.f, 0, p.alpha, p.gain, p.clamp);
+                }
+            }
+            if (p.y && live) {
+                float ys[8];
+                if (p.yscale) ld8(p.yscale + sv, ys);
+#pragma unroll
+                for (int r = 0; r < 2; ++r) {
+                    float o8[8];
+#pragma unroll
+                    for (int j = 0; j < 8; ++j) o8[j] = p.yscale ? tv[r][j] * ys[j] : tv[r][j];
+                    float* yp = p.y + ((long long)smp * p.hw + (r ? pb : pa)) * p.c + ch;
+                    __stcs(reinterpret_cast<float4*>(yp), make_float4(o8[0], o8[1], o8[2], o8[3]));
+                    __stcs(reinterpret_cast<float4*>(yp) + 1, make_float4(o8[4], o8[5], o8[6], o8[7]));
+                }
+            }
+            uint32_t af[4][4];
+#pragma unroll
+            for (int s = 0; s < 4; ++s) {
+                af[s][0] = tc::to_tf32(tv[0][s] * sr[s]);
+                af[s][1] = tc::to_tf32(tv[1][s] * sr[s]);
+                af[s][2] = tc::to_tf32(tv[0][4 + s] * sr[4 + s]);
+                af[s][3] = tc::to_tf32(tv[1][4 + s] * sr[4 + s]);
+            }
+            const uint32_t wbase = tc::smem_u32(wsm + (resident ? kc : 0) * kChunkBytes);
+            tc::wgmma_fence();
+#pragma unroll
+            for (int s = 0; s < 4; ++s) tc::WgmmaTf32<kNT>::rs(acc, af[s], tc::make_sdesc_sw128(wbase + 32 * s));
+            tc::wgmma_commit();
+            tc::wgmma_wait<0>();
+            tc::fence_regs(acc);
+        }
+        if (!live) continue;
+        const int oya = pa / p.w, oxa = pa - oya * p.w, oyb = pb / p.w, oxb = pb - oyb * p.w;
+#pragma unroll
+        for (int j = 0; j < kNT / 8; ++j) {
+            const int o = 8 * j + 2 * t;
+            if (8 * j >= p.o) break;
+            const int gi = (p.groups > 1 && 8 * j >= p.gbeg[1]) ? 1 : 0;
+            const int oc = o - p.gbeg[gi];
+            if (8 * j < p.gbeg[gi] || 8 * j >= p.gbeg[gi] + p.gch[gi]) continue;
+            const float b0 = p.brgb ? __ldg(p.brgb + o) : 0.f, b1 = p.brgb ? __ldg(p.brgb + o + 1) : 0.f;
+            float va0 = acc[4 * j] + b0, va1 = acc[4 * j + 1] + b1, vb0 = acc[4 * j + 2] + b0, vb1 = acc[4 * j + 3] + b1;
+            const int og = p.gch[gi];
+            if (p.skip[gi]) {
+                const int ih = p.h >> 1, iw = p.w >> 1;
+                const float* sk = p.skip[gi] + (long long)smp * ih * iw * og + oc;
+                up2_skip_fma(fk, sk, ih, iw, og, oya, oxa, va0, va1);
+                up2_skip_fma(fk, sk, ih, iw, og, oyb, oxb, vb0, vb1);
+            }
+            float* op = p.out[gi] + ((long long)smp * p.hw) * og + oc;
+            __stcs(reinterpret_cast<float2*>(op + (long long)pa * og), make_float2(va0, va1));
+            __stcs(reinterpret_cast<float2*>(op + (long long)pb * og), make_float2(vb0, vb1));
+        }
+    }
+}
+
+namespace {
+
+template <int A>
+int launch_planes(const PlanesArgs& p, cudaStream_t st) {
+    const int nk = p.c / kKC;
+    const int resident = nk <= kResidentChunks;
+    const int deep = !resident || nk <= 4;
+    const size_t smem = (size_t)(resident ? nk : 1) * kChunkBytes + (size_t)(deep ? 6 : 2) * kStageBytes + 1024;
+    const long long tiles = (p.m + kTileM - 1) / kTileM;
+    void (*kern)(const PlanesArgs, int) = deep ? modconv_epilogue_planes_tc_kernel<A, 6> : modconv_epilogue_planes_tc_kernel<A, 2>;
+    int grid = 1;
+    const int rc = persistent_grid(kern, kThreads, smem, tiles, grid);
+    if (rc != IDE3D_OK) return rc;
+    kern<<<grid, kThreads, smem, st>>>(p, resident);
+    IDE3D_CHECK_LAUNCH("modconv_epilogue_planes_tc_kernel");
+    return IDE3D_OK;
+}
+
+}
+}
+
+extern "C" int ide3d_modconv_epilogue_planes(const void* x, const void* scale, const void* noise, const void* b, const void* yscale, void* y,
+                                             const void* wrgb, const void* srgb, const void* brgb, int64_t rgb_channels, int64_t groups,
+                                             const int64_t* group_begin, const int64_t* group_channels, void* const* out,
+                                             const void* const* skip, const void* filter, int dtype, int act, float alpha, float gain,
+                                             float clamp, int64_t n, int64_t c, int64_t h, int64_t w, int64_t noise_batch,
+                                             ide3d_stream_t stream) {
+    using namespace ide3d;
+    IDE3D_REQUIRE(n >= 0 && c >= 0 && h >= 0 && w >= 0, "modconv_epilogue_planes: negative size");
+    if (n * c * h * w == 0) return IDE3D_OK;
+    IDE3D_REQUIRE(x && wrgb && srgb, "modconv_epilogue_planes: null x / ToRGB weight / ToRGB styles");
+    IDE3D_REQUIRE(yscale == nullptr || y != nullptr, "modconv_epilogue_planes: yscale without y");
+    IDE3D_REQUIRE(rgb_channels >= 1, "modconv_epilogue_planes: no ToRGB output channels");
+    IDE3D_REQUIRE(groups >= 1 && group_begin && group_channels && out, "modconv_epilogue_planes: no output group");
+    IDE3D_REQUIRE(noise == nullptr || noise_batch == 1 || noise_batch == n, "modconv_epilogue_planes: noise batch must be 1 or n");
+    IDE3D_REQUIRE(act >= 1 && act <= 9, "modconv_epilogue_planes: unknown activation index %d", act);
+    const uintptr_t a16 = (uintptr_t)x | (uintptr_t)y | (uintptr_t)scale | (uintptr_t)b | (uintptr_t)yscale | (uintptr_t)wrgb | (uintptr_t)srgb;
+    IDE3D_REQUIRE((a16 & 15) == 0, "modconv_epilogue_planes: x, y, the per-channel operands and the ToRGB weight must be 16-byte aligned");
+    IDE3D_REQUIRE((((uintptr_t)noise | (uintptr_t)brgb | (uintptr_t)filter) & 3) == 0, "modconv_epilogue_planes: noise / bias / filter must be 4-byte aligned");
+    if (groups > kMaxGroups) IDE3D_FAIL(IDE3D_UNSUPPORTED, "modconv_epilogue_planes: at most %d output groups", kMaxGroups);
+    for (int g = 0; g < (int)groups; ++g) {
+        IDE3D_REQUIRE(out[g] != nullptr, "modconv_epilogue_planes: null output of group %d", g);
+        IDE3D_REQUIRE(group_begin[g] >= 0 && group_channels[g] >= 1 && group_begin[g] + group_channels[g] <= rgb_channels,
+                      "modconv_epilogue_planes: channel range of group %d outside the ToRGB output", g);
+        IDE3D_REQUIRE(g == 0 || group_begin[g] >= group_begin[g - 1] + group_channels[g - 1], "modconv_epilogue_planes: group channel ranges overlap or are unordered");
+        IDE3D_REQUIRE((((uintptr_t)out[g] | (uintptr_t)(skip ? skip[g] : nullptr)) & 7) == 0, "modconv_epilogue_planes: outputs / skips must be 8-byte aligned");
+        IDE3D_REQUIRE(skip == nullptr || skip[g] == nullptr || (filter != nullptr && h % 2 == 0 && w % 2 == 0),
+                      "modconv_epilogue_planes: a skip image needs the filter and an even output size");
+    }
+    if (dtype != IDE3D_F32) IDE3D_FAIL(IDE3D_UNSUPPORTED, "modconv_epilogue_planes: float32 only");
+    if (c % kKC != 0 || c > 512) IDE3D_FAIL(IDE3D_UNSUPPORTED, "modconv_epilogue_planes: needs C %% 32 == 0 and C <= 512 (got %lld)", (long long)c);
+    if (rgb_channels % 8 != 0 || rgb_channels > kNT) IDE3D_FAIL(IDE3D_UNSUPPORTED, "modconv_epilogue_planes: needs O %% 8 == 0 and O <= %d", kNT);
+    for (int g = 0; g < (int)groups; ++g)
+        if (group_begin[g] % 8 != 0 || group_channels[g] % 8 != 0) IDE3D_FAIL(IDE3D_UNSUPPORTED, "modconv_epilogue_planes: group channels must be multiples of 8");
+    if ((h * w) % 16 != 0 || n * h * w >= (1ll << 31) || n * h * w * c >= (1ll << 40)) IDE3D_FAIL(IDE3D_UNSUPPORTED, "modconv_epilogue_planes: needs H*W %% 16 == 0");
+    PlanesArgs p{};
+    p.x = (const float*)x; p.scale = (const float*)scale; p.noise = (const float*)noise; p.b = (const float*)b;
+    p.yscale = (const float*)yscale; p.y = (float*)y; p.wrgb = (const float*)wrgb; p.srgb = (const float*)srgb; p.brgb = (const float*)brgb;
+    p.filter = (const float*)filter; p.groups = (int)groups;
+    for (int g = 0; g < (int)groups; ++g) {
+        p.out[g] = (float*)out[g];
+        p.skip[g] = skip ? (const float*)skip[g] : nullptr;
+        p.gbeg[g] = (int)group_begin[g];
+        p.gch[g] = (int)group_channels[g];
+    }
+    p.alpha = alpha; p.gain = gain; p.clamp = clamp;
+    p.n = (int)n; p.c = (int)c; p.h = (int)h; p.w = (int)w; p.hw = (int)(h * w); p.o = (int)rgb_channels; p.noise_batch = (int)noise_batch;
+    p.m = n * h * w;
+    cudaStream_t st = (cudaStream_t)stream;
+    switch (act) {
+        case 1: return launch_planes<1>(p, st);
+        case 2: return launch_planes<2>(p, st);
+        case 3: return launch_planes<3>(p, st);
+        case 4: return launch_planes<4>(p, st);
+        case 5: return launch_planes<5>(p, st);
+        case 6: return launch_planes<6>(p, st);
+        case 7: return launch_planes<7>(p, st);
+        case 8: return launch_planes<8>(p, st);
+        case 9: return launch_planes<9>(p, st);
+    }
+    IDE3D_FAIL(IDE3D_INVALID, "modconv_epilogue_planes: unknown activation index %d", act);
+}
diff --git a/ide-3d_b200/csrc/upfirdn2d.cu b/ide-3d_b200/csrc/upfirdn2d.cu
--- a/ide-3d_b200/csrc/upfirdn2d.cu
+++ b/ide-3d_b200/csrc/upfirdn2d.cu
@@ -2,6 +2,7 @@
 #include <stdlib.h>
 
 #include "common.cuh"
+#include "upfirdn2d_common.cuh"
 
 namespace ide3d {
 
@@ -32,32 +33,6 @@
 template <> __device__ __forceinline__ float ld<__half>(const __half* p) { return __half2float(*p); }
 template <typename T> __device__ __forceinline__ void st(T* p, typename AccT<T>::type v) { *p = (T)v; }
 template <> __device__ __forceinline__ void st<__half>(__half* p, float v) { *p = __float2half(v); }
-
-constexpr int cmod(int a, int m) { return ((a % m) + m) % m; }
-constexpr int cfloor(int a, int m) { return (a - cmod(a, m)) / m; }
-constexpr int kPatch = 4;
-constexpr int kTile = 64;
-
-template <int U, int D, int F, int PH>
-struct Axis {
-    static constexpr int k0(int j) { return cmod(PH - j * D, U); }
-    static constexpr int taps(int j) { return k0(j) < F ? (F - k0(j) + U - 1) / U : 0; }
-    static constexpr int off(int j) { return cfloor(j * D - PH + k0(j), U); }
-    static constexpr int lo() {
-        int m = 1 << 20;
-        for (int j = 0; j < kPatch; ++j) if (taps(j) > 0 && off(j) < m) m = off(j);
-        return m == (1 << 20) ? 0 : m;
-    }
-    static constexpr int hi() {
-        int m = -(1 << 20);
-        for (int j = 0; j < kPatch; ++j) if (taps(j) > 0 && off(j) + taps(j) - 1 > m) m = off(j) + taps(j) - 1;
-        return m == -(1 << 20) ? 0 : m;
-    }
-    static constexpr int kWin = hi() - lo() + 1;
-    static constexpr int kStep = kPatch * D / U;
-    static constexpr int kTileIn = (kTile / kPatch - 1) * kStep + kWin;
-    static_assert((kPatch * D) % U == 0, "patch origin must stay phase aligned");
-};
 
 template <typename T, typename TT, int UX, int UY, int DX, int DY, int FW, int FH, int PHX, int PHY, int PITCH>
 __device__ __forceinline__ void patch_compute_store_impl(const UpfirArgs& p, const TT* __restrict__ tile,
diff --git a/ide-3d_b200/csrc/upfirdn2d_common.cuh b/ide-3d_b200/csrc/upfirdn2d_common.cuh
--- /dev/null
+++ b/ide-3d_b200/csrc/upfirdn2d_common.cuh
@@ -0,0 +1,55 @@
+#pragma once
+
+#include "common.cuh"
+
+namespace ide3d {
+
+constexpr int cmod(int a, int m) { return ((a % m) + m) % m; }
+constexpr int cfloor(int a, int m) { return (a - cmod(a, m)) / m; }
+constexpr int kPatch = 4;
+constexpr int kTile = 64;
+
+template <int U, int D, int F, int PH>
+struct Axis {
+    static constexpr int k0(int j) { return cmod(PH - j * D, U); }
+    static constexpr int taps(int j) { return k0(j) < F ? (F - k0(j) + U - 1) / U : 0; }
+    static constexpr int off(int j) { return cfloor(j * D - PH + k0(j), U); }
+    static constexpr int lo() {
+        int m = 1 << 20;
+        for (int j = 0; j < kPatch; ++j) if (taps(j) > 0 && off(j) < m) m = off(j);
+        return m == (1 << 20) ? 0 : m;
+    }
+    static constexpr int hi() {
+        int m = -(1 << 20);
+        for (int j = 0; j < kPatch; ++j) if (taps(j) > 0 && off(j) + taps(j) - 1 > m) m = off(j) + taps(j) - 1;
+        return m == -(1 << 20) ? 0 : m;
+    }
+    static constexpr int kWin = hi() - lo() + 1;
+    static constexpr int kStep = kPatch * D / U;
+    static constexpr int kTileIn = (kTile / kPatch - 1) * kStep + kWin;
+    static_assert((kPatch * D) % U == 0, "patch origin must stay phase aligned");
+};
+
+__device__ __forceinline__ void up2_skip_fma(const float (&fk)[4][4], const float* skip, int ih, int iw, int pitch, int oy, int ox,
+                                             float& v0, float& v1) {
+    using AX = Axis<2, 1, 4, 0>;
+    static_assert(AX::k0(0) == 0 && AX::k0(1) == 1 && AX::k0(2) == 0 && AX::k0(3) == 1, "first tap = output phase");
+    const int jy = oy & (kPatch - 1), jx = ox & (kPatch - 1);
+    const int iy0 = (oy - jy) / 2 - 1 + AX::off(jy), ix0 = (ox - jx) / 2 - 1 + AX::off(jx);
+    const bool py = oy & 1, px = ox & 1;
+#pragma unroll
+    for (int ty = 0; ty < 2; ++ty) {
+        const int iy = iy0 + ty;
+#pragma unroll
+        for (int tx = 0; tx < 2; ++tx) {
+            const int ix = ix0 + tx;
+            const float w = py ? (px ? fk[1 + 2 * ty][1 + 2 * tx] : fk[1 + 2 * ty][2 * tx]) : (px ? fk[2 * ty][1 + 2 * tx] : fk[2 * ty][2 * tx]);
+            float2 s = make_float2(0.f, 0.f);
+            if ((unsigned)iy < (unsigned)ih && (unsigned)ix < (unsigned)iw) s = __ldg(reinterpret_cast<const float2*>(skip + ((long long)iy * iw + ix) * pitch));
+            v0 = fmaf(w, s.x, v0);
+            v1 = fmaf(w, s.y, v1);
+        }
+    }
+}
+
+}
diff --git a/ide-3d_b200/torch_utils/ops/bias_act.py b/ide-3d_b200/torch_utils/ops/bias_act.py
--- a/ide-3d_b200/torch_utils/ops/bias_act.py
+++ b/ide-3d_b200/torch_utils/ops/bias_act.py
@@ -120,13 +120,13 @@
 
 
 def scaled_bias_act(x, scale=None, noise=None, b=None, act='linear', alpha=None, gain=None, clamp=None, next_scale=None,
-                    only_next=False, emit_y=True, y_scale=None, rgb=None):
+                    only_next=False, emit_y=True, y_scale=None, rgb=None, planes=None):
     from . import fma
     if x.device.type != 'cuda':
         raise RuntimeError('ide3d_b200.scaled_bias_act: x must be a CUDA tensor (no CPU path in this package)')
     _init()
-    if rgb is not None or y_scale is not None or not emit_y:
-        return _scaled_bias_act_fold(x, scale, noise, b, act, alpha, gain, clamp, next_scale, emit_y and not only_next, y_scale, rgb)
+    if rgb is not None or planes is not None or y_scale is not None or not emit_y:
+        return _scaled_bias_act_fold(x, scale, noise, b, act, alpha, gain, clamp, next_scale, emit_y and not only_next, y_scale, rgb, planes)
     spec = activation_funcs[act]
     needs_grad = torch.is_grad_enabled() and any(t is not None and t.requires_grad for t in (x, scale, noise, b, next_scale))
     if not needs_grad and x.ndim == 4:
@@ -148,14 +148,22 @@
     return y2 if only_next else (y, y2)
 
 
-def _scaled_bias_act_fold(x, scale, noise, b, act, alpha, gain, clamp, next_scale, emit_y, y_scale, rgb):
-    from . import conv2d_resample
+def _scaled_bias_act_fold(x, scale, noise, b, act, alpha, gain, clamp, next_scale, emit_y, y_scale, rgb, planes=None):
+    from . import conv2d_resample, upfirdn2d
     spec = activation_funcs[act]
     alpha = float(alpha if alpha is not None else spec.def_alpha)
     gain = float(gain if gain is not None else spec.def_gain)
     clamp_f = float(clamp if clamp is not None else -1)
     needs_grad = torch.is_grad_enabled() and any(t is not None and t.requires_grad for t in (x, scale, noise, b, next_scale, y_scale, *(rgb or ())))
-    if not needs_grad and x.ndim == 4:
+    if planes is not None:
+        assert rgb is None and next_scale is None
+        needs_grad = needs_grad or torch.is_grad_enabled() and any(isinstance(t, torch.Tensor) and t.requires_grad for t in (
+            *planes[:4], *(s for _, s in planes[4])))
+        if not needs_grad and x.ndim == 4:
+            out = _plugin.modconv_epilogue_planes(x, scale, noise, b, spec.cuda_idx, alpha, gain, clamp_f, emit_y, y_scale, planes)
+            if out is not None:
+                return out
+    elif not needs_grad and x.ndim == 4:
         out = _plugin.modconv_epilogue_rgb(x, scale, noise, b, spec.cuda_idx, alpha, gain, clamp_f, emit_y=emit_y, y_scale=y_scale,
                                            next_scale=next_scale, rgb=rgb)
         if out is not None:
@@ -172,4 +180,16 @@
         r = conv2d_resample.conv2d_resample(x=mod(styles), w=weight.to(y.dtype))
         r = bias_act(r, None if bias is None else bias.to(r.dtype))
         out.append(r.contiguous())
+    if planes is not None:
+        weight, styles, bias, f, groups = planes
+        r = conv2d_resample.conv2d_resample(x=mod(styles), w=weight.to(y.dtype))
+        o0 = 0
+        for ch, skip in groups:
+            bg = None if bias is None else bias[o0:o0 + ch]
+            if skip is None:
+                g = r[:, o0:o0 + ch] if bg is None else r[:, o0:o0 + ch] + bg.to(r.dtype).reshape(1, -1, 1, 1)
+                out.append(g.contiguous(memory_format=torch.channels_last))
+            else:
+                out.append(upfirdn2d.upsample2d_add(skip, f, r[:, o0:o0 + ch], bg))
+            o0 += ch
     return out
diff --git a/ide-3d_b200/training/networks.py b/ide-3d_b200/training/networks.py
--- a/ide-3d_b200/training/networks.py
+++ b/ide-3d_b200/training/networks.py
@@ -14,6 +14,7 @@
 STYLE_PLAN = os.environ.get('IDE3D_STYLE_PLAN', '1') != '0'
 CHAIN_MODULATION = True
 FUSED_TORGB = os.environ.get('IDE3D_FUSED_TORGB', '1') != '0'
+FUSED_PLANES_MAX_C = 256
 CONV1X1_AS_MATMUL = os.environ.get('IDE3D_CONV1X1_MM', '0') != '0'
 
 
@@ -188,7 +189,7 @@
         self.bias = torch.nn.Parameter(torch.zeros([out_channels]))
 
     def forward(self, x, w, noise_mode='random', fused_modconv=True, gain=1, styles=None, premodulated=False, next_styles=None,
-                only_next=False, dcoefs=None, y_styles=None, emit_y=True, rgb=None):
+                only_next=False, dcoefs=None, y_styles=None, emit_y=True, rgb=None, planes=None):
         assert noise_mode in ['random', 'const', 'none']
         if styles is None:
             styles = self.affine(w)
@@ -211,6 +212,8 @@
             epilogue['emit_y'] = False
         if rgb is not None:
             epilogue['rgb'] = rgb
+        if planes is not None:
+            epilogue['planes'] = planes
         w_t = None
         if inference and self.up > 1 and not fused_modconv and x.dtype == self.weight.dtype:
             fmt = torch.channels_last if CHANNELS_LAST else torch.contiguous_format
@@ -282,7 +285,7 @@
     def can_fold(self):
         return FUSED_TORGB and CHAIN_MODULATION and CHANNELS_LAST and self.conv1.conv_clamp is None and self.torgb.conv_clamp is None
 
-    def _features(self, x, ws, force_fp32, fused_modconv, layer_kwargs):
+    def _features(self, x, ws, force_fp32, fused_modconv, layer_kwargs, skips=None):
         layer_kwargs = dict(layer_kwargs)
         premod_in = layer_kwargs.pop('premodulated_x', False)
         x_next_styles = layer_kwargs.pop('x_next_styles', None)
@@ -322,6 +325,8 @@
                                **layer_kwargs)
                 pre = True
             fold_rgb = x.is_cuda and self.torgb.weight.shape[0] <= 4 and self.can_fold()
+            fold_planes = (skips is not None and x.is_cuda and not fold_rgb and self.can_fold() and torch.backends.cudnn.allow_tf32
+                           and (x_next_styles is not None or drop_x) and self.out_channels <= FUSED_PLANES_MAX_C)
             fold = {}
             if x_next_styles is not None:
                 fold['y_styles'] = x_next_styles
@@ -329,10 +334,15 @@
                 fold['emit_y'] = False
             if fold_rgb:
                 fold['rgb'] = (self.torgb.weight, s_rgb, self.torgb.bias)
-            outs = self.conv1(x, w1, fused_modconv=False, styles=s1, dcoefs=d1, premodulated=pre, next_styles=None if fold_rgb else s_rgb,
+            if fold_planes:
+                fold['planes'] = (self.torgb.weight, s_rgb, self.torgb.bias, self.resample_filter, skips)
+            outs = self.conv1(x, w1, fused_modconv=False, styles=s1, dcoefs=d1, premodulated=pre,
+                              next_styles=None if fold_rgb or fold_planes else s_rgb,
                               **fold, **layer_kwargs)
             x = None if drop_x else outs[0]
-            if fold_rgb:
+            if fold_planes:
+                y_rgb = list(outs[-len(skips):])
+            elif fold_rgb:
                 y_rgb = outs[-1]
             else:
                 rgb_in = (outs[-1], s_rgb)
@@ -394,7 +404,10 @@
         return super()._load_from_state_dict(state_dict, prefix, *args, **kwargs)
 
     def forward(self, x, img, ws, condition_img=None, force_fp32=False, fused_modconv=None, **layer_kwargs):
-        x, w_shared, fused_modconv, rgb_in, y = self._features(x, ws, force_fp32, fused_modconv, layer_kwargs)
+        skips = [(self.img_channels, img), (self.seg_channels, condition_img)]
+        x, w_shared, fused_modconv, rgb_in, y = self._features(x, ws, force_fp32, fused_modconv, layer_kwargs, skips=skips)
+        if isinstance(y, list):
+            return x, y[0], y[1]
         if y is not None:
             return x, self._accumulate(img, y[:, :self.img_channels]), self._accumulate(condition_img, y[:, self.img_channels:])
         if self._fuse_skip(rgb_in, img, condition_img):
diff --git a/include/ide3d_b200.h b/include/ide3d_b200.h
--- a/include/ide3d_b200.h
+++ b/include/ide3d_b200.h
@@ -37,6 +37,12 @@
                                void* y, const void* scale2, void* y2, const void* wrgb, const void* srgb, const void* brgb,
                                void* rgb, int64_t rgb_channels, int dtype, int act, float alpha, float gain, float clamp,
                                int64_t n, int64_t c, int64_t hw, int64_t noise_batch, ide3d_stream_t stream);
+
+int ide3d_modconv_epilogue_planes(const void* x, const void* scale, const void* noise, const void* b, const void* yscale, void* y,
+                                  const void* wrgb, const void* srgb, const void* brgb, int64_t rgb_channels, int64_t groups,
+                                  const int64_t* group_begin, const int64_t* group_channels, void* const* out, const void* const* skip,
+                                  const void* filter, int dtype, int act, float alpha, float gain, float clamp, int64_t n, int64_t c,
+                                  int64_t h, int64_t w, int64_t noise_batch, ide3d_stream_t stream);
 
 typedef struct ide3d_upfirdn2d_params {
     const void* x;
```

After: 792.0 (median of 6 runs). 1.9% higher.
